# snayfach/MicrobeCensus

Hardware: AMD Instinct MI355X
Metric: reads/sec searched vs marker DB + AGS abs-error, 150 bp @ 1/2/4/8 GPU (higher is better)
Workload: dtype u8/int32

## Files before the change

### include/mcensus.h

```cpp
#ifndef MCENSUS_H
#define MCENSUS_H
#include <stdint.h>
#ifdef __cplusplus
extern "C" {
#endif

typedef struct mc_handle mc_handle;

typedef struct mc_row {
    int32_t query, subject;
    double ident;
    int32_t alnlen, mismatch, gapopen, qstart, qend, sstart, send;
    double loge, bits;
    int32_t score, nmatch;
} mc_row;

typedef struct mc_best_hit {
    int32_t read, family, aln, target_len;
    double bits;
} mc_best_hit;

typedef struct mc_stats {
    int64_t reads, seed_tasks, gap_tasks, hsps, rows, reads_with_rows, classified;
    int64_t bucket_lookups, key_probes;
    float ms_translate, ms_seed, ms_eval, ms_gapped, ms_sort, ms_finish, ms_total;
    int64_t seed_exact_asks, seed_wild_asks, seed_pair_asks, seed_probes;
    int64_t range_splits;
} mc_stats;

const char *mc_last_error(void);
int mc_device_count(void);

mc_handle *mc_open(const char *const *names, const char *const *seqs, int32_t nseq,
                   const int32_t *marker_family, int32_t nfam, int32_t device);
void mc_close(mc_handle *h);
int mc_set_index_cache(const char *dir);
int mc_index_cache_check(const char *const *names, const char *const *seqs, int32_t nseq, const char *dir);

mc_handle *mc_open_rapdb(const char *rapdb_path, int32_t device);
int32_t mc_marker_count(const mc_handle *h);
const char *mc_marker_name(const mc_handle *h, int32_t i);
int mc_set_families(mc_handle *h, const int32_t *marker_family, int32_t nfam);
int mc_rapdb_verify(const char *rapdb_path, const char *const *names, const char *const *seqs, int32_t nseq);
int mc_rapdb_write(const char *const *names, const char *const *seqs, int32_t nseq, const char *path);

int mc_index_view(const mc_handle *h, const uint8_t **res_codes, const uint32_t **offsets, const uint32_t **bucket_starts,
                  const uint32_t **postings, const uint16_t **keys, int64_t *nres, int64_t *npostings,
                  uint32_t *freq_thr, double letter_p[10]);

int mc_set_run(mc_handle *h, int32_t read_len, double loge_thr, const double *min_cov, const double *min_score,
               const int32_t *max_aaid, const int32_t *aln_stat);

int mc_search(mc_handle *h, const uint8_t *reads, int64_t nreads, int64_t first_read_id);

int mc_search_varlen(mc_handle *h, const uint8_t *bases, const int64_t *offsets, int64_t nreads, int64_t first_read_id);

int mc_set_run_classes(mc_handle *h, const int32_t *class_len, int32_t K, double loge_thr, const double *min_cov, const double *min_score,
                       const int32_t *max_aaid, const int32_t *aln_stat);
int mc_search_classes(mc_handle *h, const uint8_t *rows, int64_t nreads, int32_t stride, int64_t first_read_id);
int64_t mc_result_best_classes(mc_handle *h, const uint8_t **cls);
int mc_result_class_reads(mc_handle *h, int64_t *out );
int64_t mc_debug_classes_prologue(mc_handle *h, const uint8_t *rows, int64_t nreads, int32_t stride, uint32_t *perm, uint32_t *start, int64_t *word0,
                                  uint8_t *sorted, int64_t sorted_cap, float *ms);

int mc_upload(mc_handle *h, const uint8_t *reads, int64_t nreads);
int mc_attach(mc_handle *h, const void *device_reads, int64_t nreads);
int mc_run(mc_handle *h, int64_t first_read_id);
int mc_run_range(mc_handle *h, int64_t first, int64_t count, int64_t first_read_id);

int mc_range_begin(mc_handle *h, int64_t first, int64_t count, int64_t first_read_id);
int mc_range_end(mc_handle *h);
int mc_ranges_in_flight(const mc_handle *h);

int64_t mc_debug_stage(mc_handle *h, int what, void *dst, int64_t cap_bytes, int32_t *record_bytes);
void mc_debug_live(int64_t out[4]);

int mc_set_counting(mc_handle *h, int on);

int64_t mc_result_rows(mc_handle *h, const mc_row **rows);
int64_t mc_result_best_hits(mc_handle *h, const mc_best_hit **hits);
int mc_result_stats(mc_handle *h, mc_stats *out);

int mc_write_m8(mc_handle *h, const char *path, int append);
int mc_write_m8_named(mc_handle *h, const char *path, int append, const char *const *query_names, int64_t n_names, int64_t first_read_id);

int mc_grid_classify(mc_handle *h, const double *aln_covs, int32_t n_cov, const int32_t *max_pids, int32_t n_pid, const double *min_scores, int32_t n_score,
                     int64_t *count_hits, int64_t *count_aln, double *count_cov);

int mc_bootstrap(mc_handle *h, const mc_best_hit *best, int64_t n, const int32_t *family_stat, int32_t nfam, int32_t B, uint64_t seed,
                 int64_t *sums_i64, double *sums_f64);
float mc_bootstrap_ms(const mc_handle *h);

int mc_fit_weights(mc_handle *h, const double *pred, const double *truth, int32_t N, int32_t F, uint64_t seed, int32_t read_len, int32_t C, int32_t G,
                   double *weights, double *trace);
int mc_weights_mue(mc_handle *h, const double *pred, const double *truth, int32_t N, int32_t F, const double *w, int32_t K, double *out);
float mc_fit_weights_ms(const mc_handle *h);

typedef struct mc_genome mc_genome;
mc_genome *mc_genome_open(const uint8_t *bases, const int64_t *contig_off, int32_t ncontig, int32_t device);
void mc_genome_close(mc_genome *g);
int mc_simulate(mc_genome *g, int32_t read_len, int64_t first, int64_t n, uint64_t seed, uint64_t library_id, uint8_t *dst_host);
enum { MC_ERR_NONE = 0, MC_ERR_UNIFORM = 1, MC_ERR_ILLUMINA = 2 };
typedef struct mc_library { int32_t paired_end, insert, error_model; double error_rate; } mc_library;
int mc_genome_set_library(mc_genome *g, const mc_library *lib);
enum { MC_READLEN_FIXED = 0, MC_READLEN_REFERENCE = 1 };
int mc_genome_set_read_lengths(mc_genome *g, int32_t mode);
int64_t mc_simulate_varlen(mc_genome *g, int32_t read_len, int64_t first, int64_t n, uint64_t seed, uint64_t library_id, uint8_t *dst_host,
                           int64_t dst_cap, int64_t *offsets);
int mc_train_library(mc_handle *h, mc_genome *g, int64_t nreads, uint64_t seed, uint64_t library_id, const double *aln_covs, int32_t n_cov,
                     const int32_t *max_pids, int32_t n_pid, const double *min_scores, int32_t n_score, int64_t *count_hits, int64_t *count_aln, double *count_cov);
int64_t mc_train_library_bases(const mc_handle *h);
int mc_train_times(const mc_handle *h, float *ms);

typedef struct mc_community mc_community;
mc_community *mc_community_open(const uint8_t *bases, const int64_t *contig_off, int32_t ncontig, const int32_t *member_first_contig,
                                const int64_t *copies, int32_t M, int32_t device);
void mc_community_close(mc_community *c);
int mc_community_set_library(mc_community *c, const mc_library *lib);
int mc_community_simulate(mc_community *c, int32_t read_len, int64_t first, int64_t n, uint64_t seed, uint64_t library_id, uint8_t *dst_host);
int mc_community_library(mc_handle *h, mc_community *c, int64_t nreads, uint64_t seed, uint64_t library_id);
int mc_community_member_reads(mc_community *c, int64_t *out);
int mc_community_times(const mc_handle *h, float *ms);

typedef struct mc_reader mc_reader;
typedef struct mc_reader_stats {
    int64_t sampled, too_short, low_qual, dups;
    int64_t records;
    int64_t bases;
    int64_t exhausted;
    int64_t ragged_end;
} mc_reader_stats;

const char *mc_reader_last_error(void);
void mc_set_host_threads(int32_t n);
mc_reader *mc_reader_open(const char *const *paths, int32_t npaths, int32_t read_len, int64_t nreads, int32_t fastq, int32_t quality_offset,
                          double min_quality, double mean_quality, double max_unknown, int32_t filter_dups, const char *fasta_out);
mc_reader *mc_reader_open_classes(const char *const *paths, int32_t npaths, const int32_t *class_len, int32_t K, int64_t nreads, int32_t fastq,
                                  int32_t quality_offset, double min_quality, double mean_quality, double max_unknown, int32_t filter_dups, const char *fasta_out);
int32_t mc_reader_stride(const mc_reader *r);
mc_reader *mc_reader_open_range(const char *path, int64_t byte_lo, int64_t byte_hi, int32_t read_len, int64_t nreads, int32_t fastq,
                                int32_t quality_offset, double min_quality, double mean_quality, double max_unknown);
typedef struct mc_rec_desc { uint64_t h1, h2; uint64_t seq_off; uint32_t len; uint8_t flags, pad[3]; } mc_rec_desc;
typedef struct mc_dupset mc_dupset;
int64_t mc_reader_describe(mc_reader *r, const mc_rec_desc **out);
mc_dupset *mc_dupset_open(void);
void mc_dupset_close(mc_dupset *s);
int mc_dupset_walk(mc_dupset *s, const char *path, const mc_rec_desc *d, int64_t n, uint8_t *verdict);
int64_t mc_reader_take(mc_reader *r, const uint8_t *verdict, int64_t n, int64_t max_take, uint8_t *dst);
mc_reader *mc_reader_open_bz2_part(const char *path, int64_t block_lo, int64_t block_hi, int32_t kind, int32_t read_len, int64_t nreads, int32_t fastq,
                                   int32_t quality_offset, double min_quality, double mean_quality, double max_unknown);
int64_t mc_bz2_blocks(const char *path);
int64_t mc_gz_chunks(const char *path, int64_t chunk_bytes);
mc_reader *mc_reader_open_gz_part(const char *path, int64_t chunk_lo, int64_t chunk_hi, int64_t chunk_bytes, int32_t kind, int32_t read_len, int64_t nreads,
                                  int32_t fastq, int32_t quality_offset, double min_quality, double mean_quality, double max_unknown);
int mc_reader_gz_provide(mc_reader *r, const uint8_t *state, int64_t n);
int64_t mc_reader_gz_end_state(mc_reader *r, uint8_t *out, int64_t cap);
int mc_reader_gz_finish(mc_reader *r, const uint8_t *crc_in, uint8_t *crc_out);
int64_t mc_reader_run(mc_reader *r);
const uint8_t *mc_reader_reads(mc_reader *r);
int mc_reader_get_stats(mc_reader *r, mc_reader_stats *out);
int32_t mc_reader_times(const mc_reader *r, double *out, int32_t n);
void mc_reader_close(mc_reader *r);
void mc_reader_trim(int64_t keep_bytes);
int64_t mc_count_bases(const char *const *paths, int32_t npaths);
int32_t mc_quality_offset(const char *path);

int mc_reader_start(mc_reader *r);
int64_t mc_reader_fetch(mc_reader *r, int64_t first, int64_t max_reads, uint8_t *dst);
int64_t mc_reader_join(mc_reader *r);
int32_t mc_reader_read_len(const mc_reader *r);
int64_t mc_reader_nreads(const mc_reader *r);

int mc_search_files(mc_handle *h, mc_reader *r, int64_t first_read_id);
int mc_search_files_multi(mc_handle *const *handles, int32_t n_dev, mc_reader *r, int64_t first_read_id);
int mc_set_keep_rows(mc_handle *h, int keep);
int mc_set_best_hits_only(mc_handle *h, int on);

int mc_set_abundance(mc_handle *h, int on, int32_t min_ident, int32_t min_aln, double min_bits, double max_loge);
int mc_abundance_reset(mc_handle *h);
int mc_abundance_read(mc_handle *h, int64_t *reads , int64_t *aligned , int64_t *searched, int64_t *assigned);
float mc_abundance_ms(const mc_handle *h);

int mc_set_coverage(mc_handle *h, int on);
int mc_coverage_read(mc_handle *h, int64_t *covered , int64_t *spanned , int64_t *max_depth );
int mc_coverage_depth(mc_handle *h, uint32_t *depth , int64_t n);
float mc_coverage_ms(const mc_handle *h);

#ifdef __cplusplus
}
#endif
#endif
```

### microbecensus_amd/_native.py

```python
import ctypes as C
import gzip
import json
import math
import os
import sys

import numpy as np

_HERE = os.path.dirname(os.path.abspath(__file__))
LIB_PATH = os.path.join(_HERE, "libmcensus_hip.so")
DATA_DIR = os.path.join(_HERE, "data")


class McRow(C.Structure):
    _fields_ = [("query", C.c_int32), ("subject", C.c_int32), ("ident", C.c_double), ("alnlen", C.c_int32),
                ("mismatch", C.c_int32), ("gapopen", C.c_int32), ("qstart", C.c_int32), ("qend", C.c_int32),
                ("sstart", C.c_int32), ("send", C.c_int32), ("loge", C.c_double), ("bits", C.c_double),
                ("score", C.c_int32), ("nmatch", C.c_int32)]


class McBestHit(C.Structure):
    _fields_ = [("read", C.c_int32), ("family", C.c_int32), ("aln", C.c_int32), ("target_len", C.c_int32),
                ("bits", C.c_double)]


class McStats(C.Structure):
    _fields_ = [(n, C.c_int64) for n in ("reads", "seed_tasks", "gap_tasks", "hsps", "rows", "reads_with_rows", "classified", "bucket_lookups", "key_probes")] + \
               [(n, C.c_float) for n in ("ms_translate", "ms_seed", "ms_eval", "ms_gapped", "ms_sort", "ms_finish", "ms_total")] + \
               [("_pad", C.c_float)] + [(n, C.c_int64) for n in ("seed_exact_asks", "seed_wild_asks", "seed_pair_asks", "seed_probes", "range_splits")]


class McLibrary(C.Structure):
    _fields_ = [("paired_end", C.c_int32), ("insert", C.c_int32), ("error_model", C.c_int32), ("error_rate", C.c_double)]


ERROR_MODELS = {None: 0, "uniform": 1, "illumina": 2}


class McReaderStats(C.Structure):
    _fields_ = [(n, C.c_int64) for n in ("sampled", "too_short", "low_qual", "dups", "records", "bases", "exhausted", "ragged_end")]


ROW_DTYPE = np.dtype([("query", "<i4"), ("subject", "<i4"), ("ident", "<f8"), ("alnlen", "<i4"), ("mismatch", "<i4"),
                      ("gapopen", "<i4"), ("qstart", "<i4"), ("qend", "<i4"), ("sstart", "<i4"), ("send", "<i4"),
                      ("loge", "<f8"), ("bits", "<f8"), ("score", "<i4"), ("nmatch", "<i4")], align=True)
BEST_DTYPE = np.dtype([("read", "<i4"), ("family", "<i4"), ("aln", "<i4"), ("target_len", "<i4"), ("bits", "<f8")], align=True)
REC_DESC_DTYPE = np.dtype([("h1", "<u8"), ("h2", "<u8"), ("seq_off", "<u8"), ("len", "<u4"), ("flags", "u1"), ("pad", "u1", (3,))])

_lib = None


def _share_hip_runtime():
    if os.environ.get("MCENSUS_HIP_RUNTIME", "") == "system" or "torch" in sys.modules:
        return
    try:
        import importlib.util
        spec = importlib.util.find_spec("torch")
        cand = os.path.join(os.path.dirname(spec.origin), "lib", "libamdhip64.so") if spec is not None and spec.origin else None
        if cand and os.path.isfile(cand):
            C.CDLL(cand, mode=C.RTLD_GLOBAL)
    except Exception:
        pass


def load_library():
    global _lib
    if _lib is not None:
        return _lib
    path = os.environ.get("MCENSUS_LIB", LIB_PATH)
    if not os.path.isfile(path):
        raise RuntimeError("HIP extension %s is missing: run `python -c 'import __graft_entry__ as g; g.build()'`" % path)
    _share_hip_runtime()
    lib = C.CDLL(path)
    lib.mc_last_error.restype = C.c_char_p
    lib.mc_device_count.restype = C.c_int
    lib.mc_open.restype = C.c_void_p
    lib.mc_open.argtypes = [C.POINTER(C.c_char_p), C.POINTER(C.c_char_p), C.c_int32, C.POINTER(C.c_int32), C.c_int32, C.c_int32]
    lib.mc_close.argtypes = [C.c_void_p]
    lib.mc_set_index_cache.argtypes = [C.c_char_p]
    lib.mc_index_cache_check.argtypes = [C.POINTER(C.c_char_p), C.POINTER(C.c_char_p), C.c_int32, C.c_char_p]
    lib.mc_open_rapdb.restype = C.c_void_p
    lib.mc_open_rapdb.argtypes = [C.c_char_p, C.c_int32]
    lib.mc_marker_count.restype = C.c_int32
    lib.mc_marker_count.argtypes = [C.c_void_p]
    lib.mc_marker_name.restype = C.c_char_p
    lib.mc_marker_name.argtypes = [C.c_void_p, C.c_int32]
    lib.mc_set_families.argtypes = [C.c_void_p, C.POINTER(C.c_int32), C.c_int32]
    lib.mc_rapdb_verify.argtypes = [C.c_char_p, C.POINTER(C.c_char_p), C.POINTER(C.c_char_p), C.c_int32]
    lib.mc_rapdb_write.argtypes = [C.POINTER(C.c_char_p), C.POINTER(C.c_char_p), C.c_int32, C.c_char_p]
    lib.mc_index_view.argtypes = [C.c_void_p] + [C.POINTER(C.c_void_p)] * 5 + [C.POINTER(C.c_int64), C.POINTER(C.c_int64), C.POINTER(C.c_uint32), C.POINTER(C.c_double)]
    lib.mc_set_run.argtypes = [C.c_void_p, C.c_int32, C.c_double, C.POINTER(C.c_double), C.POINTER(C.c_double), C.POINTER(C.c_int32), C.POINTER(C.c_int32)]
    lib.mc_search.argtypes = [C.c_void_p, C.c_void_p, C.c_int64, C.c_int64]
    lib.mc_search_varlen.argtypes = [C.c_void_p, C.c_void_p, C.c_void_p, C.c_int64, C.c_int64]
    lib.mc_upload.argtypes = [C.c_void_p, C.c_void_p, C.c_int64]
    lib.mc_run.argtypes = [C.c_void_p, C.c_int64]
    lib.mc_attach.argtypes = [C.c_void_p, C.c_void_p, C.c_int64]
    lib.mc_run_range.argtypes = [C.c_void_p, C.c_int64, C.c_int64, C.c_int64]
    lib.mc_set_counting.argtypes = [C.c_void_p, C.c_int]
    lib.mc_debug_stage.restype = C.c_int64
    lib.mc_debug_stage.argtypes = [C.c_void_p, C.c_int, C.c_void_p, C.c_int64, C.POINTER(C.c_int32)]
    lib.mc_range_begin.argtypes = [C.c_void_p, C.c_int64, C.c_int64, C.c_int64]
    lib.mc_range_end.argtypes = [C.c_void_p]
    lib.mc_ranges_in_flight.argtypes = [C.c_void_p]
    lib.mc_result_rows.restype = C.c_int64
    lib.mc_result_rows.argtypes = [C.c_void_p, C.POINTER(C.POINTER(McRow))]
    lib.mc_result_best_hits.restype = C.c_int64
    lib.mc_result_best_hits.argtypes = [C.c_void_p, C.POINTER(C.POINTER(McBestHit))]
    lib.mc_result_stats.argtypes = [C.c_void_p, C.POINTER(McStats)]
    lib.mc_write_m8.argtypes = [C.c_void_p, C.c_char_p, C.c_int]
    lib.mc_write_m8_named.argtypes = [C.c_void_p, C.c_char_p, C.c_int, C.POINTER(C.c_char_p), C.c_int64, C.c_int64]
    lib.mc_reader_last_error.restype = C.c_char_p
    lib.mc_set_host_threads.restype = None
    lib.mc_set_host_threads.argtypes = [C.c_int32]
    lib.mc_reader_open.restype = C.c_void_p
    lib.mc_reader_open.argtypes = [C.POINTER(C.c_char_p), C.c_int32, C.c_int32, C.c_int64, C.c_int32, C.c_int32, C.c_double, C.c_double, C.c_double, C.c_int32, C.c_char_p]
    lib.mc_reader_open_range.restype = C.c_void_p
    lib.mc_reader_open_range.argtypes = [C.c_char_p, C.c_int64, C.c_int64, C.c_int32, C.c_int64, C.c_int32, C.c_int32, C.c_double, C.c_double, C.c_double]
    lib.mc_reader_run.restype = C.c_int64
    lib.mc_reader_run.argtypes = [C.c_void_p]
    lib.mc_reader_reads.restype = C.POINTER(C.c_uint8)
    lib.mc_reader_reads.argtypes = [C.c_void_p]
    lib.mc_reader_get_stats.argtypes = [C.c_void_p, C.POINTER(McReaderStats)]
    lib.mc_reader_open_bz2_part.restype = C.c_void_p
    lib.mc_reader_open_bz2_part.argtypes = [C.c_char_p, C.c_int64, C.c_int64, C.c_int32, C.c_int32, C.c_int64, C.c_int32, C.c_int32, C.c_double, C.c_double, C.c_double]
    lib.mc_bz2_blocks.restype = C.c_int64
    lib.mc_bz2_blocks.argtypes = [C.c_char_p]
    lib.mc_gz_chunks.restype = C.c_int64
    lib.mc_gz_chunks.argtypes = [C.c_char_p, C.c_int64]
    lib.mc_reader_open_gz_part.restype = C.c_void_p
    lib.mc_reader_open_gz_part.argtypes = [C.c_char_p, C.c_int64, C.c_int64, C.c_int64, C.c_int32, C.c_int32, C.c_int64, C.c_int32, C.c_int32, C.c_double, C.c_double, C.c_double]
    lib.mc_reader_gz_provide.argtypes = [C.c_void_p, C.c_char_p, C.c_int64]
    lib.mc_reader_gz_end_state.restype = C.c_int64
    lib.mc_reader_gz_end_state.argtypes = [C.c_void_p, C.c_void_p, C.c_int64]
    lib.mc_reader_gz_finish.argtypes = [C.c_void_p, C.c_char_p, C.c_void_p]
    lib.mc_reader_describe.restype = C.c_int64
    lib.mc_reader_describe.argtypes = [C.c_void_p, C.POINTER(C.c_void_p)]
    lib.mc_dupset_open.restype = C.c_void_p
    lib.mc_dupset_close.argtypes = [C.c_void_p]
    lib.mc_dupset_walk.argtypes = [C.c_void_p, C.c_char_p, C.c_void_p, C.c_int64, C.c_void_p]
    lib.mc_reader_take.restype = C.c_int64
    lib.mc_reader_take.argtypes = [C.c_void_p, C.c_void_p, C.c_int64, C.c_int64, C.c_void_p]
    lib.mc_reader_times.restype = C.c_int32
    lib.mc_reader_times.argtypes = [C.c_void_p, C.POINTER(C.c_double), C.c_int32]
    lib.mc_reader_close.argtypes = [C.c_void_p]
    lib.mc_reader_trim.restype = None
    lib.mc_reader_trim.argtypes = [C.c_int64]
    lib.mc_count_bases.restype = C.c_int64
    lib.mc_count_bases.argtypes = [C.POINTER(C.c_char_p), C.c_int32]
    lib.mc_quality_offset.restype = C.c_int32
    lib.mc_quality_offset.argtypes = [C.c_char_p]
    lib.mc_reader_start.argtypes = [C.c_void_p]
    lib.mc_reader_fetch.restype = C.c_int64
    lib.mc_reader_fetch.argtypes = [C.c_void_p, C.c_int64, C.c_int64, C.c_void_p]
    lib.mc_reader_join.restype = C.c_int64
    lib.mc_reader_join.argtypes = [C.c_void_p]
    lib.mc_reader_read_len.restype = C.c_int32
    lib.mc_reader_read_len.argtypes = [C.c_void_p]
    lib.mc_reader_nreads.restype = C.c_int64
    lib.mc_reader_nreads.argtypes = [C.c_void_p]
    lib.mc_search_files.argtypes = [C.c_void_p, C.c_void_p, C.c_int64]
    lib.mc_search_files_multi.argtypes = [C.POINTER(C.c_void_p), C.c_int32, C.c_void_p, C.c_int64]
    lib.mc_set_keep_rows.argtypes = [C.c_void_p, C.c_int]
    lib.mc_set_best_hits_only.argtypes = [C.c_void_p, C.c_int]
    lib.mc_grid_classify.argtypes = [C.c_void_p, C.POINTER(C.c_double), C.c_int32, C.POINTER(C.c_int32), C.c_int32, C.POINTER(C.c_double), C.c_int32,
                                     C.POINTER(C.c_int64), C.POINTER(C.c_int64), C.POINTER(C.c_double)]
    lib.mc_bootstrap.argtypes = [C.c_void_p, C.c_void_p, C.c_int64, C.POINTER(C.c_int32), C.c_int32, C.c_int32, C.c_uint64, C.POINTER(C.c_int64), C.POINTER(C.c_double)]
    lib.mc_bootstrap_ms.restype = C.c_float
    lib.mc_bootstrap_ms.argtypes = [C.c_void_p]
    lib.mc_fit_weights.argtypes = [C.c_void_p, C.c_void_p, C.c_void_p, C.c_int32, C.c_int32, C.c_uint64, C.c_int32, C.c_int32, C.c_int32, C.c_void_p, C.c_void_p]
    lib.mc_weights_mue.argtypes = [C.c_void_p, C.c_void_p, C.c_void_p, C.c_int32, C.c_int32, C.c_void_p, C.c_int32, C.c_void_p]
    lib.mc_fit_weights_ms.restype = C.c_float
    lib.mc_fit_weights_ms.argtypes = [C.c_void_p]
    lib.mc_genome_open.restype = C.c_void_p
    lib.mc_genome_open.argtypes = [C.c_void_p, C.c_void_p, C.c_int32, C.c_int32]
    lib.mc_genome_close.restype = None
    lib.mc_genome_close.argtypes = [C.c_void_p]
    lib.mc_genome_set_library.argtypes = [C.c_void_p, C.c_void_p]
    lib.mc_simulate.argtypes = [C.c_void_p, C.c_int32, C.c_int64, C.c_int64, C.c_uint64, C.c_uint64, C.c_void_p]
    lib.mc_train_library.argtypes = [C.c_void_p, C.c_void_p, C.c_int64, C.c_uint64, C.c_uint64, C.POINTER(C.c_double), C.c_int32, C.POINTER(C.c_int32), C.c_int32,
                                     C.POINTER(C.c_double), C.c_int32, C.POINTER(C.c_int64), C.POINTER(C.c_int64), C.POINTER(C.c_double)]
    lib.mc_train_times.argtypes = [C.c_void_p, C.POINTER(C.c_float)]
    lib.mc_genome_set_read_lengths.argtypes = [C.c_void_p, C.c_int32]
    lib.mc_simulate_varlen.restype = C.c_int64
    lib.mc_simulate_varlen.argtypes = [C.c_void_p, C.c_int32, C.c_int64, C.c_int64, C.c_uint64, C.c_uint64, C.c_void_p, C.c_int64, C.c_void_p]
    lib.mc_train_library_bases.restype = C.c_int64
    lib.mc_train_library_bases.argtypes = [C.c_void_p]
    lib.mc_community_open.restype = C.c_void_p
    lib.mc_community_open.argtypes = [C.c_void_p, C.c_void_p, C.c_int32, C.c_void_p, C.c_void_p, C.c_int32, C.c_int32]
    lib.mc_community_close.restype = None
    lib.mc_community_close.argtypes = [C.c_void_p]
    lib.mc_community_set_library.argtypes = [C.c_void_p, C.c_void_p]
    lib.mc_community_simulate.argtypes = [C.c_void_p, C.c_int32, C.c_int64, C.c_int64, C.c_uint64, C.c_uint64, C.c_void_p]
    lib.mc_community_library.argtypes = [C.c_void_p, C.c_void_p, C.c_int64, C.c_uint64, C.c_uint64]
    lib.mc_community_member_reads.argtypes = [C.c_void_p, C.c_void_p]
    lib.mc_community_times.argtypes = [C.c_void_p, C.POINTER(C.c_float)]
    lib.mc_set_run_classes.argtypes = [C.c_void_p, C.POINTER(C.c_int32), C.c_int32, C.c_double, C.POINTER(C.c_double), C.POINTER(C.c_double), C.POINTER(C.c_int32), C.POINTER(C.c_int32)]
    lib.mc_search_classes.argtypes = [C.c_void_p, C.c_void_p, C.c_int64, C.c_int32, C.c_int64]
    lib.mc_result_best_classes.restype = C.c_int64
    lib.mc_result_best_classes.argtypes = [C.c_void_p, C.POINTER(C.POINTER(C.c_uint8))]
    lib.mc_result_class_reads.argtypes = [C.c_void_p, C.POINTER(C.c_int64)]
    lib.mc_debug_classes_prologue.restype = C.c_int64
    lib.mc_debug_classes_prologue.argtypes = [C.c_void_p, C.c_void_p, C.c_int64, C.c_int32, C.c_void_p, C.c_void_p, C.c_void_p, C.c_void_p, C.c_int64, C.POINTER(C.c_float)]
    lib.mc_reader_open_classes.restype = C.c_void_p
    lib.mc_reader_open_classes.argtypes = [C.POINTER(C.c_char_p), C.c_int32, C.POINTER(C.c_int32), C.c_int32, C.c_int64, C.c_int32, C.c_int32, C.c_double, C.c_double, C.c_double, C.c_int32, C.c_char_p]
    lib.mc_reader_stride.restype = C.c_int32
    lib.mc_reader_stride.argtypes = [C.c_void_p]
    lib.mc_set_abundance.argtypes = [C.c_void_p, C.c_int, C.c_int32, C.c_int32, C.c_double, C.c_double]
    lib.mc_abundance_reset.argtypes = [C.c_void_p]
    lib.mc_abundance_read.argtypes = [C.c_void_p, C.c_void_p, C.c_void_p, C.POINTER(C.c_int64), C.POINTER(C.c_int64)]
    lib.mc_abundance_ms.restype = C.c_float
    lib.mc_abundance_ms.argtypes = [C.c_void_p]
    lib.mc_set_coverage.argtypes = [C.c_void_p, C.c_int]
    lib.mc_coverage_read.argtypes = [C.c_void_p, C.c_void_p, C.c_void_p, C.c_void_p]
    lib.mc_coverage_depth.argtypes = [C.c_void_p, C.c_void_p, C.c_int64]
    lib.mc_coverage_ms.restype = C.c_float
    lib.mc_coverage_ms.argtypes = [C.c_void_p]
    lib.mc_debug_live.restype = None
    lib.mc_debug_live.argtypes = [C.POINTER(C.c_int64)]
    _lib = lib
    return lib


EXPORTED_SYMBOLS = ["mc_last_error", "mc_device_count", "mc_open", "mc_close", "mc_set_index_cache", "mc_index_cache_check", "mc_open_rapdb", "mc_marker_count", "mc_marker_name", "mc_set_families", "mc_rapdb_verify", "mc_rapdb_write", "mc_index_view", "mc_set_run", "mc_search", "mc_search_varlen",
                    "mc_upload", "mc_attach", "mc_run", "mc_run_range", "mc_set_counting", "mc_debug_stage", "mc_range_begin", "mc_range_end", "mc_ranges_in_flight", "mc_result_rows", "mc_result_best_hits", "mc_result_stats", "mc_write_m8", "mc_write_m8_named",
                    "mc_reader_last_error", "mc_set_host_threads", "mc_reader_open", "mc_reader_open_range", "mc_reader_open_bz2_part", "mc_bz2_blocks", "mc_gz_chunks", "mc_reader_open_gz_part", "mc_reader_gz_provide", "mc_reader_gz_end_state", "mc_reader_gz_finish", "mc_reader_run", "mc_reader_reads", "mc_reader_get_stats", "mc_reader_times", "mc_reader_describe", "mc_dupset_open", "mc_dupset_close", "mc_dupset_walk", "mc_reader_take", "mc_reader_close", "mc_reader_trim", "mc_count_bases", "mc_quality_offset",
                    "mc_reader_start", "mc_reader_fetch", "mc_reader_join", "mc_reader_read_len", "mc_reader_nreads", "mc_search_files", "mc_search_files_multi", "mc_set_keep_rows", "mc_set_best_hits_only", "mc_grid_classify", "mc_bootstrap", "mc_bootstrap_ms",
                    "mc_fit_weights", "mc_weights_mue", "mc_fit_weights_ms",
                    "mc_genome_open", "mc_genome_close", "mc_genome_set_library", "mc_simulate", "mc_train_library", "mc_train_times",
                    "mc_genome_set_read_lengths", "mc_simulate_varlen", "mc_train_library_bases",
                    "mc_community_open", "mc_community_close", "mc_community_set_library", "mc_community_simulate", "mc_community_library", "mc_community_member_reads",
                    "mc_community_times",
                    "mc_set_run_classes", "mc_search_classes", "mc_result_best_classes", "mc_result_class_reads", "mc_debug_classes_prologue", "mc_reader_open_classes", "mc_reader_stride",
                    "mc_set_abundance", "mc_abundance_reset", "mc_abundance_read", "mc_abundance_ms",
                    "mc_set_coverage", "mc_coverage_read", "mc_coverage_depth", "mc_coverage_ms", "mc_debug_live"]


class DupSet:

    def __init__(self):
        self.lib = load_library()
        self.s = self.lib.mc_dupset_open()
        if not self.s:
            raise RuntimeError(self.lib.mc_reader_last_error().decode())

    def walk(self, path, descs):
        import numpy as np
        d = np.ascontiguousarray(descs)
        v = np.empty(len(d), np.uint8)
        if self.lib.mc_dupset_walk(self.s, path.encode(), d.ctypes.data, len(d), v.ctypes.data) != 0:
            raise RuntimeError(self.lib.mc_reader_last_error().decode())
        return v

    def close(self):
        if getattr(self, "s", None):
            self.lib.mc_dupset_close(self.s)
            self.s = None

    def __del__(self):
        try:
            self.close()
        except Exception:
            pass


class ReferenceError_(Exception):
    """The reference's Python would have raised inside run_pipeline (which prints the error and returns None)."""


class Reader:

    def __init__(self, paths, read_len, nreads, fastq, quality_offset, min_quality, mean_quality, max_unknown, filter_dups, fasta_out=None):
        lib = load_library()
        if nreads is None:
            nreads = (1 << 63) - 1
        arr = (C.c_char_p * len(paths))(*[p.encode() for p in paths])
        self.lib, self.read_len = lib, read_len
        self.r = lib.mc_reader_open(arr, len(paths), read_len, nreads, 1 if fastq else 0, int(quality_offset), float(min_quality), float(mean_quality),
                                    float(max_unknown), 1 if filter_dups else 0, fasta_out.encode() if fasta_out else None)
        if not self.r:
            raise RuntimeError(lib.mc_reader_last_error().decode())

    @classmethod
    def with_classes(cls, paths, class_len, nreads, fastq, quality_offset, min_quality, mean_quality, max_unknown, filter_dups, fasta_out=None):
        lib = load_library()
        self = cls.__new__(cls)
        if nreads is None:
            nreads = (1 << 63) - 1
        arr = (C.c_char_p * len(paths))(*[p.encode() for p in paths])
        cl = (C.c_int32 * len(class_len))(*[int(x) for x in class_len])
        self.lib, self.class_len = lib, [int(x) for x in class_len]
        self.r = lib.mc_reader_open_classes(arr, len(paths), cl, len(class_len), nreads, 1 if fastq else 0, int(quality_offset), float(min_quality), float(mean_quality),
                                            float(max_unknown), 1 if filter_dups else 0, fasta_out.encode() if fasta_out else None)
        if not self.r:
            raise RuntimeError(lib.mc_reader_last_error().decode())
        self.read_len = lib.mc_reader_stride(self.r)
        return self

    @classmethod
    def on_range(cls, path, byte_lo, byte_hi, read_len, nreads, fastq, quality_offset, min_quality, mean_quality, max_unknown):
        lib = load_library()
        self = cls.__new__(cls)
        self.lib, self.read_len = lib, read_len
        if nreads is None:
            nreads = (1 << 63) - 1
        self.r = lib.mc_reader_open_range(path.encode(), int(byte_lo), int(byte_hi), read_len, nreads, 1 if fastq else 0, int(quality_offset), float(min_quality),
                                          float(mean_quality), float(max_unknown))
        if not self.r:
            raise RuntimeError(lib.mc_reader_last_error().decode())
        return self

    @classmethod
    def on_bz2_part(cls, path, block_lo, block_hi, kind, read_len, nreads, fastq, quality_offset, min_quality, mean_quality, max_unknown):
        lib = load_library()
        self = cls.__new__(cls)
        self.lib, self.read_len = lib, read_len
        if nreads is None:
            nreads = (1 << 63) - 1
        self.r = lib.mc_reader_open_bz2_part(path.encode(), int(block_lo), int(block_hi), ord(kind), read_len, nreads, 1 if fastq else 0, int(quality_offset),
                                             float(min_quality), float(mean_quality), float(max_unknown))
        if not self.r:
            raise RuntimeError(lib.mc_reader_last_error().decode())
        return self

    @classmethod
    def on_gz_part(cls, path, chunk_lo, chunk_hi, chunk_bytes, kind, read_len, nreads, fastq, quality_offset, min_quality, mean_quality, max_unknown):
        lib = load_library()
        self = cls.__new__(cls)
        self.lib, self.read_len = lib, read_len
        if nreads is None:
            nreads = (1 << 63) - 1
        self.r = lib.mc_reader_open_gz_part(path.encode(), int(chunk_lo), int(chunk_hi), int(chunk_bytes), ord(kind), read_len, nreads, 1 if fastq else 0, int(quality_offset),
                                            float(min_quality), float(mean_quality), float(max_unknown))
        if not self.r:
            raise RuntimeError(lib.mc_reader_last_error().decode())
        return self

    def start(self):
        if self.lib.mc_reader_start(self.r) != 0:
            raise RuntimeError(self.lib.mc_reader_last_error().decode())

    def join(self):
        return self.check(self.lib.mc_reader_join(self.r))

    def gz_provide(self, state):
        self.lib.mc_reader_gz_provide(self.r, state if state else None, len(state) if state else 0)

    def gz_end_state(self):
        buf = C.create_string_buffer(32768 + 64)
        n = self.lib.mc_reader_gz_end_state(self.r, buf, len(buf))
        return None if n < 0 else buf.raw[:n]

    def gz_finish(self, crc_in):
        out = C.create_string_buffer(12)
        self.check(self.lib.mc_reader_gz_finish(self.r, crc_in, out))
        return out.raw

    def close(self):
        if getattr(self, "r", None):
            self.lib.mc_reader_close(self.r)
            self.r = None

    def __del__(self):
        try:
            self.close()
        except Exception:
            pass

    def check(self, n):
        if n == -3:
            raise ReferenceError_(self.lib.mc_reader_last_error().decode())
        if n < 0:
            raise RuntimeError(self.lib.mc_reader_last_error().decode())
        return n

    def run(self):
        return self.check(self.lib.mc_reader_run(self.r))

# ... 342 lines not shown
                cov[i], aaid[i], score[i], stat[i] = float(p[0]), int(round(float(p[1]))), float(p[2]), ALN_STAT[p[3]]
                assert float(p[1]) == aaid[i]
        self._check(self.lib.mc_set_run(self.h, read_len, loge_thr, cov, score, aaid, stat), "mc_set_run")
        self.read_len = read_len

    def set_run_classes(self, class_len, pars_by_len=None, families=None, loge_thr=1.0):
        nf, K = self.nfam, len(class_len)
        cov = (C.c_double * (nf * K))(*([0.0] * (nf * K))); score = (C.c_double * (nf * K))(*([0.0] * (nf * K)))
        aaid = (C.c_int32 * (nf * K))(*([100] * (nf * K))); stat = (C.c_int32 * (nf * K))(*([0] * (nf * K)))
        if pars_by_len is not None:
            for k, L in enumerate(class_len):
                for i, fam in enumerate(families):
                    p = pars_by_len[L][fam]
                    j = k * nf + i
                    cov[j], aaid[j], score[j], stat[j] = float(p[0]), int(round(float(p[1]))), float(p[2]), ALN_STAT[p[3]]
                    assert float(p[1]) == aaid[j]
        cl = (C.c_int32 * max(K, 1))(*[int(x) for x in class_len])
        self._check(self.lib.mc_set_run_classes(self.h, cl, K, loge_thr, cov, score, aaid, stat), "mc_set_run_classes")
        self.class_len = [int(x) for x in class_len]
        self.read_len = self.class_len[-1]

    def search_classes(self, rows, first_read_id=0):
        rows = np.ascontiguousarray(rows, dtype=np.uint8)
        assert rows.ndim == 2
        self._check(self.lib.mc_search_classes(self.h, rows.ctypes.data_as(C.c_void_p), rows.shape[0], rows.shape[1], first_read_id), "mc_search_classes")
        return self.class_results()

    def class_results(self):
        best = self.best_hits()
        pc = C.POINTER(C.c_uint8)()
        m = self.lib.mc_result_best_classes(self.h, C.byref(pc))
        if m < 0:
            raise RuntimeError("mc_result_best_classes failed: %s" % self.lib.mc_last_error().decode())
        cls = np.ctypeslib.as_array(pc, shape=(m,)).copy() if m else np.zeros(0, np.uint8)
        out = (C.c_int64 * (len(self.class_len) + 1))()
        self._check(self.lib.mc_result_class_reads(self.h, out), "mc_result_class_reads")
        return best, cls, np.array(list(out), np.int64)

    def classes_prologue(self, rows, want_sorted=True):
        rows = np.ascontiguousarray(rows, dtype=np.uint8)
        n, K = rows.shape[0], len(self.class_len)
        perm = np.zeros(n, np.uint32); start = np.zeros(K + 2, np.uint32); word0 = np.zeros(K + 1, np.int64)
        cap = n * rows.shape[1] + 16 * K + 16
        srt = np.zeros(cap if want_sorted else 0, np.uint8)
        ms = (C.c_float * 2)()
        nb = self.lib.mc_debug_classes_prologue(self.h, rows.ctypes.data_as(C.c_void_p), n, rows.shape[1], perm.ctypes.data_as(C.c_void_p), start.ctypes.data_as(C.c_void_p),
                                                word0.ctypes.data_as(C.c_void_p), srt.ctypes.data_as(C.c_void_p) if want_sorted else None, len(srt), ms)
        if nb < 0:
            raise RuntimeError("mc_debug_classes_prologue failed: %s" % self.lib.mc_last_error().decode())
        return perm, start, word0, (srt[:nb] if want_sorted else None), (ms[0], ms[1])

    def search(self, reads, first_read_id=0):
        reads = np.ascontiguousarray(reads, dtype=np.uint8)
        assert reads.ndim == 2 and reads.shape[1] == self.read_len
        self._check(self.lib.mc_search(self.h, reads.ctypes.data_as(C.c_void_p), reads.shape[0], first_read_id), "mc_search")
        return self.results()

    def search_varlen(self, reads, first_read_id=0):
        if isinstance(reads, tuple):
            bases, offsets = reads
            bases = np.ascontiguousarray(bases, dtype=np.uint8)
            offsets = np.ascontiguousarray(offsets, dtype=np.int64)
            if bases.ndim != 1 or offsets.ndim != 1 or len(offsets) < 1:
                raise ValueError("search_varlen: bases and offsets must be 1-D, offsets of n + 1 values")
            if len(offsets) > 1 and (offsets[0] < 0 or offsets[-1] > len(bases) or (np.diff(offsets) < 0).any()):
                raise ValueError("search_varlen: offsets must ascend from >= 0 to at most len(bases)")
        else:
            seqs = [s.encode("latin-1") if isinstance(s, str) else bytes(s) for s in reads]
            bases = np.frombuffer(b"".join(seqs), dtype=np.uint8)
            offsets = np.zeros(len(seqs) + 1, np.int64)
            np.cumsum([len(s) for s in seqs], out=offsets[1:])
        self._check(self.lib.mc_search_varlen(self.h, bases.ctypes.data_as(C.c_void_p), offsets.ctypes.data_as(C.c_void_p), len(offsets) - 1, first_read_id),
                    "mc_search_varlen")
        return self.results()

    def set_best_hits_only(self, on):
        self._check(self.lib.mc_set_best_hits_only(self.h, 1 if on else 0), "mc_set_best_hits_only")

    def search_files(self, reader, first_read_id=0, keep_rows=True, best_only=False):
        self._check(self.lib.mc_set_keep_rows(self.h, 1 if keep_rows else 0), "mc_set_keep_rows")
        self.set_best_hits_only(best_only)
        try:
            rc = self.lib.mc_search_files(self.h, reader.r, first_read_id)
            if rc == -3:
                raise ReferenceError_(self.lib.mc_last_error().decode())
            self._check(rc, "mc_search_files")
        finally:
            self.lib.mc_set_keep_rows(self.h, 1)
            self.lib.mc_set_best_hits_only(self.h, 0)
        return self.results()

    def set_abundance(self, on=True, min_ident=0, min_aln=0, min_bits=0.0, max_loge=1.0):
        if on and (isinstance(min_ident, float) and min_ident != int(min_ident)):
            raise ValueError("min_ident must be an integer percent (%r given)" % (min_ident,))
        self._check(self.lib.mc_set_abundance(self.h, 1 if on else 0, int(min_ident), int(min_aln), float(min_bits), float(max_loge)), "mc_set_abundance")

    def abundance_reset(self):
        self._check(self.lib.mc_abundance_reset(self.h), "mc_abundance_reset")

    def abundance(self):
        n = len(self.names)
        reads = np.zeros(n, np.int64); aligned = np.zeros(n, np.int64)
        searched, assigned = C.c_int64(0), C.c_int64(0)
        self._check(self.lib.mc_abundance_read(self.h, reads.ctypes.data_as(C.c_void_p), aligned.ctypes.data_as(C.c_void_p), C.byref(searched), C.byref(assigned)),
                    "mc_abundance_read")
        return {"reads": reads, "aligned": aligned, "searched": int(searched.value), "assigned": int(assigned.value)}

    def abundance_ms(self):
        return float(self.lib.mc_abundance_ms(self.h))

    def set_coverage(self, on=True):
        self._check(self.lib.mc_set_coverage(self.h, 1 if on else 0), "mc_set_coverage")

    def coverage(self):
        n = len(self.names)
        out = {k: np.zeros(n, np.int64) for k in ("covered", "spanned", "max_depth")}
        self._check(self.lib.mc_coverage_read(self.h, *(out[k].ctypes.data_as(C.c_void_p) for k in ("covered", "spanned", "max_depth"))), "mc_coverage_read")
        return out

    def coverage_depth(self):
        p = [C.c_void_p() for _ in range(5)]
        nres, npost, thr, lp = C.c_int64(), C.c_int64(), C.c_uint32(), (C.c_double * 10)()
        self._check(self.lib.mc_index_view(self.h, *[C.byref(x) for x in p], C.byref(nres), C.byref(npost), C.byref(thr), lp), "mc_index_view")
        depth = np.zeros(int(nres.value), np.uint32)
        self._check(self.lib.mc_coverage_depth(self.h, depth.ctypes.data_as(C.c_void_p), depth.size), "mc_coverage_depth")
        return depth

    def coverage_ms(self):
        return float(self.lib.mc_coverage_ms(self.h))

    def upload(self, reads):
        reads = np.ascontiguousarray(reads, dtype=np.uint8)
        assert reads.ndim == 2 and reads.shape[1] == self.read_len
        self._check(self.lib.mc_upload(self.h, reads.ctypes.data_as(C.c_void_p), reads.shape[0]), "mc_upload")

    def run(self, first_read_id=0):
        self._check(self.lib.mc_run(self.h, first_read_id), "mc_run")

    def attach(self, device_ptr, nreads):
        self._check(self.lib.mc_attach(self.h, C.c_void_p(device_ptr), nreads), "mc_attach")

    def set_counting(self, on):
        self._check(self.lib.mc_set_counting(self.h, 1 if on else 0), "mc_set_counting")

    def range_begin(self, first, count, first_read_id=0):
        self._check(self.lib.mc_range_begin(self.h, first, count, first_read_id), "mc_range_begin")

    def range_end(self):
        self._check(self.lib.mc_range_end(self.h), "mc_range_end")

    def ranges_in_flight(self):
        return self.lib.mc_ranges_in_flight(self.h)

    def run_range(self, first, count, first_read_id=0):
        self._check(self.lib.mc_run_range(self.h, first, count, first_read_id), "mc_run_range")

    def debug_stage(self, what):
        rec = C.c_int32(0)
        n = self.lib.mc_debug_stage(self.h, what, None, 0, C.byref(rec))
        if n < 0:
            raise RuntimeError("mc_debug_stage failed: %s" % self.lib.mc_last_error().decode())
        buf = np.zeros(n, np.uint8)
        if n and self.lib.mc_debug_stage(self.h, what, buf.ctypes.data_as(C.c_void_p), n, C.byref(rec)) != n:
            raise RuntimeError("mc_debug_stage failed: %s" % self.lib.mc_last_error().decode())
        return buf.reshape(-1, rec.value) if rec.value else buf

    def gap_counts(self):
        v = self.debug_stage(4).reshape(-1).view("<u4")
        return {"flanks": int(v[0]), "second_window": int(v[1]), "full_size": int(v[2])}

    def rows(self, copy=True):
        pr = C.POINTER(McRow)()
        n = self.lib.mc_result_rows(self.h, C.byref(pr))
        if not n:
            return np.zeros(0, ROW_DTYPE)
        a = np.ctypeslib.as_array(C.cast(pr, C.POINTER(C.c_uint8)), shape=(n * C.sizeof(McRow),)).view(ROW_DTYPE)
        return a.copy() if copy else a

    def best_hits(self, copy=True):
        pb = C.POINTER(McBestHit)()
        m = self.lib.mc_result_best_hits(self.h, C.byref(pb))
        if not m:
            return np.zeros(0, BEST_DTYPE)
        a = np.ctypeslib.as_array(C.cast(pb, C.POINTER(C.c_uint8)), shape=(m * C.sizeof(McBestHit),)).view(BEST_DTYPE)
        return a.copy() if copy else a

    def results(self):
        return self.rows(), self.best_hits()

    def stats(self):
        s = McStats()
        self._check(self.lib.mc_result_stats(self.h, C.byref(s)), "mc_result_stats")
        return {k: getattr(s, k) for k, _ in McStats._fields_ if not k.startswith("_")}

    def write_m8(self, path, append=False):
        self._check(self.lib.mc_write_m8(self.h, path.encode(), 1 if append else 0), "mc_write_m8")

    def write_m8_named(self, path, names, append=False, first_read_id=0):
        arr = (C.c_char_p * len(names))(*[n.encode() for n in names])
        self._check(self.lib.mc_write_m8_named(self.h, path.encode(), 1 if append else 0, arr, len(names), first_read_id), "mc_write_m8_named")

    def grid_classify(self, aln_covs, max_pids, min_scores):
        nc, npid, ns = len(aln_covs), len(max_pids), len(min_scores)
        shape = (nc, npid, ns, self.nfam)
        hits = np.zeros(shape, np.int64); aln = np.zeros(shape, np.int64); cov = np.zeros(shape, np.float64)
        self._check(self.lib.mc_grid_classify(self.h, (C.c_double * nc)(*aln_covs), nc, (C.c_int32 * npid)(*_grid_pids(max_pids)), npid, (C.c_double * ns)(*min_scores), ns,
                                              hits.ctypes.data_as(C.POINTER(C.c_int64)), aln.ctypes.data_as(C.POINTER(C.c_int64)), cov.ctypes.data_as(C.POINTER(C.c_double))),
                    "mc_grid_classify")
        return hits, aln, cov

    def bootstrap(self, best, stats, B, seed):
        best = np.ascontiguousarray(best, dtype=BEST_DTYPE)
        nfam, B = len(stats), int(B)
        stat = (C.c_int32 * nfam)(*[ALN_STAT.get(s, s) for s in stats])
        si = np.zeros((max(B, 0), nfam + 1), np.int64); sf = np.zeros((max(B, 0), nfam), np.float64)
        self._check(self.lib.mc_bootstrap(self.h, best.ctypes.data_as(C.c_void_p), len(best), stat, nfam, B, int(seed) & 0xFFFFFFFFFFFFFFFF,
                                          si.ctypes.data_as(C.POINTER(C.c_int64)), sf.ctypes.data_as(C.POINTER(C.c_double))), "mc_bootstrap")
        return si, sf

    def bootstrap_ms(self):
        return float(self.lib.mc_bootstrap_ms(self.h))

    def fit_weights(self, pred, truth, seed, read_len, candidates=None, generations=None):
        pred = np.ascontiguousarray(pred, dtype=np.float64)
        truth = np.ascontiguousarray(truth, dtype=np.float64)
        if pred.ndim != 2 or truth.shape != (pred.shape[0],):
            raise ValueError("fit_weights: pred (N, F) and truth (N,)")
        Cn = 0 if candidates is None else int(candidates)
        Gn = -1 if generations is None else int(generations)
        rows = (WFIT_DEFAULT_G if Gn == -1 else max(Gn, 0)) + 1
        w = np.zeros(pred.shape[1], np.float64); trace = np.zeros((rows, 3), np.float64)
        self._check(self.lib.mc_fit_weights(self.h, pred.ctypes.data, truth.ctypes.data, pred.shape[0], pred.shape[1], int(seed) & 0xFFFFFFFFFFFFFFFF, int(read_len), Cn, Gn,
                                            w.ctypes.data, trace.ctypes.data), "mc_fit_weights")
        return w, trace

    def weights_mue(self, pred, truth, w):
        pred = np.ascontiguousarray(pred, dtype=np.float64)
        truth = np.ascontiguousarray(truth, dtype=np.float64)
        w = np.ascontiguousarray(np.atleast_2d(w), dtype=np.float64)
        if pred.ndim != 2 or truth.shape != (pred.shape[0],) or w.shape[1] != pred.shape[1]:
            raise ValueError("weights_mue: pred (N, F), truth (N,) and w (K, F)")
        out = np.zeros(w.shape[0], np.float64)
        self._check(self.lib.mc_weights_mue(self.h, pred.ctypes.data, truth.ctypes.data, pred.shape[0], pred.shape[1], w.ctypes.data, w.shape[0], out.ctypes.data), "mc_weights_mue")
        return out

    def fit_weights_ms(self):
        return float(self.lib.mc_fit_weights_ms(self.h))

    def simulate(self, genome, n, seed, library_id, first=0):
        return genome.simulate(self.read_len, n, seed, library_id, first)

    def train_library(self, genome, nreads, seed, library_id, aln_covs, max_pids, min_scores):
        nc, npid, ns = len(aln_covs), len(max_pids), len(min_scores)
        shape = (nc, npid, ns, self.nfam)
        hits = np.zeros(shape, np.int64); aln = np.zeros(shape, np.int64); cov = np.zeros(shape, np.float64)
        self._check(self.lib.mc_train_library(self.h, genome.g, int(nreads), int(seed), int(library_id), (C.c_double * nc)(*aln_covs), nc,
                                              (C.c_int32 * npid)(*_grid_pids(max_pids)), npid, (C.c_double * ns)(*min_scores), ns,
                                              hits.ctypes.data_as(C.POINTER(C.c_int64)), aln.ctypes.data_as(C.POINTER(C.c_int64)), cov.ctypes.data_as(C.POINTER(C.c_double))),
                    "mc_train_library")
        return hits, aln, cov

    def train_library_bases(self):
        return int(self.lib.mc_train_library_bases(self.h))

    def train_times(self):
        ms = (C.c_float * 3)()
        self._check(self.lib.mc_train_times(self.h, ms), "mc_train_times")
        return {"simulate": ms[0], "search": ms[1], "grid": ms[2]}

    def community_library(self, community, nreads, seed, library_id):
        self._check(self.lib.mc_community_library(self.h, community.c, int(nreads), int(seed), int(library_id)), "mc_community_library")
        return self.best_hits()

    def community_times(self):
        ms = (C.c_float * 2)()
        self._check(self.lib.mc_community_times(self.h, ms), "mc_community_times")
        return {"simulate": ms[0], "search": ms[1]}

    def index_view(self):
        p = [C.c_void_p() for _ in range(5)]
        nres, npost, thr = C.c_int64(), C.c_int64(), C.c_uint32()
        lp = (C.c_double * 10)()
        self._check(self.lib.mc_index_view(self.h, *[C.byref(x) for x in p], C.byref(nres), C.byref(npost), C.byref(thr), lp), "mc_index_view")
        nseq = len(self.names)

        def arr(ptr, dtype, n):
            return np.ctypeslib.as_array(C.cast(ptr, C.POINTER(C.c_uint8)), shape=(n * np.dtype(dtype).itemsize,)).view(dtype).copy()
        return {"res": arr(p[0], "u1", nres.value), "off": arr(p[1], "<u4", nseq + 1), "bstart": arr(p[2], "<u4", 1000001),
                "post": arr(p[3], "<u4", npost.value), "keys": arr(p[4], "<u2", npost.value), "thr": thr.value, "letter_p": list(lp)}


def search_files_multi(engines, reader, first_read_id=0, keep_rows=False, best_only=False):
    lib = load_library()
    arr = (C.c_void_p * len(engines))(*[e.h for e in engines])
    for e in engines:
        lib.mc_set_keep_rows(e.h, 1 if keep_rows else 0)
        lib.mc_set_best_hits_only(e.h, 1 if best_only else 0)
    try:
        rc = lib.mc_search_files_multi(arr, len(engines), reader.r, first_read_id)
        if rc == -3:
            raise ReferenceError_(lib.mc_last_error().decode())
        if rc != 0:
            raise RuntimeError("mc_search_files_multi failed (%d): %s" % (rc, lib.mc_last_error().decode()))
    finally:
        for e in engines:
            lib.mc_set_keep_rows(e.h, 1)
# ... 4 lines not shown
```

### microbecensus_amd/csrc/mc_hip.hip

```cpp
#include "mc_hip_common.h"
#include "k_translate_seg.h"
#include "k_enumerate.h"
#include "k_eval_seeds.h"
#include "k_gapped.h"
#include "k_order.h"
#include "k_finish.h"
#include "k_grid.h"
#include "k_simulate.h"
#include "k_community.h"
#include "k_varlen.h"
#include "k_classes.h"
#include "k_bootstrap.h"
#include "k_wfit.h"
#include "k_abundance.h"
#include "k_coverage.h"
#include "mc_pieces.h"
#include "mc_owned.h"

#include <map>

struct McCtx {
    McStream stream; hipStream_t side = nullptr, side2 = nullptr;
    McEvent ev[8], ev_fork, ev_join, ev_join2;
    int64_t cap_reads = 0; int pool_len = 0;
    int ts_staged = -1;
    uint32_t cap_tasks = 0, cap_gaps = 0, cap_hsps = 0, cap_rows = 0;
    McDev<uint8_t> d_frames_base; uint8_t *d_frames = nullptr;
    McDev<unsigned long long> d_stats;
    McDev<McSeedTask> d_tasks; McDev<McGapTask> d_gaps; McDev<McHsp> d_hsps, d_v, d_tmp;
    McDev<uint64_t> d_k64, d_hkeys, d_hplace, d_places; McDev<uint32_t> d_idx, d_idxo, d_heads, d_scan, d_gsz, d_nv, d_ghist;
    McDev<uint32_t> d_counters;
    McDev<McRow> d_rows; McDev<uint32_t> d_nrow, d_rowoff; McDev<McBestHit> d_best, d_bestof; McDev<uint8_t> d_low, d_cand;
    McDev<McGapCell> d_gws_full; McDev<uint32_t> d_retry, d_retry2; int gap_threads_full = 0;
    McDev<unsigned long long> d_gtab; uint32_t gtab_slots = 0; McDev<uint32_t> d_gleader; McDev<McFlankOut> d_fout;
    McPin<uint32_t> h_c; McPin<unsigned long long> h_stats; McPin<McBestHit> h_best; size_t h_best_cap = 0;
    const uint8_t *reads = nullptr; int64_t n = 0, first_read_id = 0;
    uint32_t ntasks = 0, ngaps = 0, gpad = 0, nh = 0, nh_all = 0, nheads = 0, nrows = 0, nbest = 0, nsegs = 0;
    bool busy = false;
};

struct mc_handle {
    McHostIndex H;
    std::vector<int32_t> fam;
    int nfam = 0, device = 0;
    McDev<uint8_t> d_res_base; uint8_t *d_res = nullptr; McDev<uint32_t> d_off, d_bstart, d_post; McDev<unsigned long long> d_post8; McDev<uint16_t> d_keys; McDev<int32_t> d_fam;
    McDev<McTables> d_T; McDev<McClassPars> d_P;
    McTables hT; McClassPars hP;
    int read_len = 0, FP = 0; bool run_set = false;
    McDev<uint32_t> d_bitmap;
    McDev<McBucketRec> d_rec;
    McDev<uint32_t> d_filt, d_wild, d_pair; McDev<uint64_t> d_segtab; McDev<unsigned long long> d_rt;
    bool fast_enum = false;
    bool count_traffic = false;
    int pipe_nout = 0;
    bool keep_rows = true;
    bool best_only = false;
    bool rows_stay = false;
    float train_ms[3] = {0, 0, 0};
    float comm_ms[2] = {0, 0};
    int64_t train_bases = 0;
    float boot_ms = 0;
    float wfit_ms = 0;
    bool abund = false; McAbundPars abund_pars = {}; McDev<unsigned long long> d_abund; int64_t abund_searched = 0; float abund_ms = 0;
    McEvent ev_abund[2];
    bool cov = false; McDev<uint32_t> d_cov; McDev<unsigned long long> d_covout; float cov_ms = 0;
    McEvent ev_cov[2];
    McPin<uint8_t> stage_pin[2]; McDev<uint8_t> stage_dev[2]; size_t stage_bytes = 0; McStream copy_stream;
    int64_t nreads = 0, cap_own = 0;
    McDev<uint8_t> d_reads;
    const uint8_t *reads_dev = nullptr;
    McCtx ctx;
    McPin<mc_row> pin_slot[2]; size_t pin_slot_cap[2] = {0, 0}; int pin_cur = 0;
    McStream side, side2;
    McStream rows_stream; McEvent ev_rows; bool rows_pending = false, rows_ever = false;
    std::vector<mc_row> all_rows, split_rows;
    const mc_row *res_rows = nullptr; int64_t n_res_rows = 0;
    std::vector<mc_best_hit> best; mc_stats stats;
    McCtx *best_from = nullptr; uint32_t best_count = 0;
    std::map<int, McTables> vl_tables; double vl_thr = 0;
    McClasses cls = {}; bool cls_set = false, cls_results = false; std::vector<McClassPars> cls_pars;
    std::vector<uint8_t> best_cls; int64_t cls_reads[MC_CL_BINS] = {};
};

static McIndex dev_index(const mc_handle *h)
{
    McIndex X; X.res = h->d_res; X.off = h->d_off; X.bstart = h->d_bstart; X.post = h->d_post; X.post8 = h->d_post8; X.keys = h->d_keys; X.rec = h->d_rec; X.filt = h->d_filt; X.wild = h->d_wild; X.pair = h->d_pair; X.rt = h->d_rt; X.rt_mask = h->H.rt_mask; X.nseq = h->H.nseq;
    return X;
}

extern "C" void mc_debug_live(int64_t out[4]) { for (int k = 0; k < MC_LIVE_N; k++) out[k] = mc_live[k].load(); }

extern "C" int mc_device_count(void)
{
    int n = 0;
    if (hipGetDeviceCount(&n) != hipSuccess) return 0;
    return n;
}

extern "C" void mc_close(mc_handle *h)
{
    if (!h) return;
    (void)hipSetDevice(h->device);
    if (h->rows_stream) (void)hipStreamSynchronize(h->rows_stream);
    delete h;
}

struct McUploader {
    static constexpr size_t CH = (size_t)8 << 20;
    McPin<uint8_t> pin[2]; McEvent ev[2]; McStream st; int k = 0; bool used[2] = {false, false};
    int init()
    {
        if (st.create()) return -1;
        for (int i = 0; i < 2; i++) if (pin[i].alloc(CH) || ev[i].create(false)) return -1;
        return 0;
    }
    int put(void *dst, const void *src, size_t bytes)
    {
        for (size_t at = 0; at < bytes; at += CH) {
            const size_t n = std::min(CH, bytes - at);
            if (used[k]) HIPCK(hipEventSynchronize(ev[k]));
            memcpy(pin[k], (const uint8_t *)src + at, n);
            HIPCK(hipMemcpyAsync((uint8_t *)dst + at, pin[k], n, hipMemcpyHostToDevice, st));
            HIPCK(hipEventRecord(ev[k], st)); used[k] = true;
            k ^= 1;
        }
        return 0;
    }
    int finish() { if (st) HIPCK(hipStreamSynchronize(st)); return 0; }
    ~McUploader() { if (st) (void)hipStreamSynchronize(st); }
};

static int open_impl(mc_handle *h, const int32_t *marker_family, int32_t nfam, int32_t device)
{
    int ndev = 0;
    double t0 = mc_now();
    if (hipGetDeviceCount(&ndev) != hipSuccess || ndev <= 0) { g_err = "no HIP device available: libmcensus_hip has no CPU fallback"; return -1; }
    if (device < 0 || device >= ndev) { g_err = "device index out of range"; return -1; }
    if (nfam > 32) { g_err = "at most 32 gene families are supported"; return -1; }
    const int nseq = h->H.nseq;
    if (nseq > 32767) { g_err = "more than 32767 markers: the HSP sort key (read<<43 | subject<<28 | hit order) holds 15 bits of subject index"; return -1; }
    for (int s = 0; s < nseq; s++) if ((int)(h->H.off[s + 1] - h->H.off[s]) > MC_GAP_W - 8) { g_err = "marker longer than the gapped-extension workspace"; return -1; }
    if (marker_family) h->fam.assign(marker_family, marker_family + nseq); else h->fam.assign((size_t)nseq, 0);
    h->nfam = nfam; h->device = device;
    HIPCK(hipSetDevice(device));
    HIPCK(hipFree(nullptr));
    MC_OT("  HIP runtime, device", t0);
    if (h->side.create() || h->side2.create()) return -1;
    {
        McCtx &c = h->ctx;
        if (c.stream.create()) return -1;
        c.side = h->side; c.side2 = h->side2;
        for (auto &e : c.ev) if (e.create()) return -1;
        if (c.ev_fork.create(false) || c.ev_join.create(false) || c.ev_join2.create(false)) return -1;
        if (c.d_counters.alloc(C_N) || c.d_stats.alloc(S_N) || c.d_ghist.alloc((size_t)MC_GS_BINS)) return -1;
        if (c.h_c.alloc(C_N) || c.h_stats.alloc(S_N)) return -1;
    }
    if (h->rows_stream.create() || h->ev_rows.create(false)) return -1;
    const McHostIndex &H = h->H;
    if (H.res.size() >= MC_TASK_ABS_LIMIT) { g_err = "marker database too large: more than 16 M residues (MC_TASK_W3)"; return -1; }
    if (h->d_res_base.alloc(H.res.size() + 128) || h->d_off.alloc(H.off.size()) || h->d_bstart.alloc(H.bstart.size()) || h->d_post.alloc(H.post.size() + 1) || h->d_post8.alloc((H.post.size() + 1) * MC_POST_WORDS) ||
        h->d_keys.alloc(H.keys.size()) || h->d_fam.alloc((size_t)nseq) || h->d_T.alloc(1) || h->d_P.alloc(1)) return -1;
    HIPCK(hipMemset(h->d_res_base, MC_INV, H.res.size() + 128));
    h->d_res = h->d_res_base + 64;
    if (h->d_bitmap.alloc(H.bitmap.size()) || h->d_filt.alloc(H.filt.size()) || h->d_wild.alloc(H.wild.size()) || h->d_pair.alloc(H.pair.size()) || h->d_rt.alloc(H.rt.size())) return -1;
    if (!H.rec.empty() && h->d_rec.alloc(H.rec.size())) return -1;
    {
        McUploader up;
        if (up.init() || up.put(h->d_res, H.res.data(), H.res.size()) || up.put(h->d_off, H.off.data(), H.off.size() * 4) || up.put(h->d_bstart, H.bstart.data(), H.bstart.size() * 4) ||
            up.put(h->d_post, H.post.data(), H.post.size() * 4) || up.put(h->d_keys, H.keys.data(), H.keys.size() * 2) || up.put(h->d_fam, h->fam.data(), (size_t)nseq * 4) ||
            up.put(h->d_bitmap, H.bitmap.data(), H.bitmap.size() * 4) || up.put(h->d_pair, H.pair.data(), H.pair.size() * 4) || up.put(h->d_wild, H.wild.data(), H.wild.size() * 4) ||
            up.put(h->d_rt, H.rt.data(), H.rt.size() * 8) || up.put(h->d_filt, H.filt.data(), H.filt.size() * 4) ||
            (!H.rec.empty() && up.put(h->d_rec, H.rec.data(), H.rec.size() * sizeof(McBucketRec))) || up.finish()) return -1;
    }
    if (H.nseq > 32767) { g_err = "marker database too large: more than 32,767 sequences (MC_POST8)"; return -1; }
    k_post8<<<dim3((unsigned)((H.post.size() + 255) / 256)), dim3(256)>>>(h->d_post, h->d_off, h->d_res, (uint32_t)H.post.size(), h->d_post8);
    HIPCK(hipDeviceSynchronize());
    MC_OT("  index upload", t0);
    if (H.max_bucket > 2047) { g_err = "a seed bucket holds more than 2047 postings: the hit-order key cannot index it"; return -1; }
    h->fast_enum = (H.freq_thr == 0) && !H.rec.empty() && !getenv("MC_FORCE_SEQUENTIAL_ENUM");
    for (int g = 0; g < 10; g++) if (!(H.letter_p[g] > 0.0)) h->fast_enum = false;
    return 0;
}

static std::mutex g_ixc_mu;
static std::string g_ixc_dir;
extern "C" int mc_set_index_cache(const char *dir)
{
    std::unique_lock<std::mutex> lk(g_ixc_mu);
    g_ixc_dir = dir ? dir : "";
    return 0;
}

extern "C" int mc_index_cache_check(const char *const *names, const char *const *seqs, int32_t nseq, const char *dir)
{
    McHostIndex A, B, C2;
    std::string err;
    if (!dir || !mc_build_index(A, names, seqs, nseq, err)) { g_err = err.empty() ? "bad argument" : err; return -1; }
    const uint64_t ih = mc_ixc_input_hash(names, seqs, nseq);
    char nm[64]; snprintf(nm, sizeof nm, "/index_%016llx.mcix", (unsigned long long)ih);
    const std::string path = std::string(dir) + nm;
    if (!mc_index_save(A, ih, path.c_str())) { g_err = "cannot write " + path; return -1; }
    if (!mc_index_load(B, ih, nseq, path.c_str())) { g_err = "the file just written was not accepted"; return 1; }
    if (!(A.names == B.names && A.res_code == B.res_code && A.res == B.res && A.off == B.off && A.bstart == B.bstart && A.post == B.post && A.keys == B.keys && A.bitmap == B.bitmap &&
          A.filt == B.filt && A.wild == B.wild && A.pair == B.pair && A.rt == B.rt && A.rec.size() == B.rec.size() &&
          (A.rec.empty() || memcmp(A.rec.data(), B.rec.data(), A.rec.size() * sizeof(McBucketRec)) == 0) && A.rt_mask == B.rt_mask && A.max_bucket == B.max_bucket &&
          A.freq_thr == B.freq_thr && A.nres == B.nres && A.nseq == B.nseq && memcmp(A.letter_p, B.letter_p, sizeof A.letter_p) == 0)) { g_err = "the index read back differs from the one built"; return 2; }
    if (mc_index_load(C2, ih ^ 1, nseq, path.c_str())) { g_err = "a file of other sequences was accepted"; return 3; }
    if (!mc_index_matches_input(B, names, seqs, nseq)) { g_err = "the index read back does not pass the input comparison"; return 6; }
    {
        McHostIndex D = B;
        if (D.nres > 0) { D.res[(size_t)D.nres / 2] ^= 1; if (mc_index_matches_input(D, names, seqs, nseq)) { g_err = "an index with another residue was accepted"; return 7; } D.res[(size_t)D.nres / 2] ^= 1; }
        if (!D.post.empty()) { const uint32_t keep = D.post[D.post.size() / 2]; D.post[D.post.size() / 2] = ((uint32_t)nseq << 11); if (mc_index_matches_input(D, names, seqs, nseq)) { g_err = "a posting outside the database was accepted"; return 8; } D.post[D.post.size() / 2] = keep; }
        if (!D.rec.empty()) { D.rec[D.rec.size() / 3].start += 1; if (mc_index_matches_input(D, names, seqs, nseq)) { g_err = "a bucket record outside its bucket was accepted"; return 9; } D.rec[D.rec.size() / 3].start -= 1; }
        if (nseq > 1) { std::vector<const char *> nm2(names, names + nseq); std::swap(nm2[0], nm2[1]); if (mc_index_matches_input(D, nm2.data(), seqs, nseq)) { g_err = "other marker names were accepted"; return 10; } }
    }
    {
        FILE *f = fopen(path.c_str(), "r+b");
        if (!f) { g_err = "cannot reopen " + path; return -1; }
        fseek(f, 0, SEEK_END); const long sz = ftell(f);
        fseek(f, sz / 2, SEEK_SET); int c = fgetc(f); fseek(f, sz / 2, SEEK_SET); fputc(c ^ 0x40, f); fclose(f);
        if (mc_index_load(C2, ih, nseq, path.c_str())) { g_err = "a damaged file was accepted"; return 4; }
        f = fopen(path.c_str(), "r+b"); fseek(f, sz / 2, SEEK_SET); fputc(c, f); fclose(f);
        if (truncate(path.c_str(), sz - 9) != 0 || mc_index_load(C2, ih, nseq, path.c_str())) { g_err = "a truncated file was accepted"; return 5; }
    }
    remove(path.c_str());
    return 0;
}

extern "C" mc_handle *mc_open(const char *const *names, const char *const *seqs, int32_t nseq, const int32_t *marker_family, int32_t nfam, int32_t device)
{
    mc_handle *h = new mc_handle();
    std::string err;
    double t0 = mc_now();
    std::string cache;
    uint64_t ih = 0;
    { std::unique_lock<std::mutex> lk(g_ixc_mu); cache = g_ixc_dir; }
    bool loaded = false;
    if (!cache.empty() && nseq > 0) {
        ih = mc_ixc_input_hash(names, seqs, nseq);
        char nm[64]; snprintf(nm, sizeof nm, "/index_%016llx.mcix", (unsigned long long)ih);
        cache += nm;
        loaded = mc_index_load(h->H, ih, nseq, cache.c_str());
        if (loaded && !mc_index_matches_input(h->H, names, seqs, nseq)) { loaded = false; h->H = McHostIndex(); }
        MC_OT(loaded ? "index cache: loaded" : "index cache: none / not usable", t0);
    }
    if (!loaded) {
        if (!mc_build_index(h->H, names, seqs, nseq, err)) { delete h; g_err = err; return nullptr; }
        MC_OT("mc_build_index", t0);
        if (!cache.empty()) { (void)mc_index_save(h->H, ih, cache.c_str()); MC_OT("index cache: written", t0); }
    }
    if (open_impl(h, marker_family, nfam, device) != 0) { std::string e = g_err; mc_close(h); g_err = e; return nullptr; }
    MC_OT("open_impl (device side)", t0);
    return h;
}

extern "C" mc_handle *mc_open_rapdb(const char *rapdb_path, int32_t device)
{
    mc_handle *h = new mc_handle();
    std::string err;
    if (!mc_load_rapdb(h->H, rapdb_path, err)) { delete h; g_err = err; return nullptr; }
    if (open_impl(h, nullptr, 1, device) != 0) { std::string e = g_err; mc_close(h); g_err = e; return nullptr; }
    return h;
}

extern "C" int32_t mc_marker_count(const mc_handle *h) { return h ? h->H.nseq : -1; }
extern "C" const char *mc_marker_name(const mc_handle *h, int32_t i) { return (h && i >= 0 && i < h->H.nseq) ? h->H.names[(size_t)i].c_str() : nullptr; }

extern "C" int mc_set_families(mc_handle *h, const int32_t *marker_family, int32_t nfam)
{
    if (!h || !marker_family) { g_err = "null argument"; return -1; }
    if (nfam < 1 || nfam > 32) { g_err = "1..32 gene families are supported"; return -1; }
    for (int i = 0; i < h->H.nseq; i++) if (marker_family[i] < 0 || marker_family[i] >= nfam) { g_err = "family index out of range"; return -1; }
    HIPCK(hipSetDevice(h->device));
    h->fam.assign(marker_family, marker_family + h->H.nseq);
    h->nfam = nfam;
    HIPCK(hipMemcpy(h->d_fam, h->fam.data(), (size_t)h->H.nseq * 4, hipMemcpyHostToDevice));
    h->run_set = false;
    return 0;
}

extern "C" int mc_rapdb_write(const char *const *names, const char *const *seqs, int32_t nseq, const char *path)
{
    McHostIndex A;
    std::string err;
    if (!mc_build_index(A, names, seqs, nseq, err) || !mc_write_rapdb(A, path, err)) { g_err = err; return -1; }
    return 0;
}

extern "C" int mc_rapdb_verify(const char *rapdb_path, const char *const *names, const char *const *seqs, int32_t nseq)
{
    McHostIndex A, B;
    std::string err;
    if (!mc_load_rapdb(A, rapdb_path, err) || !mc_build_index(B, names, seqs, nseq, err)) { g_err = err; return -1; }
    if (A.nseq != B.nseq || A.off != B.off) { g_err = "sequence count / offsets differ"; return 1; }
    if (A.res != B.res) { g_err = "residues differ"; return 2; }
    if (A.bstart != B.bstart) { g_err = "bucket sizes differ"; return 3; }
    if (A.post != B.post) { g_err = "posting order differs"; return 4; }
    if (A.keys != B.keys) { g_err = "suffix keys differ"; return 5; }
    if (A.names != B.names) { g_err = "names differ"; return 6; }
    return 0;
}

extern "C" int mc_index_view(const mc_handle *h, const uint8_t **res_codes, const uint32_t **offsets, const uint32_t **bucket_starts, const uint32_t **postings,
                             const uint16_t **keys, int64_t *nres, int64_t *npostings, uint32_t *freq_thr, double letter_p[10])
{
    if (!h) { g_err = "null handle"; return -1; }
    *res_codes = h->H.res_code.data(); *offsets = h->H.off.data(); *bucket_starts = h->H.bstart.data(); *postings = h->H.post.data(); *keys = h->H.keys.data();
    *nres = h->H.nres; *npostings = (int64_t)h->H.post.size(); *freq_thr = h->H.freq_thr;
    for (int i = 0; i < 10; i++) letter_p[i] = h->H.letter_p[i];
    return 0;
}

static hipError_t run_tables_up(mc_handle *h) { return hipMemcpy(h->d_T, &h->hT, sizeof(McTables), hipMemcpyHostToDevice); }

extern "C" int mc_set_run(mc_handle *h, int32_t read_len, double loge_thr, const double *min_cov, const double *min_score, const int32_t *max_aaid, const int32_t *aln_stat)
{
    if (!h) { g_err = "null handle"; return -1; }
    if (read_len < 18 || read_len > 3 * MC_MAXAA) { g_err = "read_len out of range (18..510)"; return -1; }
    HIPCK(hipSetDevice(h->device));
    double t0 = mc_now();
    mc_fill_tables(h->hT, h->H, read_len, loge_thr);
    MC_OT("set_run: tables", t0);
    if (mc_seg_fx_verify(h->hT, nullptr) != 0) { g_err = "internal: the fixed-point SEG tests disagree with the reference arithmetic"; return -1; }
    MC_OT("set_run: seg_fx_verify", t0);
    memset(&h->hP, 0, sizeof h->hP);
    h->hP.nfam = h->nfam; h->hP.read_len = read_len;
    for (int f = 0; f < h->nfam; f++) { h->hP.min_cov[f] = min_cov[f]; h->hP.min_score[f] = min_score[f]; h->hP.max_aaid[f] = max_aaid[f]; h->hP.aln_stat[f] = aln_stat[f]; }
    HIPCK(run_tables_up(h));
    if (!h->d_segtab) {
        std::vector<uint64_t> tab;
        mc_build_segtab(h->hT.lnfac, tab);
        if (h->d_segtab.alloc(tab.size())) return -1;
        HIPCK(hipMemcpy(h->d_segtab, tab.data(), tab.size() * 8, hipMemcpyHostToDevice));
    }
    HIPCK(hipMemcpy(h->d_P, &h->hP, sizeof(McClassPars), hipMemcpyHostToDevice));
    const int newFP = ((read_len / 3 + 2) + 3) & ~3;
    if (newFP != h->FP || read_len != h->read_len) h->ctx.cap_reads = 0;
    h->read_len = read_len; h->FP = newFP; h->run_set = true;
    h->cls_set = false;
    MC_OT("set_run: segtab, uploads", t0);
    return 0;
}

static void best_materialize(mc_handle *h);
static int ensure_capacity(mc_handle *h, McCtx &c, int64_t nreads)
{
    if (nreads <= c.cap_reads && h->read_len <= c.pool_len) return 0;
    if (h->best_from == &c) best_materialize(h);
    double t0 = mc_now();
    int64_t cap = nreads;
    if (cap > (1 << 21) - 1) { g_err = "batch larger than 2097151 reads"; return -1; }
    const int64_t L = h->read_len;
    c.cap_reads = 0;
    c.cap_tasks = (uint32_t)std::min<int64_t>(cap * (L + 32) + (1 << 20) + (int64_t)256 * 32 * MC_EN_BLK, 0x7fffffff);
    const int64_t ev_pad = (int64_t)256 * 8 * (MC_EV_BS / 64) * MC_EV_BLK;
    c.cap_gaps = (uint32_t)std::min<int64_t>(cap * (L / 8 + 8) + (1 << 18) + ev_pad, (1 << 27) - 2);
    c.cap_hsps = (uint32_t)std::min<int64_t>(cap * (L / 3 + 8) + (1 << 20) + ev_pad, 0x7fffffff);
    c.cap_rows = (uint32_t)std::min<int64_t>(cap * 16 + (1 << 20), 0x7fffffff);
    c.gap_threads_full = 16 * 1024;
    if (c.d_frames_base.alloc((size_t)cap * 6 * h->FP + 128) || c.d_tasks.alloc(c.cap_tasks) ||
        c.d_gaps.alloc(c.cap_gaps) || c.d_hsps.alloc(c.cap_hsps) || c.d_v.alloc(c.cap_hsps) ||
        c.d_tmp.alloc((size_t)c.cap_hsps * 2) || c.d_k64.alloc(c.cap_hsps) || c.d_hkeys.alloc(c.cap_hsps) || c.d_hplace.alloc(c.cap_hsps) || c.d_places.alloc(c.cap_hsps) || c.d_idx.alloc(c.cap_hsps) ||
        c.d_idxo.alloc(c.cap_hsps) || c.d_heads.alloc((size_t)cap + 2) || c.d_scan.alloc((size_t)4100) || c.d_gsz.alloc(c.cap_hsps) || c.d_nv.alloc((size_t)cap + 1) || c.d_rows.alloc(c.cap_rows) ||
        c.d_low.alloc((size_t)cap + 64) || c.d_cand.alloc((size_t)cap + 64) || c.d_nrow.alloc((size_t)cap + 1) || c.d_rowoff.alloc((size_t)cap + 1) || c.d_best.alloc((size_t)cap + 1) || c.d_bestof.alloc((size_t)cap + 1) ||
        c.d_gws_full.alloc((size_t)c.gap_threads_full * MC_GAP_W) || c.d_retry.alloc((size_t)c.cap_gaps * 2 + (size_t)cap + 1) || c.d_retry2.alloc((size_t)c.cap_gaps * 2) || c.d_gleader.alloc((size_t)c.cap_gaps) ||
        c.d_fout.alloc((size_t)c.cap_gaps * 2))
        return -1;
    c.d_frames = c.d_frames_base + 64;
    HIPCK(hipMemsetAsync(c.d_frames_base, MC_INV, 64, c.stream));
    if (c.h_best.alloc((size_t)cap + 1)) return -1;
    c.h_best_cap = (size_t)cap + 1;
    c.cap_reads = cap; c.pool_len = (int)L;
    HIPCK(hipStreamSynchronize(c.stream));
    MC_OT("ensure_capacity (pools)", t0);
    return 0;
}

static int reads_reserve(mc_handle *h, int64_t nreads)
{
    const int64_t need = nreads * (int64_t)h->read_len + 16;
    if (need > h->cap_own) { if (h->d_reads.alloc((size_t)need)) return -1; h->cap_own = need; }
    return 0;
}

extern "C" int mc_upload(mc_handle *h, const uint8_t *reads, int64_t nreads)
{
    if (!h || !h->run_set) { g_err = "mc_set_run() must be called first"; return -1; }
    HIPCK(hipSetDevice(h->device));
    if (reads_reserve(h, nreads)) return -1;
    if (nreads) HIPCK(hipMemcpyAsync(h->d_reads, reads, (size_t)nreads * h->read_len, hipMemcpyHostToDevice, h->ctx.stream));
    HIPCK(hipStreamSynchronize(h->ctx.stream));
    h->reads_dev = h->d_reads; h->nreads = nreads;
    return 0;
}

extern "C" int mc_attach(mc_handle *h, const void *device_reads, int64_t nreads)
{
    if (!h || !h->run_set) { g_err = "mc_set_run() must be called first"; return -1; }
    h->reads_dev = (const uint8_t *)device_reads; h->nreads = nreads;
    return 0;
}

static float ev_ms(hipEvent_t a, hipEvent_t b) { float ms = 0; (void)hipEventElapsedTime(&ms, a, b); return ms; }

static int stage_wait(McCtx &c) { HIPCK(hipStreamSynchronize(c.stream)); return 0; }
static int counters_to_host(McCtx &c) { HIPCK(hipMemcpyAsync(c.h_c, c.d_counters, sizeof(uint32_t) * C_N, hipMemcpyDeviceToHost, c.stream)); return 0; }

#ifdef MC_EXP_TIMING
static int exp_timing_dump(McCtx &c, char stage)
{
    if (stage == 'a') {
        HIPCK(hipStreamSynchronize(c.stream));
        unsigned long long acc[12], cnt[12];
        HIPCK(hipMemcpyFromSymbol(acc, HIP_SYMBOL(g_ts_acc), sizeof acc)); HIPCK(hipMemcpyFromSymbol(cnt, HIP_SYMBOL(g_ts_cnt), sizeof cnt));
        const char *nm[12] = {"flags", "advance", "numbering", "class-0 rounds", "class-1 rounds", "reduction", "owners", "mask", "staging", "translation", "write-out", ""};
        const double waves = (double)((c.n + MC_TS_READS - 1) / MC_TS_READS) * MC_TS_WAVES;
        for (int k = 0; k < 11; k++) fprintf(stderr, "ts-timing %-15s %9.1f cycles/wave  %8.2f entries/wave  total %8.1f Mcycles\n", nm[k], (double)acc[k] / waves, (double)cnt[k] / waves, acc[k] / 1e6);
        unsigned long long z[12] = {0, 0, 0, 0, 0, 0, 0, 0, 0, 0, 0, 0};
        HIPCK(hipMemcpyToSymbol(HIP_SYMBOL(g_ts_acc), z, sizeof z)); HIPCK(hipMemcpyToSymbol(HIP_SYMBOL(g_ts_cnt), z, sizeof z));
    } else {
        HIPCK(hipStreamSynchronize(c.stream)); HIPCK(hipStreamSynchronize(c.side));
        unsigned long long acc[8], cnt[8];
        HIPCK(hipMemcpyFromSymbol(acc, HIP_SYMBOL(g_fh_acc), sizeof acc)); HIPCK(hipMemcpyFromSymbol(cnt, HIP_SYMBOL(g_fh_cnt), sizeof cnt));
        {
            unsigned long long fr[8];
            HIPCK(hipMemcpyFromSymbol(fr, HIP_SYMBOL(g_fr_acc), sizeof fr));
            const char *fn[7] = {"groups", "items", "std::sort", "threshold, keys", "heap sort", "rows", "classification"};
            for (int k = 0; k < 7; k++) fprintf(stderr, "fr-timing %-17s total %9.1f Mcycles (thread wall time, summed)\n", fn[k], fr[k] / 1e6);
            unsigned long long z8[8] = {0, 0, 0, 0, 0, 0, 0, 0};
            HIPCK(hipMemcpyToSymbol(HIP_SYMBOL(g_fr_acc), z8, sizeof z8));
            HIPCK(hipMemcpyFromSymbol(fr, HIP_SYMBOL(g_fr_acc2), sizeof fr));
            const char *gn[8] = {"-", "sort by frame", "sort by start, stable", "choice", "sum statistics", "copies", "groups (count)", "groups linked (count)"};
            for (int k = 1; k < 8; k++) fprintf(stderr, "fg-timing %-22s %12.1f M\n", gn[k], fr[k] / 1e6);
            HIPCK(hipMemcpyToSymbol(HIP_SYMBOL(g_fr_acc2), z8, sizeof z8));
        }
        {
            unsigned long long ev[8];
            HIPCK(hipMemcpyFromSymbol(ev, HIP_SYMBOL(g_ev_acc), sizeof ev));
            const char *en[7] = {"loop, records asked", "survivors queued", "X-drop extension", "HSP, marks", "records written", "residue wait + seed", "growth, gate"};
            for (int k = 0; k < 7; k++) fprintf(stderr, "ev-timing %-21s total %9.1f Mcycles (lane 0 of every wave)\n", en[k], ev[k] / 1e6);
            unsigned long long z8[8] = {0, 0, 0, 0, 0, 0, 0, 0};
            HIPCK(hipMemcpyToSymbol(HIP_SYMBOL(g_ev_acc), z8, sizeof z8));
            unsigned long long tr[4];
            HIPCK(hipMemcpyFromSymbol(tr, HIP_SYMBOL(g_ev_turns), sizeof tr));
            fprintf(stderr, "ev-turns forward: %.1f M lane-turns in %.2f M wave-turns = %.1f lanes of 64; backward: %.1f M in %.2f M = %.1f lanes\n", tr[0] / 1e6, tr[1] / 1e6, tr[1] ? (double)tr[0] / (double)tr[1] : 0.0,
                    tr[2] / 1e6, tr[3] / 1e6, tr[3] ? (double)tr[2] / (double)tr[3] : 0.0);
            HIPCK(hipMemcpyToSymbol(HIP_SYMBOL(g_ev_turns), z8, sizeof tr));
        }
        const char *nm[8] = {"group starts", "groups", "scan, items", "sort", "threshold, ranks", "heap sort", "rows", "other"};
        for (int k = 0; k < 8; k++) fprintf(stderr, "fh-timing %-17s total %9.1f Mcycles %9llu entries\n", nm[k], acc[k] / 1e6, cnt[k]);
        {
            unsigned long long w[12];
            HIPCK(hipMemcpyFromSymbol(w, HIP_SYMBOL(g_fh_worst), sizeof w));
            fprintf(stderr, "fh-worst read: %llu stacked HSPs, %.3f Mcycles:", w[0] & 0xFFFFF, (double)(w[0] >> 20) / 1e6);
            for (int k = 0; k < 8; k++) fprintf(stderr, " %s %.3f", nm[k], (double)w[1 + k] / 1e6);
            fprintf(stderr, "\n");
            unsigned long long z12[12] = {0, 0, 0, 0, 0, 0, 0, 0, 0, 0, 0, 0};
            HIPCK(hipMemcpyToSymbol(HIP_SYMBOL(g_fh_worst), z12, sizeof z12));
        }
        unsigned long long z[8] = {0, 0, 0, 0, 0, 0, 0, 0};
        HIPCK(hipMemcpyToSymbol(HIP_SYMBOL(g_fh_acc), z, sizeof z)); HIPCK(hipMemcpyToSymbol(HIP_SYMBOL(g_fh_cnt), z, sizeof z));
    }
    return 0;
}
#else
static int exp_timing_dump(McCtx &, char) { return 0; }
#endif

static int stage_a(mc_handle *h, McCtx &c)
{
    const int64_t n = c.n;
    const int L = h->read_len, FP = h->FP;
    hipStream_t st = c.stream;
    McIndex X = dev_index(h);
    c.ntasks = c.ngaps = c.gpad = c.nh = c.nheads = c.nrows = c.nbest = c.nsegs = 0;
    HIPCK(hipMemsetAsync(c.d_counters, 0, sizeof(uint32_t) * C_N, st));
    HIPCK(hipMemsetAsync(c.d_stats, 0, sizeof(unsigned long long) * S_N, st));
    if (h->best_only) HIPCK(hipMemsetAsync(c.d_cand, 0, (size_t)n, st));
    HIPCK(hipMemsetAsync(c.d_low, 0, (size_t)n, st));
    HIPCK(hipEventRecord(c.ev[0], st));
    const int64_t threads = n * 6;
    const size_t lds_rest = (size_t)MC_TS_NLNF(FP) * 8 + (size_t)MC_TS_THREADS * MC_TS_STRIDE(FP);
    const size_t lds_staged = (size_t)MC_TS_STAGE(L) + lds_rest, lds_direct = (size_t)MC_TS_STAGE(0) + lds_rest;
    static const int ts_force = getenv("MC_TS_STAGED") ? atoi(getenv("MC_TS_STAGED")) : -1;
    const size_t cu_lds = 160 * 1024 - 1024;
    const bool staged = ts_force >= 0 ? ts_force != 0 : cu_lds / lds_staged >= cu_lds / lds_direct;
    const size_t lds = staged ? lds_staged : lds_direct;
    c.ts_staged = staged ? 1 : 0;
    const unsigned ts_blocks = (unsigned)((n + MC_TS_READS - 1) / MC_TS_READS);
    if (staged) {
        if (lds > 48 * 1024) HIPCK(hipFuncSetAttribute((const void *)k_translate_seg<true>, hipFuncAttributeMaxDynamicSharedMemorySize, (int)lds));
        k_translate_seg<true><<<dim3(ts_blocks), dim3(MC_TS_THREADS), lds, st>>>(h->d_T, c.reads, L, n, c.d_frames, FP, h->d_segtab);
    } else {
        if (lds > 48 * 1024) HIPCK(hipFuncSetAttribute((const void *)k_translate_seg<false>, hipFuncAttributeMaxDynamicSharedMemorySize, (int)lds));
        k_translate_seg<false><<<dim3(ts_blocks), dim3(MC_TS_THREADS), lds, st>>>(h->d_T, c.reads, L, n, c.d_frames, FP, h->d_segtab);
    }
    HIPCK(hipEventRecord(c.ev[1], st));
    if (exp_timing_dump(c, 'a')) return -1;
    if (h->fast_enum) {
        const bool enq = !h->count_traffic;
        const size_t per_wave = enq ? MC_ENQ_WAVE_LDS(FP, L) : sizeof(McEnWave) + MC_EN_WAVE_LDS(FP, L);
        int waves = 0, bpc = 1;
        {
            static const int shapes_q[][2] = {{8, 2}, {4, 4}, {16, 1}, {12, 1}, {4, 3}, {8, 1}, {4, 2}, {4, 1}};
            static const int shapes_c[][2] = {{12, 2}, {8, 3}, {4, 6}, {4, 5}, {16, 1}, {8, 2}, {4, 4}, {12, 1}, {4, 3}, {8, 1}, {4, 2}, {4, 1}};
            if (enq) { for (const auto &sh : shapes_q) if (!waves && (size_t)sh[1] * (64 + sh[0] * per_wave) <= 160 * 1024) { waves = sh[0]; bpc = sh[1]; } }
            else for (const auto &sh : shapes_c) if (!waves && (size_t)sh[1] * (64 + sh[0] * per_wave) <= 160 * 1024) { waves = sh[0]; bpc = sh[1]; }
        }
        if (!waves) { g_err = "reads too long for the seed kernel's LDS layout"; return -1; }
        const size_t lds2 = 64 + waves * per_wave;
#define MC_LAUNCH_EN(KERNEL, WV)                                                                                                                   \
    do {                                                                                                                                           \
        HIPCK(hipFuncSetAttribute((const void *)KERNEL<WV>, hipFuncAttributeMaxDynamicSharedMemorySize, (int)lds2));                               \
        const int blocks_ = (int)std::min<int64_t>((int64_t)256 * bpc, (n + WV - 1) / WV);                                                         \
        KERNEL<WV><<<dim3(blocks_), dim3(64 * WV), lds2, st>>>(h->d_T, X, h->d_bitmap, c.d_frames, FP, L, n, c.d_tasks, c.cap_tasks, c.d_counters, c.d_stats); \
    } while (0)
        if (enq) { if (waves == 16) MC_LAUNCH_EN(k_enumerate_q, 16); else if (waves == 12) MC_LAUNCH_EN(k_enumerate_q, 12); else if (waves == 8) MC_LAUNCH_EN(k_enumerate_q, 8); else MC_LAUNCH_EN(k_enumerate_q, 4); }
        else { if (waves == 16) MC_LAUNCH_EN(k_enumerate_count, 16); else if (waves == 12) MC_LAUNCH_EN(k_enumerate_count, 12); else if (waves == 8) MC_LAUNCH_EN(k_enumerate_count, 8); else MC_LAUNCH_EN(k_enumerate_count, 4); }
#undef MC_LAUNCH_EN
    } else
        k_enumerate<<<dim3((unsigned)((threads + 255) / 256)), dim3(256), 0, st>>>(h->d_T, X, c.d_frames, FP, L, n, c.d_tasks, c.cap_tasks, c.d_counters, c.d_stats);
    HIPCK(hipEventRecord(c.ev[2], st));
    const size_t lds_ev = (size_t)(MC_EV_BS / 64) * MC_EV_QCAP * 32;
    const bool ranges = h->fast_enum && !h->count_traffic;
    HIPCK(hipFuncSetAttribute(ranges ? (const void *)k_eval_seeds<true> : (const void *)k_eval_seeds<false>, hipFuncAttributeMaxDynamicSharedMemorySize, (int)lds_ev));
    if (ranges) k_eval_seeds<true><<<dim3(256u * MC_EV_BPC), dim3(MC_EV_BS), lds_ev, st>>>(h->d_T, X, c.d_frames, FP, L, c.d_tasks, c.d_counters + C_TASKS, c.cap_tasks, c.d_hsps, c.cap_hsps, c.d_gaps, c.cap_gaps, c.d_counters, h->d_P, h->d_fam, h->best_only ? c.d_cand : nullptr, c.d_hkeys, c.d_low, c.d_hplace);
    else k_eval_seeds<false><<<dim3(256u * MC_EV_BPC), dim3(MC_EV_BS), lds_ev, st>>>(h->d_T, X, c.d_frames, FP, L, c.d_tasks, c.d_counters + C_TASKS, c.cap_tasks, c.d_hsps, c.cap_hsps, c.d_gaps, c.cap_gaps, c.d_counters, h->d_P, h->d_fam, h->best_only ? c.d_cand : nullptr, c.d_hkeys, c.d_low, c.d_hplace);
    HIPCK(hipEventRecord(c.ev[3], st));
    return counters_to_host(c);
}

static int stage_b(mc_handle *h, McCtx &c)
{
    const int L = h->read_len, FP = h->FP;
    hipStream_t st = c.stream;
    McIndex X = dev_index(h);
    if (c.h_c[C_OVERFLOW]) { g_err = "seed task / HSP / gap task buffer overflow"; return -2; }
    c.ntasks = c.h_c[C_TASKS];
    const uint32_t ngaps = c.ngaps = c.h_c[C_GAPS];
    c.gpad = c.h_c[C_GPAD];
    if (ngaps) {
        uint32_t slots = 1u << 16;
        while (slots < 2 * ngaps) slots <<= 1;
        if (slots > c.gtab_slots) { if (c.d_gtab.alloc((size_t)slots)) return -1; c.gtab_slots = slots; }
        if (2 * (uint64_t)ngaps > c.cap_hsps) { g_err = "gap task pool larger than the sort buffers"; return -2; }
        uint32_t *gk = (uint32_t *)c.d_k64.get(), *gi = c.d_idx, *gio = c.d_idxo;
        HIPCK(hipMemsetAsync(c.d_gtab, 0, (size_t)slots * 8, st));
        HIPCK(hipMemsetAsync(c.d_ghist, 0, MC_GS_BINS * sizeof(uint32_t), st));
        k_gap_dedupe<<<dim3((ngaps + 255) / 256), dim3(256), 0, st>>>(X, L, c.d_gaps, ngaps, c.d_gtab, slots - 1, c.d_gleader, gk, gi, c.d_counters);
        k_gap_sort_hist<<<dim3(512), dim3(256), 0, st>>>(gk, c.d_counters + C_ITEMS, 2 * ngaps, c.d_ghist);
        k_gap_sort_scan<<<dim3(1), dim3(1024), 0, st>>>(c.d_ghist);
        k_gap_sort_scatter<<<dim3(512), dim3(256), 0, st>>>(gk, gi, c.d_counters + C_ITEMS, 2 * ngaps, c.d_ghist, gio);
        k_gapped_lds<MC_GAP_WIN, 64, MC_GAP_REFILL><<<dim3(std::min<uint32_t>((2 * ngaps + 63) / 64, 256u * 8u)), dim3(64), 0, st>>>(h->d_T, X, c.d_frames, FP, L, c.d_gaps, gio, c.d_counters + C_ITEMS, c.d_fout,
                                                                                                                          c.d_counters + C_RETRY, c.d_retry, c.d_counters + C_GTAKE);
        k_gapped_lds<MC_GAP_WIN2, MC_GAP_LANES2, 1><<<dim3(256u * 4u), dim3(64), 0, st>>>(h->d_T, X, c.d_frames, FP, L, c.d_gaps, c.d_retry, c.d_counters + C_RETRY, c.d_fout, c.d_counters + C_RETRY2, c.d_retry2, c.d_counters + C_GTAKE2);
        k_gapped<<<dim3(c.gap_threads_full / 128), dim3(128), 0, st>>>(h->d_T, X, c.d_frames, FP, L, c.d_gaps, c.d_retry2, c.d_counters + C_RETRY2, c.d_fout, c.d_counters, c.d_gws_full, MC_GAP_W);
        k_gap_emit<<<dim3((ngaps + 255) / 256), dim3(256), 0, st>>>(h->d_T, X, L, c.d_gaps, ngaps, c.d_gleader, c.d_fout, c.d_hsps, c.cap_hsps, c.d_counters, h->d_P, h->d_fam, h->best_only ? c.d_cand : nullptr, c.d_hkeys, c.d_low, c.d_hplace);
    }
    HIPCK(hipEventRecord(c.ev[4], st));
    return counters_to_host(c);
}

static int stage_c(mc_handle *h, McCtx &c)
{
    hipStream_t st = c.stream;
    if (c.h_c[C_OVERFLOW]) { g_err = "HSP buffer overflow"; return -2; }
    const uint32_t nslots = c.h_c[C_HSPS];
    c.nh_all = nslots - c.h_c[C_HPAD];
    c.nh = c.nh_all;
    if (c.nh) {
        const uint32_t n = (uint32_t)c.n;
        const uint8_t *cand = h->best_only ? c.d_cand : nullptr;
        uint32_t *cur = c.d_heads + 1;
        uint64_t *keys = c.d_k64;
        uint32_t *slots = c.d_idxo, *order = c.d_idx, *heavy = c.d_retry2, *heavy2 = c.d_retry2 + c.cap_gaps;
        HIPCK(hipMemsetAsync(c.d_heads, 0, ((size_t)n + 2) * sizeof(uint32_t), st));
        HIPCK(hipMemsetAsync(c.d_nrow, 0, ((size_t)n + 1) * sizeof(uint32_t), st));
        HIPCK(hipMemsetAsync(order, 0xFF, (size_t)nslots * sizeof(uint32_t), st));
        k_bin_count<<<dim3(256u * 8u), dim3(256), 0, st>>>(c.d_hkeys, c.d_counters, c.cap_hsps, cand, cur);
        if (mc_scan_u32(cur, n, cur, c.d_scan, st)) return -1;
        k_bin_scatter<<<dim3(256u * 8u), dim3(256), 0, st>>>(c.d_hkeys, c.d_counters, c.cap_hsps, cand, cur, c.d_hplace, keys, c.d_places, slots);
        uint32_t *heavy3 = heavy2 + c.cap_gaps / 2;
        k_order_lists<<<dim3((n + 255) / 256), dim3(256), 0, st>>>(c.d_heads, n, c.d_counters, heavy, heavy2, heavy3);
        hipStream_t side = c.side, side2 = h->best_only ? c.side : c.side2;
        HIPCK(hipEventRecord(c.ev_fork, st)); HIPCK(hipStreamWaitEvent(c.side, c.ev_fork, 0)); HIPCK(hipStreamWaitEvent(c.side2, c.ev_fork, 0));
        HIPCK(hipFuncSetAttribute((const void *)k_order_heavy<1024, MC_ORDER_LDS>, hipFuncAttributeMaxDynamicSharedMemorySize, (int)(MC_ORDER_LDS * 18)));
        k_order_heavy<1024, MC_ORDER_LDS><<<dim3(256u), dim3(1024), MC_ORDER_LDS * 18, side>>>(keys, c.d_places, slots, c.d_heads, heavy3, c.d_counters + C_ORDER3, c.d_counters + C_OTAKE3, c.d_low, order, c.d_gsz, c.d_nv, c.d_nrow, (uint64_t *)c.d_tmp.get());
        k_order_heavy<256, MC_ORDER_MID><<<dim3(256u * 4u), dim3(256), MC_ORDER_MID * 18, side2>>>(keys, c.d_places, slots, c.d_heads, heavy2, c.d_counters + C_ORDER2, c.d_counters + C_OTAKE2, c.d_low, order, c.d_gsz, c.d_nv, c.d_nrow, (uint64_t *)c.d_tmp.get());
        HIPCK(hipEventRecord(c.ev_join, c.side)); HIPCK(hipEventRecord(c.ev_join2, c.side2));
        k_order_light<<<dim3((n + MC_OL_READS - 1) / MC_OL_READS), dim3(256), 0, st>>>(keys, c.d_places, slots, c.d_heads, n, c.d_low, order, c.d_gsz, c.d_nv, c.d_nrow);
        k_order_heavy<64, MC_ORDER_SMALL><<<dim3(256u * 16u), dim3(64), MC_ORDER_SMALL * 18, st>>>(keys, c.d_places, slots, c.d_heads, heavy, c.d_counters + C_ORDER, c.d_counters + C_OTAKE, c.d_low, order, c.d_gsz, c.d_nv, c.d_nrow, (uint64_t *)c.d_tmp.get());
        HIPCK(hipStreamWaitEvent(st, c.ev_join, 0)); HIPCK(hipStreamWaitEvent(st, c.ev_join2, 0));
        k_order_copy<<<dim3(256u * 8u), dim3(256), 0, st>>>(order, c.d_gsz, c.d_hsps, c.d_heads, n, c.d_v);
    }
    HIPCK(hipEventRecord(c.ev[5], st));
    return 0;
}

static int stage_d(mc_handle *h, McCtx &c)
{
    hipStream_t st = c.stream;
    McIndex X = dev_index(h);
    const uint32_t nh = c.nh, nheads = c.nheads = nh ? (uint32_t)c.n : 0u;
    if (nh) {
        uint32_t *d_heavy = c.d_retry, *d_heavy2 = c.d_retry + c.cap_gaps / 2, *d_heavy3 = c.d_retry + c.cap_gaps;
        uint32_t *d_light = c.d_retry + c.cap_gaps + c.cap_gaps / 2;
        uint32_t *d_heavy1 = c.d_retry2, *d_heap_order = c.d_retry2 + c.cap_gaps;
        const uint32_t light_pitch = (uint32_t)c.cap_reads + 1;
        k_heavy_lists<<<dim3((nheads + 255) / 256), dim3(256), 0, st>>>(c.d_nv, nheads, c.d_nrow, c.d_bestof, c.d_counters, d_heavy, d_light, light_pitch, h->best_only ? MC_FH_MIN_BEST : MC_FH_MIN,
                                                                         d_heavy1, d_heavy2, d_heavy3);
        HIPCK(hipEventRecord(c.ev_fork, st));
        {
            const size_t l1 = (size_t)MC_FH_N1 * 16 + 3 * (size_t)(MC_FH_N1 + 2) * 2, l2 = (size_t)MC_FH_N2 * 16 + 3 * (size_t)(MC_FH_N2 + 2) * 2, l3 = (size_t)MC_FH_N3 * 16 + 3 * (size_t)(MC_FH_N3 + 2) * 2;
            HIPCK(hipFuncSetAttribute((const void *)k_finish_heavy<MC_FH_N3, C_HEAVY3, -1>, hipFuncAttributeMaxDynamicSharedMemorySize, (int)l3));
            HIPCK(hipStreamWaitEvent(c.side, c.ev_fork, 0));
            HIPCK(hipStreamWaitEvent(c.side2, c.ev_fork, 0));
            const unsigned wpc2 = (unsigned)std::min<size_t>(8, std::max<size_t>(1, (size_t)(158 * 1024) / (l2 + 1024)));
            uint32_t *d_sorted1 = c.d_retry2 + c.cap_gaps / 2, *d_sorted2 = c.d_retry2 + c.cap_gaps + c.cap_gaps / 2;
            k_heavy_order<<<dim3(1), dim3(1024), 0, c.side2>>>(d_heavy2, c.d_counters + C_HEAVY2, d_heavy, c.d_nv, 2, d_sorted2);
            k_finish_heavy<MC_FH_N2, C_HEAVY2, -1><<<dim3(256 * wpc2), dim3(64), l2, c.side2>>>(h->d_T, X, h->d_P, h->d_fam, c.d_nv, c.d_heads, nheads, c.d_v, c.d_tmp, c.first_read_id,
                                                                                            c.d_nrow, c.d_bestof, c.d_counters, d_heavy, d_sorted2, nullptr);
            k_finish_heavy<MC_FH_N3, C_HEAVY3, -1><<<dim3(256), dim3(64), l3, c.side2>>>(h->d_T, X, h->d_P, h->d_fam, c.d_nv, c.d_heads, nheads, c.d_v, c.d_tmp, c.first_read_id,
                                                                                         c.d_nrow, c.d_bestof, c.d_counters, d_heavy, d_heavy3, nullptr);
            HIPCK(hipEventRecord(c.ev_join2, c.side2));
            k_heavy_order<<<dim3(1), dim3(1024), 0, c.side>>>(d_heavy1, c.d_counters + C_HEAVY1, d_heavy, c.d_nv, 0, d_sorted1);
            k_finish_heavy<MC_FH_N1, C_HEAVY1, -1><<<dim3(256 * 12), dim3(64), l1, c.side>>>(h->d_T, X, h->d_P, h->d_fam, c.d_nv, c.d_heads, nheads, c.d_v, c.d_tmp, c.first_read_id,
                                                                                            c.d_nrow, c.d_bestof, c.d_counters, d_heavy, d_sorted1, nullptr);
            HIPCK(hipStreamWaitEvent(c.side, c.ev_join2, 0));
            const size_t lh = (size_t)(MC_MAX_M8 + 2) * 64 * 4;
            HIPCK(hipFuncSetAttribute((const void *)k_heap_lanes, hipFuncAttributeMaxDynamicSharedMemorySize, (int)lh));
            k_heap_order<<<dim3(1), dim3(1024), 0, c.side>>>(d_heavy, c.d_nrow, c.d_counters, d_heap_order);
            k_heap_lanes<<<dim3(256), dim3(64), lh, c.side>>>(c.d_heads, nheads, nh, c.d_tmp, c.d_nrow, c.d_counters, d_heavy, d_heap_order);
            k_heavy_rows<<<dim3(256 * 12), dim3(64), 0, c.side>>>(h->d_T, X, h->d_P, h->d_fam, c.d_heads, nheads, c.d_v, c.d_tmp, c.first_read_id, c.d_nrow, c.d_bestof, c.d_counters, d_heavy);
            HIPCK(hipEventRecord(c.ev_join, c.side));
        }
        {
            const size_t lb = 32 * (MC_FH_MIN * 16 + 16), ls = 128 * (16 * 16 + 16);
            HIPCK(hipFuncSetAttribute((const void *)k_finish<32, MC_FH_MIN, 2>, hipFuncAttributeMaxDynamicSharedMemorySize, (int)lb));
            k_finish<32, MC_FH_MIN, 2><<<dim3((nheads + 31) / 32, 2), dim3(32), lb, st>>>(h->d_T, X, h->d_P, h->d_fam, c.d_nv, c.d_heads, nheads, c.d_v, c.d_tmp,
                                                                                 c.first_read_id, c.d_nrow, c.d_bestof, d_light, light_pitch, c.d_counters + C_LIGHT0);
            k_finish<128, 16, 0><<<dim3((nheads + 127) / 128, 2), dim3(128), ls, st>>>(h->d_T, X, h->d_P, h->d_fam, c.d_nv, c.d_heads, nheads, c.d_v, c.d_tmp,
                                                                                     c.first_read_id, c.d_nrow, c.d_bestof, d_light, light_pitch, c.d_counters + C_LIGHT0);
        }
        HIPCK(hipStreamWaitEvent(st, c.ev_join, 0));
        if (mc_scan_u32(c.d_nrow, nheads, c.d_rowoff, c.d_scan, st)) return -1;
        if (h->rows_ever) HIPCK(hipStreamWaitEvent(st, h->ev_rows, 0));
        k_emit_rows<<<dim3((nheads + 255) / 256), dim3(256), 0, st>>>(c.d_heads, nheads, c.d_nrow, c.d_rowoff, c.d_tmp, c.d_rows, c.cap_rows, c.d_bestof, c.d_best, c.d_counters, h->best_only ? 0 : 1);
    }
    HIPCK(hipEventRecord(c.ev[6], st));
    if (exp_timing_dump(c, 'd')) return -1;
    HIPCK(hipMemcpyAsync(c.h_stats, c.d_stats, sizeof(unsigned long long) * S_N, hipMemcpyDeviceToHost, st));
    return counters_to_host(c);
}

static bool rows_stay(const mc_handle *h) { return h->rows_stay || (h->abund && !h->keep_rows); }

static int stage_e(mc_handle *h, McCtx &c)
{
    hipStream_t st = c.stream;
    if (c.nrows && !rows_stay(h)) HIPCK(hipMemcpyAsync(h->pin_slot[h->pin_cur], c.d_rows, sizeof(McRow) * c.nrows, hipMemcpyDeviceToHost, h->rows_stream));
    if (c.nbest) HIPCK(hipMemcpyAsync(c.h_best, c.d_best, sizeof(McBestHit) * c.nbest, hipMemcpyDeviceToHost, st));
    return 0;
}

static void rows_wait(mc_handle *h)
{
    if (h->rows_pending) { (void)hipEventSynchronize(h->ev_rows); h->rows_pending = false; }
}

static void stats_add(mc_stats &tot, const mc_stats &s)
{
    tot.reads += s.reads; tot.seed_tasks += s.seed_tasks; tot.gap_tasks += s.gap_tasks; tot.hsps += s.hsps; tot.rows += s.rows;
    tot.reads_with_rows += s.reads_with_rows; tot.classified += s.classified; tot.bucket_lookups += s.bucket_lookups; tot.key_probes += s.key_probes;
    tot.seed_exact_asks += s.seed_exact_asks; tot.seed_wild_asks += s.seed_wild_asks; tot.seed_pair_asks += s.seed_pair_asks; tot.seed_probes += s.seed_probes;
    tot.ms_translate += s.ms_translate; tot.ms_seed += s.ms_seed; tot.ms_eval += s.ms_eval; tot.ms_gapped += s.ms_gapped;
    tot.ms_sort += s.ms_sort; tot.ms_finish += s.ms_finish; tot.ms_total += s.ms_total;
    tot.range_splits += s.range_splits;
}

static int run_range_once(mc_handle *h, int64_t first, int64_t count, int64_t first_read_id);
static void best_materialize(mc_handle *h);

struct McResults {
    std::vector<mc_row> own_rows, &rows;
    std::vector<mc_best_hit> best; std::vector<uint8_t> tag; mc_stats tot;
    bool want_rows, tagged;
    McResults(bool want_rows_, std::vector<mc_row> *rows_ = nullptr, bool tagged_ = false) : rows(rows_ ? *rows_ : own_rows), want_rows(want_rows_), tagged(tagged_) { memset(&tot, 0, sizeof tot); }
    McResults(const McResults &) = delete;
    void take(mc_handle *h, int tag_ = 0)
    {
        if (want_rows) { rows_wait(h); rows.insert(rows.end(), h->res_rows, h->res_rows + h->n_res_rows); }
        best_materialize(h);
        best.insert(best.end(), h->best.begin(), h->best.end());
        if (tagged) tag.insert(tag.end(), h->best.size(), (uint8_t)tag_);
        stats_add(tot, h->stats);
    }
};

extern "C" int mc_run_range(mc_handle *h, int64_t first, int64_t count, int64_t first_read_id)
{
    if (h && h->pipe_nout) { g_err = "mc_run_range: ranges begun with mc_range_begin() are still in flight"; return -1; }
    int rc = run_range_once(h, first, count, first_read_id);
    if (rc != -2 || count <= 1) return rc;
    h->split_rows.clear();
    McResults R(true, &h->split_rows);
    R.tot.range_splits = 1;
    int64_t off = 0, step = std::max<int64_t>(1, count / 2);
    while (off < count) {
        const int64_t nb = std::min<int64_t>(step, count - off);
        rc = run_range_once(h, first + off, nb, first_read_id + off);
        if (rc == -2 && nb > 1) { step = std::max<int64_t>(1, nb / 2); R.tot.range_splits++; continue; }
        if (rc) return rc;
        R.take(h);
        off += nb;
    }
    h->res_rows = R.rows.data(); h->n_res_rows = (int64_t)R.rows.size(); h->best.swap(R.best); h->best_from = nullptr; h->stats = R.tot;
    return 0;
}

static int range_begin(mc_handle *h, McCtx &c, int64_t first, int64_t count, int64_t first_read_id)
{
    if (ensure_capacity(h, c, count)) return -1;
    c.reads = h->reads_dev + first * h->read_len; c.n = count; c.first_read_id = first_read_id;
    const int rc = stage_a(h, c);
    if (rc) { (void)hipStreamSynchronize(c.stream); return rc; }
    c.busy = true;
    return 0;
}

static void best_materialize(mc_handle *h)
{
    McCtx *c = h->best_from;
    if (!c) return;
    h->best_from = nullptr;
    const uint32_t nb = h->best_count;
    std::sort(c->h_best.get(), c->h_best + nb, [](const McBestHit &x, const McBestHit &y) { return x.read < y.read; });
    h->best.resize(nb);
    for (uint32_t i = 0; i < nb; i++) { const McBestHit &x = c->h_best[i]; mc_best_hit &o = h->best[i]; o.read = x.read; o.family = x.family; o.aln = x.aln; o.target_len = x.target_len; o.bits = x.bits; }
}

static int range_end(mc_handle *h, McCtx &c)
{
    c.busy = false;
    h->cls_results = false;
    memset(&h->stats, 0, sizeof h->stats);
    h->res_rows = nullptr; h->n_res_rows = 0; h->best.clear(); h->best_from = nullptr;
    h->stats.reads = c.n;
    int rc = stage_wait(c);
    if (rc == 0) rc = stage_b(h, c);
    if (rc == 0 && (rc = stage_wait(c)) == 0 && (rc = stage_c(h, c)) == 0) rc = stage_d(h, c);
    if (rc == 0) rc = stage_wait(c);
    if (rc == 0 && c.h_c[C_OVERFLOW]) { g_err = "row buffer overflow"; rc = -2; }
    if (rc) { (void)hipStreamSynchronize(c.stream); return rc; }
    h->pin_cur ^= 1;
    c.nrows = (c.nh && !h->best_only) ? c.h_c[C_ROWS] : 0u; c.nsegs = c.h_c[C_SEGS]; c.nbest = c.h_c[C_BEST];
    const bool abund = h->abund && !h->best_only;
    if (abund) {
        HIPCK(hipEventRecord(h->ev_abund[0], c.stream));
        const uint32_t nr = std::min(c.nrows, c.cap_rows);
        if (nr && h->cov) k_abundance_cov<<<dim3((nr + 255) / 256), dim3(256), 0, c.stream>>>(h->abund_pars, c.d_rows, nr, (int32_t)h->H.nseq, h->d_abund, h->d_off, h->d_cov);
        else if (nr) k_abundance<<<dim3((nr + 255) / 256), dim3(256), 0, c.stream>>>(h->abund_pars, c.d_rows, nr, (int32_t)h->H.nseq, h->d_abund);
        HIPCK(hipEventRecord(h->ev_abund[1], c.stream));
    }
    if ((size_t)c.nrows > h->pin_slot_cap[h->pin_cur] && !rows_stay(h)) {
        (void)hipStreamSynchronize(h->rows_stream);
        const size_t want = (size_t)c.nrows + c.nrows / 4 + 1024;
        McPin<mc_row> nb, ob;
        if (nb.alloc(want)) { g_err = "out of pinned host memory for the rows"; return -1; }
        h->pin_slot[h->pin_cur] = std::move(nb); h->pin_slot_cap[h->pin_cur] = want;
        const int other = h->pin_cur ^ 1;
        if (h->pin_slot_cap[other] < want && ob.alloc(want) == 0) { h->pin_slot[other] = std::move(ob); h->pin_slot_cap[other] = want; }
    }
    rc = stage_e(h, c);
    if (rc) { (void)hipStreamSynchronize(c.stream); (void)hipStreamSynchronize(h->rows_stream); return rc; }
    if (c.nrows && !rows_stay(h)) { HIPCK(hipEventRecord(h->ev_rows, h->rows_stream)); h->rows_pending = true; h->rows_ever = true; }
    if ((rc = stage_wait(c)) != 0) return rc;
    if (abund) { h->abund_searched += c.n; h->abund_ms += ev_ms(h->ev_abund[0], h->ev_abund[1]); }
    h->res_rows = rows_stay(h) ? nullptr : (const mc_row *)h->pin_slot[h->pin_cur]; h->n_res_rows = rows_stay(h) ? 0 : (int64_t)c.nrows;
    h->best_from = &c; h->best_count = c.nbest;
#ifdef MC_EXP_TIMING
    { const char *nm[6] = {"staging/other", "append", "lookup", "push", "setup", "expand"}; for (int k = 0; k < 6; k++) fprintf(stderr, "timing %-14s %8.3f Mcycles/wave-avg  %10llu entries\n", nm[k], (double)c.h_stats[4 + k] / 4096.0 / 1e6, c.h_stats[10 + k]); }
#endif
    h->stats.bucket_lookups += (int64_t)c.h_stats[S_LOOKUPS]; h->stats.key_probes += (int64_t)c.h_stats[S_KEYPROBES]; h->stats.seed_tasks += (int64_t)c.h_stats[S_TASKS];
    h->stats.seed_exact_asks += (int64_t)c.h_stats[S_EXACT]; h->stats.seed_wild_asks += (int64_t)c.h_stats[S_WILD]; h->stats.seed_pair_asks += (int64_t)c.h_stats[S_PAIRS]; h->stats.seed_probes += (int64_t)c.h_stats[S_PROBES];
    h->stats.gap_tasks += c.ngaps - c.gpad; h->stats.hsps += c.nh_all; h->stats.rows += c.nrows; h->stats.reads_with_rows += c.nsegs;
    h->stats.ms_translate += ev_ms(c.ev[0], c.ev[1]); h->stats.ms_seed += ev_ms(c.ev[1], c.ev[2]); h->stats.ms_eval += ev_ms(c.ev[2], c.ev[3]);
    h->stats.ms_gapped += ev_ms(c.ev[3], c.ev[4]); h->stats.ms_sort += ev_ms(c.ev[4], c.ev[5]); h->stats.ms_finish += ev_ms(c.ev[5], c.ev[6]); h->stats.ms_total += ev_ms(c.ev[0], c.ev[6]);
    h->stats.classified = (int64_t)c.nbest;
    return 0;
}

static int range_check(mc_handle *h, int64_t first, int64_t count)
{
    if (!h || !h->run_set) { g_err = "mc_set_run() must be called first"; return -1; }
    if (first < 0 || count < 0 || first + count > h->nreads) { g_err = "range outside the resident read set"; return -1; }
    if (count > (1 << 21) - 1) { g_err = "batch larger than 2097151 reads"; return -1; }
    HIPCK(hipSetDevice(h->device));
    return 0;
}

static int run_range_once(mc_handle *h, int64_t first, int64_t count, int64_t first_read_id)
{
    if (range_check(h, first, count)) return -1;
    if (count == 0) { memset(&h->stats, 0, sizeof h->stats); h->res_rows = nullptr; h->n_res_rows = 0; h->best.clear(); h->best_from = nullptr; return 0; }
    McCtx &c = h->ctx;
    const int rc = range_begin(h, c, first, count, first_read_id);
    if (rc) return rc;
    return range_end(h, c);
}

extern "C" int mc_range_begin(mc_handle *h, int64_t first, int64_t count, int64_t first_read_id)
{
    if (range_check(h, first, count)) return -1;
    if (count <= 0) { g_err = "mc_range_begin: an empty range"; return -1; }
    if (h->pipe_nout) { g_err = "mc_range_begin: a range is in flight already (mc_range_end first)"; return -1; }
    const int rc = range_begin(h, h->ctx, first, count, first_read_id);
    if (rc) return rc;
    h->pipe_nout = 1;
    return 0;
}

extern "C" int mc_range_end(mc_handle *h)
{
    if (!h) { g_err = "null handle"; return -1; }
    if (h->pipe_nout == 0) { g_err = "mc_range_end: no range in flight"; return -1; }
    HIPCK(hipSetDevice(h->device));
    h->pipe_nout = 0;
    return range_end(h, h->ctx);
}

extern "C" int mc_ranges_in_flight(const mc_handle *h) { return h ? h->pipe_nout : 0; }

extern "C" int64_t mc_debug_stage(mc_handle *h, int what, void *dst, int64_t cap_bytes, int32_t *record_bytes)
{
    if (!h || !h->run_set || what < 0 || what > 5) { g_err = "mc_debug_stage: bad argument"; return -1; }
    if (h->pipe_nout) { g_err = "mc_debug_stage: ranges are in flight"; return -1; }
    HIPCK(hipSetDevice(h->device));
    const McCtx &c = h->ctx;
    if (what == 4) {
        if (!c.h_c) { g_err = "mc_debug_stage: no range has run"; return -1; }
        const uint32_t v[3] = {c.h_c[C_ITEMS], c.h_c[C_RETRY], c.h_c[C_RETRY2]};
        if (record_bytes) *record_bytes = (int32_t)sizeof(uint32_t);
        if (dst && (int64_t)sizeof v <= cap_bytes) memcpy(dst, v, sizeof v);
        return (int64_t)sizeof v;
    }
    if (what == 5) {
        if (c.ts_staged < 0) { g_err = "mc_debug_stage: no range has run"; return -1; }
        const uint32_t v = (uint32_t)c.ts_staged;
        if (record_bytes) *record_bytes = (int32_t)sizeof v;
        if (dst && (int64_t)sizeof v <= cap_bytes) memcpy(dst, &v, sizeof v);
        return (int64_t)sizeof v;
    }
    const void *src = nullptr; int64_t bytes = 0; int32_t rec = 0;
    if (what == 0) { src = c.d_frames; rec = h->FP; bytes = c.n * 6 * (int64_t)h->FP; }
    else if (what == 1) { src = c.d_tasks; rec = (int32_t)sizeof(McSeedTask); bytes = (int64_t)c.ntasks * rec; }
    else if (what == 2) { src = c.d_gaps; rec = (int32_t)sizeof(McGapTask); bytes = (int64_t)c.ngaps * rec; }
    else { src = c.d_hsps; rec = (int32_t)sizeof(McHsp); bytes = (int64_t)(c.nh_all + (c.h_c ? c.h_c[C_HPAD] : 0u)) * rec; }
    if (record_bytes) *record_bytes = rec;
    if (dst && bytes && bytes <= cap_bytes) { HIPCK(hipStreamSynchronize(c.stream)); HIPCK(hipMemcpy(dst, src, (size_t)bytes, hipMemcpyDeviceToHost)); }
    return bytes;
}

extern "C" int mc_set_counting(mc_handle *h, int on)
{
    if (!h) { g_err = "null handle"; return -1; }
    h->count_traffic = on != 0;
    return 0;
}

extern "C" int mc_run(mc_handle *h, int64_t first_read_id) { return h ? mc_run_range(h, 0, h->nreads, first_read_id) : -1; }

#define MC_STREAM_BATCH 2000000
static int64_t stream_batch()
{
    if (const char *e = getenv("MC_STREAM_BATCH")) { const long long v = atoll(e); if (v >= 1000 && v <= MC_STREAM_BATCH) return (int64_t)v; }
    return MC_STREAM_BATCH;
}
struct McBatchSlot { uint8_t *pin = nullptr, *dev = nullptr; int64_t n = 0, first = 0; int state = 0;  int64_t rc = 0; };

static int run_stream(mc_handle *h, const std::function<int64_t(uint8_t *, int64_t, int64_t *)> &fetch, int64_t first_read_id, int64_t expect_reads = 0)
{
    HIPCK(hipSetDevice(h->device));
    if (h->pipe_nout) { g_err = "ranges begun with mc_range_begin() are still in flight"; return -1; }
    const int64_t BMAX = MC_STREAM_BATCH, B = stream_batch(), L = h->read_len;
    double t0 = mc_now();
    int64_t bmax_run = B;
    if (B == BMAX && expect_reads > 0) { bmax_run = 262144; while (bmax_run < BMAX && bmax_run * 4 < expect_reads) bmax_run <<= 1; bmax_run = std::min(bmax_run, BMAX); }
    const size_t stage_bytes = (size_t)(bmax_run * L + 64);
    if (h->stage_bytes < stage_bytes) {
        h->stage_bytes = 0;
        for (int k = 0; k < 2; k++) if (h->stage_pin[k].alloc(stage_bytes) || h->stage_dev[k].alloc(stage_bytes)) return -1;
        h->stage_bytes = stage_bytes;
        MC_OT("run_stream: staging buffers", t0);
    }
    if (!h->copy_stream && h->copy_stream.create()) return -1;
    if (expect_reads > 0 && ensure_capacity(h, h->ctx, std::min<int64_t>(bmax_run, expect_reads))) return -1;
    MC_OT("run_stream: pools", t0);
    McBatchSlot slot[2];
    for (int k = 0; k < 2; k++) { slot[k].pin = h->stage_pin[k]; slot[k].dev = h->stage_dev[k]; }
    std::mutex mu; std::condition_variable cv;
    bool abort_up = false;
    std::string up_err;
    std::thread uploader([&] {
        (void)hipSetDevice(h->device);
        int nb = 0;
        for (int k = 0;; k ^= 1) {
            { std::unique_lock<std::mutex> lk(mu); cv.wait(lk, [&] { return slot[k].state == 0 || abort_up; }); if (abort_up) return; }
            int64_t at = 0;
            const int64_t want = B == BMAX ? std::min<int64_t>(bmax_run, (int64_t)262144 << std::min(nb, 3)) : B;
            nb++;
            const int64_t n = fetch(slot[k].pin, want, &at);
            int64_t rc = n;
            if (n > 0) {
                hipError_t e = hipMemcpyAsync(slot[k].dev, slot[k].pin, (size_t)(n * L), hipMemcpyHostToDevice, h->copy_stream);
                if (e == hipSuccess) e = hipStreamSynchronize(h->copy_stream);
                if (e != hipSuccess) { up_err = std::string("upload: ") + hipGetErrorString(e); rc = -1; }
            }
            std::unique_lock<std::mutex> lk(mu);
            slot[k].n = n > 0 ? n : 0; slot[k].first = at; slot[k].rc = rc; slot[k].state = rc > 0 ? 1 : 2;
            cv.notify_all();
            if (rc <= 0) return;
        }
    });
    h->all_rows.clear();
    if (h->keep_rows && expect_reads > 0) h->all_rows.reserve((size_t)expect_reads * 2 + 1024);
    McResults R(h->keep_rows, &h->all_rows);
    const uint8_t *saved_reads = h->reads_dev; const int64_t saved_n = h->nreads;
    bool pending = false;
    auto collect = [&]() { if (pending) { pending = false; R.take(h); } };
    auto release = [&](int k) { std::unique_lock<std::mutex> lk(mu); slot[k].state = 0; cv.notify_all(); };
    auto end_batch = [&](int k) -> int {
        int r = mc_range_end(h);
        if (r == -2) { h->reads_dev = slot[k].dev; h->nreads = slot[k].n; r = mc_run_range(h, 0, slot[k].n, first_read_id + slot[k].first); }
        if (r) return r;
        pending = true;
        release(k);
        return 0;
    };
    int rc = 0, flying = -1;
    for (int k = 0;; k ^= 1) {
        {
            bool ready;
            { std::unique_lock<std::mutex> lk(mu); ready = slot[k].state != 0; }
            if (!ready && flying >= 0) { if ((rc = end_batch(flying)) != 0) break; flying = -1; collect(); }
        }
        { std::unique_lock<std::mutex> lk(mu); cv.wait(lk, [&] { return slot[k].state != 0; }); }
        if (slot[k].state == 2) { if (slot[k].rc < 0) { rc = (int)slot[k].rc; if (!up_err.empty()) g_err = up_err; } break; }
        if (flying >= 0) { if ((rc = end_batch(flying)) != 0) break; flying = -1; }
        h->reads_dev = slot[k].dev; h->nreads = slot[k].n;
        if ((rc = mc_range_begin(h, 0, slot[k].n, first_read_id + slot[k].first)) != 0) break;
        flying = k;
        collect();
    }
    if (rc == 0 && flying >= 0) { rc = end_batch(flying); flying = -1; }
    if (rc == 0) collect();
    if (h->pipe_nout) (void)mc_range_end(h);
    { std::unique_lock<std::mutex> lk(mu); abort_up = true; cv.notify_all(); }
    uploader.join();
    h->reads_dev = saved_reads; h->nreads = saved_n;
    if (rc) return rc;
    h->res_rows = R.rows.data(); h->n_res_rows = (int64_t)R.rows.size(); h->best.swap(R.best); h->best_from = nullptr; h->stats = R.tot;
    return 0;
}

void mc_host_copy(uint8_t *dst, const uint8_t *src, size_t bytes);
int32_t mc_reader_class_list(const mc_reader *r, int32_t *out);
extern "C" int mc_search(mc_handle *h, const uint8_t *reads, int64_t nreads, int64_t first_read_id)
{
    if (!h || !h->run_set) { g_err = "mc_set_run() must be called first"; return -1; }
    if (nreads < 0 || (nreads > 0 && !reads)) { g_err = "bad argument"; return -1; }
    const int64_t L = h->read_len;
    int64_t at = 0;
    return run_stream(h, [&](uint8_t *dst, int64_t max_reads, int64_t *first) -> int64_t {
        const int64_t n = std::max<int64_t>(0, std::min(max_reads, nreads - at));
        if (n > 0) mc_host_copy(dst, reads + at * L, (size_t)(n * L));
        *first = at; at += n;
        return n;
    }, first_read_id, nreads);
}

extern "C" int mc_search_files_multi(mc_handle *const *handles, int32_t n_dev, mc_reader *r, int64_t first_read_id)
{
    if (!handles || n_dev < 1 || !r) { g_err = "bad argument"; return -1; }
    { int32_t cl[MC_CLS_MAX]; if (mc_reader_class_list(r, cl) > 0) { g_err = "mc_search_files_multi: a reader of length classes (one device: mc_search_files)"; return -1; } }
    for (int d = 0; d < n_dev; d++) {
        if (!handles[d] || !handles[d]->run_set) { g_err = "mc_set_run() must be called first on every handle"; return -1; }
        if (mc_reader_read_len(r) != handles[d]->read_len) { g_err = "the reader trims to another length than mc_set_run() was given"; return -1; }
    }
    if (mc_reader_start(r) != 0) { g_err = mc_reader_last_error(); return -1; }
    const int64_t cap_reads = mc_reader_nreads(r);
    const int64_t expect = cap_reads > 0 && cap_reads < ((int64_t)1 << 40) ? (cap_reads + n_dev - 1) / n_dev : 0;
    std::mutex deal_mu;
    int64_t next = 0;
    bool ended = false;
    std::vector<int> rcs((size_t)n_dev, 0);
    std::vector<std::string> errs((size_t)n_dev);
    auto work = [&](int d) {
        std::string ferr;
        rcs[(size_t)d] = run_stream(handles[d], [&](uint8_t *dst, int64_t max_reads, int64_t *first) -> int64_t {
            int64_t at;
            { std::unique_lock<std::mutex> lk(deal_mu); if (ended) return 0; at = next; next += max_reads; }
            const int64_t n = mc_reader_fetch(r, at, max_reads, dst);
            if (n < 0) ferr = mc_reader_last_error();
            if (n < max_reads) { std::unique_lock<std::mutex> lk(deal_mu); ended = true; }
            *first = at;
            return n;
        }, first_read_id, expect);
        errs[(size_t)d] = !ferr.empty() ? ferr : std::string(rcs[(size_t)d] ? mc_last_error() : "");
    };
    std::vector<std::thread> th;
    for (int d = 1; d < n_dev; d++) th.emplace_back(work, d);
    work(0);
    for (auto &t : th) t.join();
    const int64_t sampled = mc_reader_join(r);
    for (int d = 0; d < n_dev; d++) if (rcs[(size_t)d] == -3) { g_err = errs[(size_t)d]; return -3; }
    if (sampled == -3) { g_err = mc_reader_last_error(); return -3; }
    for (int d = 0; d < n_dev; d++) if (rcs[(size_t)d]) { g_err = errs[(size_t)d]; return rcs[(size_t)d]; }
    if (sampled < 0) { g_err = mc_reader_last_error(); return (int)sampled; }
    return 0;
}

static int search_files_classes(mc_handle *h, mc_reader *r, int64_t first_read_id);
extern "C" int mc_search_files(mc_handle *h, mc_reader *r, int64_t first_read_id)
{
    int32_t cl[MC_CLS_MAX];
    if (h && r && (h->cls_set || mc_reader_class_list(r, cl) > 0)) return search_files_classes(h, r, first_read_id);
    return mc_search_files_multi(&h, 1, r, first_read_id);
}

struct McModeGuard {
    mc_handle *h; bool best_only, rows_stay;
    McModeGuard(mc_handle *h_, bool best, bool stay) : h(h_), best_only(h_->best_only), rows_stay(h_->rows_stay) { h->best_only = best; h->rows_stay = stay; }
    McModeGuard(const McModeGuard &) = delete;
    ~McModeGuard() { h->best_only = best_only; h->rows_stay = rows_stay; }
};

struct McLenBorrow {
    mc_handle *h; int read_len, FP; const uint8_t *reads_dev; int64_t nreads; bool tables = false, pars = false, open = true;
    explicit McLenBorrow(mc_handle *h_) : h(h_), read_len(h_->read_len), FP(h_->FP), reads_dev(h_->reads_dev), nreads(h_->nreads) {}
    McLenBorrow(const McLenBorrow &) = delete;
    ~McLenBorrow() { (void)close(-1); }
    void set_len(int L) { h->read_len = L; h->FP = ((L / 3 + 2) + 3) & ~3; }
    int pools(int Lmax, int64_t nmax)
    {
        set_len(Lmax);
        return ensure_capacity(h, h->ctx, std::min<int64_t>(std::max(h->ctx.cap_reads, nmax), (1 << 21) - 1));
    }
    int use(int L, const McClassPars *P = nullptr)
    {
        if (h->vl_thr != h->hT.loge_thr) { h->vl_tables.clear(); h->vl_thr = h->hT.loge_thr; }
        auto it = h->vl_tables.find(L);
        if (it == h->vl_tables.end()) { it = h->vl_tables.emplace(L, McTables()).first; mc_fill_tables(it->second, h->H, L, h->vl_thr); }
        tables = true;
        HIPCK(hipMemcpy(h->d_T, &it->second, sizeof(McTables), hipMemcpyHostToDevice));
        if (P) { pars = true; HIPCK(hipMemcpy(h->d_P, P, sizeof(McClassPars), hipMemcpyHostToDevice)); }
        set_len(L);
        return 0;
    }
    int close(int rc = 0)
    {
        if (!open) return rc;
        open = false;
        h->read_len = read_len; h->FP = FP; h->reads_dev = reads_dev; h->nreads = nreads;
        hipError_t e = tables ? run_tables_up(h) : hipSuccess;
        if (e == hipSuccess && pars) e = hipMemcpy(h->d_P, &h->hP, sizeof(McClassPars), hipMemcpyHostToDevice);
        if (rc == 0 && e != hipSuccess) { g_err = std::string("restoring the run's tables: ") + hipGetErrorString(e); rc = -1; }
        return rc;
    }
};

template <class BlockOf> static int run_pieces(mc_handle *h, McLenBorrow &len, const std::vector<McPiece> &pieces, BlockOf block_of, const McClassPars *pars, McResults &R)
{
    auto begin = [&](const McPiece &q) -> int {
        if (len.use(q.L, pars ? pars + q.tag : nullptr)) return -1;
        h->reads_dev = block_of(q); h->nreads = q.bin_n;
        return mc_range_begin(h, q.first, q.n, q.bin_first + q.first);
    };
    int rc = pieces.empty() ? 0 : begin(pieces[0]);
    for (size_t j = 0; rc == 0 && j < pieces.size(); j++) {
        const McPiece &q = pieces[j];
        rc = mc_range_end(h);
        if (rc == -2) rc = mc_run_range(h, q.first, q.n, q.bin_first + q.first);
        if (rc) break;
        if (j + 1 < pieces.size() && (rc = begin(pieces[j + 1])) != 0) break;
        R.take(h, q.tag);
    }
    if (h->pipe_nout) (void)mc_range_end(h);
    return rc;
}


static int vl_bucket(McDevBuf &B, hipStream_t st, const uint8_t *d_bases, const int64_t *d_off, int64_t nreads, int64_t total, uint8_t **d_sorted,
                     uint32_t **d_perm, std::vector<uint32_t> &start, std::vector<int64_t> &boff)
{
    const uint32_t ntiles = (uint32_t)((nreads + MC_VL_TILE - 1) / MC_VL_TILE);
    int64_t *d_boff = nullptr; uint32_t *d_cnt = nullptr, *d_start = nullptr;
    if (B.get(d_sorted, (size_t)total + 64) || B.get(&d_boff, MC_VL_BINS) || B.get(&d_cnt, (size_t)MC_VL_BINS * ntiles) || B.get(&d_start, MC_VL_BINS + 1) ||
        B.get(d_perm, (size_t)nreads)) return -1;
    HIPCK(hipMemsetAsync(*d_sorted + total, 0, 64, st));
    k_vl_hist<<<dim3(ntiles), dim3(MC_VL_BS), 0, st>>>(d_off, nreads, ntiles, d_cnt);
    HIPCK(hipGetLastError());
    k_bin_scan<<<dim3(1), dim3(1024), 0, st>>>(d_cnt, (uint32_t)MC_VL_BINS * ntiles, ntiles, MC_VL_BINS, d_start);
    HIPCK(hipGetLastError());
    k_vl_scatter<<<dim3(ntiles), dim3(MC_VL_BS), 0, st>>>(d_off, nreads, ntiles, d_cnt, *d_perm);
    HIPCK(hipGetLastError());
    start.assign(MC_VL_BINS + 1, 0);
    HIPCK(hipMemcpyAsync(start.data(), d_start, start.size() * 4, hipMemcpyDeviceToHost, st));
    HIPCK(hipStreamSynchronize(st));
    if (start[MC_VL_BINS] != (uint32_t)nreads) { g_err = "internal: the length buckets do not hold every read"; return -1; }
    boff.assign(MC_VL_BINS, 0);
    for (int L = 1; L < MC_VL_BINS; L++) boff[(size_t)L] = boff[(size_t)L - 1] + (int64_t)(start[(size_t)L] - start[(size_t)L - 1]) * (L - 1);
    HIPCK(hipMemcpyAsync(d_boff, boff.data(), boff.size() * 8, hipMemcpyHostToDevice, st));
    const int64_t waves = MC_VL_BS / 64;
    k_vl_gather<<<dim3((unsigned)std::min<int64_t>((nreads + waves - 1) / waves, MC_VL_GATHER_BLOCKS)), dim3(MC_VL_BS), 0, st>>>(d_bases, d_off, *d_perm, nreads, d_start, d_boff, *d_sorted);
    HIPCK(hipGetLastError());
    return 0;
}

static std::vector<McBin> vl_bins(const std::vector<uint32_t> &start)
{
    std::vector<McBin> bins;
    for (int L = 1; L < MC_VL_BINS; L++) bins.push_back({L, (int64_t)(start[(size_t)L + 1] - start[(size_t)L]), (int64_t)start[(size_t)L]});
    return bins;
}

static int search_varlen(mc_handle *h, const uint8_t *bases, const int64_t *offsets, int64_t nreads, int64_t first_read_id)
{
    McCtx &c = h->ctx;
    const int64_t total = offsets[nreads] - offsets[0];
    std::vector<int64_t> off((size_t)nreads + 1);
    for (int64_t i = 0; i <= nreads; i++) off[(size_t)i] = offsets[i] - offsets[0];
    McDevBuf B;
    uint8_t *d_bases = nullptr, *d_sorted = nullptr; int64_t *d_off = nullptr; uint32_t *d_perm = nullptr;
    if (B.get(&d_bases, (size_t)total + 64) || B.get(&d_off, (size_t)nreads + 1)) return -1;
    hipStream_t st = c.stream;
    HIPCK(hipMemcpyAsync(d_bases, bases + offsets[0], (size_t)total, hipMemcpyHostToDevice, st));
    HIPCK(hipMemcpyAsync(d_off, off.data(), off.size() * 8, hipMemcpyHostToDevice, st));
    std::vector<uint32_t> start; std::vector<int64_t> boff;
    if (vl_bucket(B, st, d_bases, d_off, nreads, total, &d_sorted, &d_perm, start, boff)) { (void)hipStreamSynchronize(st); return -1; }
    std::vector<uint32_t> perm((size_t)nreads);
    HIPCK(hipMemcpyAsync(perm.data(), d_perm, perm.size() * 4, hipMemcpyDeviceToHost, st));
    HIPCK(hipStreamSynchronize(st));
    const McPieces P = mc_cut_pieces(vl_bins(start), stream_batch());
    McResults R(h->keep_rows);
    int rc = 0;
    if (!P.v.empty()) {
        McLenBorrow len(h);
        if ((rc = len.pools(P.Lmax, P.nmax)) == 0) rc = run_pieces(h, len, P.v, [&](const McPiece &q) { return d_sorted + boff[(size_t)q.L]; }, nullptr, R);
        rows_wait(h);
        rc = len.close(rc);
    }
    h->res_rows = nullptr; h->n_res_rows = 0; h->best.clear(); h->best_from = nullptr;
    if (rc) return rc;
    std::vector<int64_t> at((size_t)nreads + 1, 0);
    for (const mc_row &r : R.rows) at[(size_t)perm[(size_t)r.query] + 1]++;
    for (int64_t i = 0; i < nreads; i++) at[(size_t)i + 1] += at[(size_t)i];
    std::vector<mc_row> &out = h->all_rows; out.resize(R.rows.size());
    for (const mc_row &r : R.rows) { const uint32_t o = perm[(size_t)r.query]; mc_row &d = out[(size_t)at[o]++]; d = r; d.query = (int32_t)(first_read_id + o); }
    for (mc_best_hit &b : R.best) b.read = (int32_t)(first_read_id + perm[(size_t)b.read]);
    std::sort(R.best.begin(), R.best.end(), [](const mc_best_hit &x, const mc_best_hit &y) { return x.read < y.read; });
    R.tot.reads += P.nshort;
    if (h->abund) h->abund_searched += P.nshort;
    h->res_rows = out.data(); h->n_res_rows = (int64_t)out.size(); h->best.swap(R.best); h->stats = R.tot;
    return 0;
}

extern "C" int mc_search_varlen(mc_handle *h, const uint8_t *bases, const int64_t *offsets, int64_t nreads, int64_t first_read_id)
{
    if (!h || !h->run_set) { g_err = "mc_set_run() must be called first"; return -1; }
    if (nreads < 0 || !offsets || (nreads > 0 && !bases)) { g_err = "bad argument"; return -1; }
    if (nreads > 0x7fffffff) { g_err = "more than 2^31 - 1 reads in one call"; return -1; }
    if (h->pipe_nout) { g_err = "ranges begun with mc_range_begin() are still in flight"; return -1; }
    bool one = true;
    for (int64_t i = 0; i < nreads; i++) {
        const int64_t len = offsets[i + 1] - offsets[i];
        if (len <= 0) { g_err = "read " + std::to_string(i) + " is empty (offsets " + std::to_string(offsets[i]) + ", " + std::to_string(offsets[i + 1]) + ")"; return -1; }
        if (len > 3 * MC_MAXAA) { g_err = "read " + std::to_string(i) + " is " + std::to_string(len) + " bases long: longer than 510"; return -1; }
        one = one && len == h->read_len;
    }
    if (one) return mc_search(h, nreads ? bases + offsets[0] : nullptr, nreads, first_read_id);
    HIPCK(hipSetDevice(h->device));
    return search_varlen(h, bases, offsets, nreads, first_read_id);
}

extern "C" int mc_set_run_classes(mc_handle *h, const int32_t *class_len, int32_t K, double loge_thr, const double *min_cov, const double *min_score,
                                  const int32_t *max_aaid, const int32_t *aln_stat)
{
    if (!h || !class_len || !min_cov || !min_score || !max_aaid || !aln_stat) { g_err = "null argument"; return -1; }
    int32_t bad = 0;
    const int what = mc_classes_check(class_len, K, &bad);
    if (what == 1) { g_err = "mc_set_run_classes: " + std::to_string(bad) + " length classes (1 .. 32 are supported)"; return -1; }
    if (what == 2) { g_err = "mc_set_run_classes: class length " + std::to_string(bad) + " out of range (18 .. 510)"; return -1; }
    if (what == 3) { g_err = "mc_set_run_classes: class length " + std::to_string(bad) + " does not ascend"; return -1; }
    if (h->pipe_nout) { g_err = "mc_set_run_classes: ranges begun with mc_range_begin() are still in flight"; return -1; }
    const size_t F = (size_t)h->nfam, top = (size_t)(K - 1) * F;
    if (mc_set_run(h, class_len[K - 1], loge_thr, min_cov + top, min_score + top, max_aaid + top, aln_stat + top)) return -1;
    h->cls.K = K;
    h->cls_pars.assign((size_t)K, h->hP);
    for (int k = 0; k < K; k++) {
        h->cls.len[k] = class_len[k];
        McClassPars &P = h->cls_pars[(size_t)k];
        P.read_len = class_len[k];
        for (size_t f = 0; f < F; f++) { P.min_cov[f] = min_cov[k * F + f]; P.min_score[f] = min_score[k * F + f]; P.max_aaid[f] = max_aaid[k * F + f]; P.aln_stat[f] = aln_stat[k * F + f]; }
    }
    h->cls_set = true;
    return 0;
}

struct McClSorted { uint8_t *d_sorted = nullptr; uint32_t *d_perm = nullptr; std::vector<uint32_t> start; McClGather G; float ms[2] = {0, 0}; };

static int cl_prologue(McDevBuf &B, hipStream_t st, const uint8_t *d_rows, int64_t n, int stride, const McClasses &C, McClSorted &S, hipEvent_t *ev = nullptr)
{
    const uint32_t ntiles = (uint32_t)((n + MC_CL_TILE - 1) / MC_CL_TILE), nbins = (uint32_t)C.K + 1;
    uint8_t *d_cls = nullptr; uint32_t *d_cnt = nullptr, *d_start = nullptr;
    if (B.get(&d_cls, (size_t)n) || B.get(&d_cnt, (size_t)nbins * ntiles) || B.get(&d_start, nbins + 1) || B.get(&S.d_perm, (size_t)n)) return -1;
    if (ev) HIPCK(hipEventRecord(ev[0], st));
    k_cl_hist<<<dim3(ntiles), dim3(MC_CL_BS), 0, st>>>(d_rows, n, stride, C, mc_cl_lanes(stride), ntiles, d_cls, d_cnt);
    HIPCK(hipGetLastError());
    k_bin_scan<<<dim3(1), dim3(1024), 0, st>>>(d_cnt, nbins * ntiles, ntiles, nbins, d_start);
    HIPCK(hipGetLastError());
    k_cl_scatter<<<dim3(ntiles), dim3(MC_CL_BS), 0, st>>>(d_cls, n, ntiles, nbins, d_cnt, S.d_perm);
    HIPCK(hipGetLastError());
    if (ev) HIPCK(hipEventRecord(ev[1], st));
    S.start.assign(nbins + 1, 0);
    HIPCK(hipMemcpyAsync(S.start.data(), d_start, S.start.size() * 4, hipMemcpyDeviceToHost, st));
    HIPCK(hipStreamSynchronize(st));
    if (S.start[nbins] != (uint32_t)n) { g_err = "internal: the length classes do not hold every row"; return -1; }
    memset(&S.G, 0, sizeof S.G);
    S.G.K = C.K;
    for (int k = 0; k < C.K; k++) {
        S.G.first[k] = S.start[(size_t)k]; S.G.cnt[k] = S.start[(size_t)k + 1] - S.start[(size_t)k];
        S.G.word0[k + 1] = S.G.word0[k] + ((int64_t)S.G.cnt[k] * C.len[k] + 15) / 16;
    }
    const int64_t W = S.G.word0[C.K];
    if (B.get(&S.d_sorted, (size_t)W * 16 + MC_CL_SLACK)) return -1;
    HIPCK(hipMemsetAsync(S.d_sorted + W * 16, 0, MC_CL_SLACK, st));
    if (ev) HIPCK(hipEventRecord(ev[2], st));
    if (W) {
        k_cl_gather<<<dim3((unsigned)std::min<int64_t>((W + MC_CL_BS - 1) / MC_CL_BS, MC_CL_GATHER_BLOCKS)), dim3(MC_CL_BS), 0, st>>>(d_rows, stride, S.d_perm, C, S.G, S.d_sorted);
        HIPCK(hipGetLastError());
// ... 689 lines not shown
    const int span = span_to_make(*c, L);
    if (span <= 0) return span;
    std::vector<int64_t> vs((size_t)c->ncontig), total((size_t)c->M);
    std::vector<uint64_t> cum((size_t)c->M + 1);
    const int bad = mc_sim_member_table(c->off.data(), c->mfirst.data(), c->copies.data(), c->M, span, vs.data(), total.data(), cum.data());
    if (bad == 1) return no_contig(*c, span);
    if (bad) { g_err = "the community's universe (the sum of copies x valid starts) does not stay below 2^62"; return -1; }
    HIPCK(hipMemcpy(c->d_vstart, vs.data(), sizeof(int64_t) * vs.size(), hipMemcpyHostToDevice));
    HIPCK(hipMemcpy(c->d_total, total.data(), sizeof(int64_t) * total.size(), hipMemcpyHostToDevice));
    HIPCK(hipMemcpy(c->d_cum, cum.data(), sizeof(uint64_t) * cum.size(), hipMemcpyHostToDevice));
    c->span = span;
    return 0;
}

template <class S> static int simulate_begin(S *s, int read_len)
{
    if (read_len < 18 || read_len > 3 * MC_MAXAA) { g_err = "read_len out of range (18..510)"; return -1; }
    HIPCK(hipSetDevice(s->device));
    return source_for_len(s, read_len);
}

static uint64_t sim_key(uint64_t seed, uint64_t library_id) { return mc_mix64(seed ^ mc_mix64(library_id)); }
static McSimKind sim_kind(const McSimSource &s, int L) { return McSimKind{L, s.lib.paired_end ? 1 : 0, s.lib.paired_end ? s.lib.insert : L, s.lib.error_model != MC_ERR_NONE ? 1 : 0}; }

template <class S> static int launch_simulate(const S *s, int L, uint64_t key, int64_t first, int64_t n, uint8_t *dst, hipStream_t st)
{
    if (n <= 0) return 0;
    const auto place = s->placer();
    if (default_library(s->lib)) {
        k_sim_copy<<<dim3((unsigned)((n + 255) / 256)), dim3(256), place.lds_bytes(), st>>>(s->d_bases, place, L, key, first, n, dst);
    } else {
        const size_t lds = (size_t)64 * L + sizeof(uint64_t) * MC_SIM_NTHR + place.lds_bytes();
        k_sim_walk<<<dim3((unsigned)((n + 63) / 64)), dim3(64), lds, st>>>(s->d_bases, place, sim_kind(*s, L), s->d_thr, key, mc_mix64(key ^ MC_SIM_EKEY), first, n, dst);
    }
    HIPCK(hipGetLastError());
    return 0;
}

template <class S> static int simulate_to_host(const S *s, int L, int64_t first, int64_t n, uint64_t key, uint8_t *dst_host, const char *fn)
{
    const int64_t B = std::min<int64_t>(n, stream_batch());
    McDevBuf buf;
    uint8_t *d = nullptr;
    if (buf.get(&d, (size_t)(B * L))) return -1;
    for (int64_t at = 0; at < n; at += B) {
        const int64_t cnt = std::min(B, n - at);
        if (launch_simulate(s, L, key, first + at, cnt, d, nullptr)) return -1;
        if (hipMemcpy(dst_host + at * L, d, (size_t)(cnt * L), hipMemcpyDeviceToHost) != hipSuccess) { g_err = std::string(fn) + ": copy failed"; return -1; }
    }
    return 0;
}

static_assert(MC_READLEN_FIXED == MC_SIM_LEN_FIXED && MC_READLEN_REFERENCE == MC_SIM_LEN_REFERENCE, "one numbering of the read-length modes");
extern "C" int mc_genome_set_read_lengths(mc_genome *g, int32_t mode)
{
    if (!g) { g_err = "mc_genome_set_read_lengths: bad argument"; return -1; }
    if (mode != MC_READLEN_FIXED && mode != MC_READLEN_REFERENCE) { g_err = "unknown read-length mode " + std::to_string(mode); return -1; }
    g->read_lengths = mode;
    return 0;
}

static int simulate_var(const mc_genome *g, int L, uint64_t key, int64_t first, int64_t n, uint32_t *d_lens, int64_t *d_roff, uint8_t *d_dst, hipStream_t st,
                        int64_t *total)
{
    *total = 0;
    if (n <= 0) return 0;
    const McSimKind kind = sim_kind(*g, L);
    const McGenomePlacer place = g->placer();
    const uint64_t ekey = mc_mix64(key ^ MC_SIM_EKEY);
    const dim3 grid((unsigned)((n + 63) / 64));
    k_simulate_var<<<grid, dim3(64), 0, st>>>(g->d_bases, place, kind, g->d_thr, key, ekey, first, n, d_lens, nullptr, nullptr);
    HIPCK(hipGetLastError());
    std::vector<uint32_t> lens((size_t)n);
    HIPCK(hipMemcpyAsync(lens.data(), d_lens, (size_t)n * 4, hipMemcpyDeviceToHost, st));
    HIPCK(hipStreamSynchronize(st));
    int64_t sum = 0;
    for (int64_t k = 0; k < n; k++) {
        if (lens[(size_t)k] > 3 * MC_MAXAA) {
            g_err = "read " + std::to_string(first + k) + " of the library is " + std::to_string(lens[(size_t)k]) + " bases long (read length " + std::to_string(L) +
                    " plus its insertions): longer than 510";
            return -1;
        }
        sum += lens[(size_t)k];
    }
    k_sim_scan<<<dim3(1), dim3(1024), 0, st>>>(d_lens, n, d_roff);
    HIPCK(hipGetLastError());
    k_simulate_var<<<grid, dim3(64), 0, st>>>(g->d_bases, place, kind, g->d_thr, key, ekey, first, n, nullptr, d_roff, d_dst);
    HIPCK(hipGetLastError());
    *total = sum;
    return 0;
}

extern "C" int64_t mc_simulate_varlen(mc_genome *g, int32_t read_len, int64_t first, int64_t n, uint64_t seed, uint64_t library_id, uint8_t *dst_host,
                                      int64_t dst_cap, int64_t *offsets)
{
    if (!g || first < 0 || n < 0 || !offsets) { g_err = "mc_simulate_varlen: bad argument"; return -1; }
    if (simulate_begin(g, read_len)) return -1;
    offsets[0] = 0;
    if (n == 0) return 0;
    const int64_t B = std::min<int64_t>(n, stream_batch()), W = std::min(2 * read_len, 3 * MC_MAXAA);
    McDevBuf buf;
    uint8_t *d = nullptr; uint32_t *d_lens = nullptr; int64_t *d_roff = nullptr;
    if (buf.get(&d, (size_t)(B * W + 64)) || buf.get(&d_lens, (size_t)B) || buf.get(&d_roff, (size_t)B + 1)) return -1;
    const uint64_t key = sim_key(seed, library_id);
    int64_t at_byte = 0;
    for (int64_t at = 0; at < n; at += B) {
        const int64_t cnt = std::min(B, n - at);
        int64_t total = 0;
        if (simulate_var(g, read_len, key, first + at, cnt, d_lens, d_roff, d, nullptr, &total)) return -1;
        std::vector<int64_t> ro((size_t)cnt + 1);
        HIPCK(hipMemcpy(ro.data(), d_roff, ro.size() * 8, hipMemcpyDeviceToHost));
        for (int64_t k = 1; k <= cnt; k++) offsets[at + k] = at_byte + ro[(size_t)k];
        if (dst_host && at_byte + total <= dst_cap) HIPCK(hipMemcpy(dst_host + at_byte, d, (size_t)total, hipMemcpyDeviceToHost));
        at_byte += total;
    }
    return at_byte;
}

extern "C" int mc_simulate(mc_genome *g, int32_t read_len, int64_t first, int64_t n, uint64_t seed, uint64_t library_id, uint8_t *dst_host)
{
    if (!g || first < 0 || n < 0 || (n > 0 && !dst_host)) { g_err = "mc_simulate: bad argument"; return -1; }
    if (simulate_begin(g, read_len)) return -1;
    if (n == 0) return 0;
    return simulate_to_host(g, read_len, first, n, sim_key(seed, library_id), dst_host, "mc_simulate");
}

static int train_range(mc_handle *h, int64_t first, int64_t count, int64_t first_read_id, const McGridPars &G, unsigned long long *d_bins, size_t nbins,
                       hipEvent_t e0, hipEvent_t e1, mc_stats &tot)
{
    if (count <= 0) return 0;
    McCtx &c = h->ctx;
    int rc = range_begin(h, c, first, count, first_read_id);
    if (rc == 0) rc = range_end(h, c);
    if (rc == -2 && count > 1) {
        tot.range_splits++;
        const int64_t a = count / 2;
        if ((rc = train_range(h, first, a, first_read_id, G, d_bins, nbins, e0, e1, tot)) != 0) return rc;
        return train_range(h, first + a, count - a, first_read_id + a, G, d_bins, nbins, e0, e1, tot);
    }
    if (rc) return rc;
    stats_add(tot, h->stats);
    const int64_t nrows = (int64_t)c.nrows;
    HIPCK(hipEventRecord(e0, c.stream));
    if (nrows) k_grid_classify<<<dim3((unsigned)((nrows + 127) / 128)), dim3(128), 0, c.stream>>>(G, dev_index(h), h->d_fam, c.d_rows, nrows, d_bins, d_bins + nbins, (double *)(d_bins + 2 * nbins));
    HIPCK(hipEventRecord(e1, c.stream));
    HIPCK(hipEventSynchronize(e1));
    h->train_ms[2] += ev_ms(e0, e1);
    return 0;
}

template <class S> static int simulate_resident(mc_handle *h, const S *s, uint64_t key, int64_t at, int64_t cnt, const McEvents &ev)
{
    hipStream_t st = h->ctx.stream;
    if (hipEventRecord(ev[0], st) != hipSuccess || launch_simulate(s, h->read_len, key, at, cnt, h->d_reads, st) || hipEventRecord(ev[1], st) != hipSuccess) return -1;
    h->reads_dev = h->d_reads; h->nreads = cnt;
    return 0;
}

extern "C" int mc_train_library(mc_handle *h, mc_genome *g, int64_t nreads, uint64_t seed, uint64_t library_id, const double *aln_covs, int32_t n_cov,
                                const int32_t *max_pids, int32_t n_pid, const double *min_scores, int32_t n_score, int64_t *count_hits, int64_t *count_aln, double *count_cov)
{
    if (!h || !h->run_set) { g_err = "mc_set_run() must be called first"; return -1; }
    if (!g || nreads < 0 || !count_hits || !count_aln || !count_cov) { g_err = "mc_train_library: bad argument"; return -1; }
    if (g->lib.paired_end && (nreads & 1)) { g_err = "a paired-end library has an even number of reads (" + std::to_string(nreads) + " given)"; return -1; }
    if (g->device != h->device) { g_err = "mc_train_library: the genome lies on another device than the handle"; return -1; }
    if (h->pipe_nout) { g_err = "mc_train_library: ranges begun with mc_range_begin() are still in flight"; return -1; }
    if (h->abund) { g_err = "mc_train_library: refused while abundance counting is on (mc_set_abundance)"; return -1; }
    McGridPars G; std::vector<int> order;
    if (grid_pars(h, aln_covs, n_cov, max_pids, n_pid, min_scores, n_score, G, order)) return -1;
    HIPCK(hipSetDevice(h->device));
    const int L = h->read_len;
    if (source_for_len(g, L)) return -1;
    const int nfam = h->nfam;
    const size_t nbins = (size_t)n_cov * n_pid * (MC_GRID_MAXS + 1) * nfam;
    const size_t nout = (size_t)n_cov * n_pid * n_score * nfam;
    memset(count_hits, 0, nout * 8); memset(count_aln, 0, nout * 8); memset(count_cov, 0, nout * 8);
    h->train_ms[0] = h->train_ms[1] = h->train_ms[2] = 0.f;
    mc_stats tot; memset(&tot, 0, sizeof tot);
    if (nreads == 0) { h->stats = tot; return 0; }
    const int64_t B = std::min<int64_t>(nreads, stream_batch());
    const bool ref = g->read_lengths == MC_SIM_LEN_REFERENCE;
    h->train_bases = 0;
    if (!ref && (reads_reserve(h, B) || ensure_capacity(h, h->ctx, B))) return -1;
    McDevBuf vb;
    uint8_t *d_sim = nullptr; uint32_t *d_lens = nullptr; int64_t *d_roff = nullptr;
    if (ref && (vb.get(&d_sim, (size_t)(B * std::min(2 * L, 3 * MC_MAXAA) + 64)) || vb.get(&d_lens, (size_t)B) || vb.get(&d_roff, (size_t)B + 1))) return -1;
    unsigned long long *d_bins = nullptr;
    if (vb.get(&d_bins, nbins * 3)) { g_err = "out of device memory"; return -1; }
    McEvents ev;
    if (ev.make(4)) return -1;
    hipStream_t st = h->ctx.stream;
    McModeGuard mode(h, false, true);
    int rc = hipMemsetAsync(d_bins, 0, nbins * 24, st) == hipSuccess ? 0 : -1;
    if (rc) g_err = "hipMemsetAsync failed";
    const uint64_t key = sim_key(seed, library_id);
    for (int64_t at = 0; at < nreads && rc == 0 && !ref; at += B) {
        const int64_t cnt = std::min(B, nreads - at);
        if (simulate_resident(h, g, key, at, cnt, ev)) { rc = -1; break; }
        rc = train_range(h, 0, cnt, at, G, d_bins, nbins, ev[2], ev[3], tot);
        if (rc) break;
        h->train_ms[0] += ev_ms(ev[0], ev[1]);
        h->train_bases += cnt * L;
    }
    if (ref) {
        McLenBorrow len(h);
        for (int64_t at = 0; at < nreads && rc == 0; at += B) {
            const int64_t cnt = std::min(B, nreads - at);
            int64_t bases = 0;
            if (hipEventRecord(ev[0], st) != hipSuccess || simulate_var(g, L, key, at, cnt, d_lens, d_roff, d_sim, st, &bases)) { rc = -1; break; }
            McDevBuf bb;
            uint8_t *d_sorted = nullptr; uint32_t *d_perm = nullptr;
            std::vector<uint32_t> start; std::vector<int64_t> boff;
            if (vl_bucket(bb, st, d_sim, d_roff, cnt, bases, &d_sorted, &d_perm, start, boff) || hipEventRecord(ev[1], st) != hipSuccess || hipEventSynchronize(ev[1]) != hipSuccess) { rc = -1; break; }
            h->train_ms[0] += ev_ms(ev[0], ev[1]);
            h->train_bases += bases;
            const McPieces P = mc_cut_pieces(vl_bins(start), B);
            tot.reads += P.nshort;
            if (!P.v.empty() && (rc = len.pools(P.Lmax, P.nmax)) != 0) break;
            for (const McPiece &q : P.v) {
                if ((rc = len.use(q.L)) != 0) break;
                h->reads_dev = d_sorted + boff[(size_t)q.L]; h->nreads = q.bin_n;
                if ((rc = train_range(h, q.first, q.n, at + q.bin_first + q.first, G, d_bins, nbins, ev[2], ev[3], tot)) != 0) break;
            }
            (void)hipStreamSynchronize(st);
        }
        rc = len.close(rc);
        h->reads_dev = nullptr; h->nreads = 0;
    }
    h->res_rows = nullptr; h->n_res_rows = 0; h->best.clear(); h->best_from = nullptr;
    std::vector<unsigned long long> bins(nbins * 3);
    if (rc == 0 && (hipMemcpyAsync(bins.data(), d_bins, nbins * 24, hipMemcpyDeviceToHost, st) != hipSuccess || hipStreamSynchronize(st) != hipSuccess)) { g_err = "mc_train_library: copy of the bins failed"; rc = -1; }
    if (rc) { (void)hipStreamSynchronize(st); return rc; }
    grid_counts(bins, nbins, n_cov * n_pid, n_score, nfam, order, count_hits, count_aln, count_cov);
    h->stats = tot; h->train_ms[1] = tot.ms_total;
    return 0;
}

extern "C" int64_t mc_train_library_bases(const mc_handle *h) { if (!h) { g_err = "null handle"; return -1; } return h->train_bases; }

extern "C" int mc_train_times(const mc_handle *h, float *ms)
{
    if (!h || !ms) { g_err = "null argument"; return -1; }
    for (int k = 0; k < 3; k++) ms[k] = h->train_ms[k];
    return 0;
}

static int community_open(mc_community *c, const uint8_t *bases, const int64_t *contig_off, int32_t ncontig, const int32_t *member_first_contig, const int64_t *copies,
                          int32_t M, int32_t device)
{
    if (!bases || !contig_off || ncontig < 1 || !member_first_contig || !copies) { g_err = "mc_community_open: bad argument"; return -1; }
    if (M < 1 || M > MC_SIM_MAX_MEMBERS) { g_err = "mc_community_open: " + std::to_string(M) + " members (1 .. " + std::to_string(MC_SIM_MAX_MEMBERS) + ")"; return -1; }
    if (source_args(*c, bases, contig_off, ncontig)) return -1;
    if (member_first_contig[0] != 0 || member_first_contig[M] != ncontig) { g_err = "mc_community_open: member_first_contig must run from 0 to ncontig"; return -1; }
    for (int m = 0; m < M; m++) {
        if (member_first_contig[m + 1] <= member_first_contig[m]) { g_err = "mc_community_open: member " + std::to_string(m) + " has no contig"; return -1; }
        if (copies[m] < 1 || copies[m] > MC_SIM_MAX_COPIES) { g_err = "mc_community_open: member " + std::to_string(m) + " has " + std::to_string(copies[m]) + " copies (1 .. " + std::to_string(MC_SIM_MAX_COPIES) + ")"; return -1; }
    }
    if (source_open(*c, bases, contig_off, ncontig, device)) return -1;
    c->M = M; c->copies.assign(copies, copies + M); c->mfirst.assign(member_first_contig, member_first_contig + M + 1);
    c->member_reads.assign((size_t)M, 0);
    if (c->mem.get(&c->d_total, (size_t)M) || c->mem.get(&c->d_cum, (size_t)M + 1) || c->mem.get(&c->d_mfirst, (size_t)M + 1) || c->mem.get(&c->d_counts, (size_t)M) ||
        hipMemcpy(c->d_mfirst, member_first_contig, sizeof(int32_t) * (M + 1), hipMemcpyHostToDevice) != hipSuccess) {
        g_err = "mc_community_open: out of device memory";
        return -1;
    }
    return 0;
}
extern "C" mc_community *mc_community_open(const uint8_t *bases, const int64_t *contig_off, int32_t ncontig, const int32_t *member_first_contig, const int64_t *copies,
                                           int32_t M, int32_t device)
{
    mc_community *c = new mc_community();
    if (community_open(c, bases, contig_off, ncontig, member_first_contig, copies, M, device)) { mc_community_close(c); return nullptr; }
    return c;
}
extern "C" void mc_community_close(mc_community *c) { source_close(c); }

static int community_counts_reset(mc_community *c, hipStream_t st) { HIPCK(hipMemsetAsync(c->d_counts, 0, sizeof(unsigned long long) * c->M, st)); return 0; }
static int community_counts(mc_community *c, hipStream_t st)
{
    std::vector<unsigned long long> v((size_t)c->M);
    HIPCK(hipMemcpyAsync(v.data(), c->d_counts, sizeof(unsigned long long) * v.size(), hipMemcpyDeviceToHost, st));
    HIPCK(hipStreamSynchronize(st));
    for (int m = 0; m < c->M; m++) c->member_reads[(size_t)m] = (int64_t)v[(size_t)m];
    return 0;
}

extern "C" int mc_community_simulate(mc_community *c, int32_t read_len, int64_t first, int64_t n, uint64_t seed, uint64_t library_id, uint8_t *dst_host)
{
    if (!c || first < 0 || n < 0 || (n > 0 && !dst_host)) { g_err = "mc_community_simulate: bad argument"; return -1; }
    if (simulate_begin(c, read_len)) return -1;
    std::fill(c->member_reads.begin(), c->member_reads.end(), 0);
    if (n == 0) return 0;
    if (community_counts_reset(c, nullptr) || simulate_to_host(c, read_len, first, n, sim_key(seed, library_id), dst_host, "mc_community_simulate")) return -1;
    return community_counts(c, nullptr);
}

extern "C" int mc_community_member_reads(mc_community *c, int64_t *out)
{
    if (!c || !out) { g_err = "mc_community_member_reads: bad argument"; return -1; }
    memcpy(out, c->member_reads.data(), sizeof(int64_t) * (size_t)c->M);
    return 0;
}

extern "C" int mc_community_library(mc_handle *h, mc_community *c, int64_t nreads, uint64_t seed, uint64_t library_id)
{
    if (!h || !h->run_set) { g_err = "mc_set_run() must be called first"; return -1; }
    if (!c || nreads < 0) { g_err = "mc_community_library: bad argument"; return -1; }
    if (nreads > 0x7fffffff) { g_err = "mc_community_library: more than 2^31 - 1 reads"; return -1; }
    if (c->lib.paired_end && (nreads & 1)) { g_err = "a paired-end library has an even number of reads (" + std::to_string(nreads) + " given)"; return -1; }
    if (c->device != h->device) { g_err = "mc_community_library: the community lies on another device than the handle"; return -1; }
    if (h->pipe_nout) { g_err = "mc_community_library: ranges begun with mc_range_begin() are still in flight"; return -1; }
    if (h->abund) { g_err = "mc_community_library: refused while abundance counting is on (it runs best hits only; mc_set_abundance)"; return -1; }
    HIPCK(hipSetDevice(h->device));
    if (source_for_len(c, h->read_len)) return -1;
    std::fill(c->member_reads.begin(), c->member_reads.end(), 0);
    h->comm_ms[0] = h->comm_ms[1] = 0.f;
    mc_stats tot; memset(&tot, 0, sizeof tot);
    std::vector<mc_best_hit> all_best;
    h->res_rows = nullptr; h->n_res_rows = 0; h->best.clear(); h->best_from = nullptr;
    if (nreads == 0) { h->stats = tot; return 0; }
    const int64_t B = std::min<int64_t>(nreads, stream_batch());
    if (reads_reserve(h, B) || ensure_capacity(h, h->ctx, B)) return -1;
    McEvents ev;
    if (ev.make(2)) return -1;
    hipStream_t st = h->ctx.stream;
    McModeGuard mode(h, true, h->rows_stay);
    int rc = community_counts_reset(c, st);
    const uint64_t key = sim_key(seed, library_id);
    for (int64_t at = 0; at < nreads && rc == 0; at += B) {
        const int64_t cnt = std::min(B, nreads - at);
        if (simulate_resident(h, c, key, at, cnt, ev)) { rc = -1; break; }
        if ((rc = mc_run_range(h, 0, cnt, at)) != 0) break;
        h->comm_ms[0] += ev_ms(ev[0], ev[1]);
        best_materialize(h);
        all_best.insert(all_best.end(), h->best.begin(), h->best.end());
        stats_add(tot, h->stats);
    }
    if (rc == 0) rc = community_counts(c, st); else (void)hipStreamSynchronize(st);
    if (rc) return rc;
    h->res_rows = nullptr; h->n_res_rows = 0; h->best.swap(all_best); h->best_from = nullptr; h->stats = tot;
    h->comm_ms[1] = tot.ms_total;
    return 0;
}

extern "C" int mc_community_times(const mc_handle *h, float *ms)
{
    if (!h || !ms) { g_err = "null argument"; return -1; }
    ms[0] = h->comm_ms[0]; ms[1] = h->comm_ms[1];
    return 0;
}
```

Baseline: 64.30 million.

## Translate next batch's reads ahead on a side stream during current batch

Splits the six-frame translation/SEG stage out of stage A and issues it for the next range on a dedicated stream while the current range runs stages C and D. The next range_begin takes the precomputed frames when a key of reads generation, range, read length and tables generation matches, and otherwise falls back to translating them itself. Generation counters are bumped wherever reads or tables change, so that stale prefetched frames are dropped. This adds a second stream, events and invalidation bookkeeping, with a risk of races on the shared frames buffer or missed invalidations.

```diff
diff --git a/include/mcensus.h b/include/mcensus.h
--- a/include/mcensus.h
+++ b/include/mcensus.h
@@ -71,6 +71,7 @@
 int mc_range_begin(mc_handle *h, int64_t first, int64_t count, int64_t first_read_id);
 int mc_range_end(mc_handle *h);
 int mc_ranges_in_flight(const mc_handle *h);
+int64_t mc_ranges_translated_ahead(const mc_handle *h);
 
 int64_t mc_debug_stage(mc_handle *h, int what, void *dst, int64_t cap_bytes, int32_t *record_bytes);
 void mc_debug_live(int64_t out[4]);
diff --git a/microbecensus_amd/_native.py b/microbecensus_amd/_native.py
--- a/microbecensus_amd/_native.py
+++ b/microbecensus_amd/_native.py
@@ -102,6 +102,8 @@
     lib.mc_range_begin.argtypes = [C.c_void_p, C.c_int64, C.c_int64, C.c_int64]
     lib.mc_range_end.argtypes = [C.c_void_p]
     lib.mc_ranges_in_flight.argtypes = [C.c_void_p]
+    lib.mc_ranges_translated_ahead.restype = C.c_int64
+    lib.mc_ranges_translated_ahead.argtypes = [C.c_void_p]
     lib.mc_result_rows.restype = C.c_int64
     lib.mc_result_rows.argtypes = [C.c_void_p, C.POINTER(C.POINTER(McRow))]
     lib.mc_result_best_hits.restype = C.c_int64
@@ -222,7 +224,7 @@
 
 
 EXPORTED_SYMBOLS = ["mc_last_error", "mc_device_count", "mc_open", "mc_close", "mc_set_index_cache", "mc_index_cache_check", "mc_open_rapdb", "mc_marker_count", "mc_marker_name", "mc_set_families", "mc_rapdb_verify", "mc_rapdb_write", "mc_index_view", "mc_set_run", "mc_search", "mc_search_varlen",
-                    "mc_upload", "mc_attach", "mc_run", "mc_run_range", "mc_set_counting", "mc_debug_stage", "mc_range_begin", "mc_range_end", "mc_ranges_in_flight", "mc_result_rows", "mc_result_best_hits", "mc_result_stats", "mc_write_m8", "mc_write_m8_named",
+                    "mc_upload", "mc_attach", "mc_run", "mc_run_range", "mc_set_counting", "mc_debug_stage", "mc_range_begin", "mc_range_end", "mc_ranges_in_flight", "mc_ranges_translated_ahead", "mc_result_rows", "mc_result_best_hits", "mc_result_stats", "mc_write_m8", "mc_write_m8_named",
                     "mc_reader_last_error", "mc_set_host_threads", "mc_reader_open", "mc_reader_open_range", "mc_reader_open_bz2_part", "mc_bz2_blocks", "mc_gz_chunks", "mc_reader_open_gz_part", "mc_reader_gz_provide", "mc_reader_gz_end_state", "mc_reader_gz_finish", "mc_reader_run", "mc_reader_reads", "mc_reader_get_stats", "mc_reader_times", "mc_reader_describe", "mc_dupset_open", "mc_dupset_close", "mc_dupset_walk", "mc_reader_take", "mc_reader_close", "mc_reader_trim", "mc_count_bases", "mc_quality_offset",
                     "mc_reader_start", "mc_reader_fetch", "mc_reader_join", "mc_reader_read_len", "mc_reader_nreads", "mc_search_files", "mc_search_files_multi", "mc_set_keep_rows", "mc_set_best_hits_only", "mc_grid_classify", "mc_bootstrap", "mc_bootstrap_ms",
                     "mc_fit_weights", "mc_weights_mue", "mc_fit_weights_ms",
@@ -871,6 +873,9 @@
     def ranges_in_flight(self):
         return self.lib.mc_ranges_in_flight(self.h)
 
+    def ranges_translated_ahead(self):
+        return int(self.lib.mc_ranges_translated_ahead(self.h))
+
     def run_range(self, first, count, first_read_id=0):
         self._check(self.lib.mc_run_range(self.h, first, count, first_read_id), "mc_run_range")
 
diff --git a/microbecensus_amd/csrc/mc_ahead.h b/microbecensus_amd/csrc/mc_ahead.h
--- /dev/null
+++ b/microbecensus_amd/csrc/mc_ahead.h
@@ -0,0 +1,30 @@
+#pragma once
+#include <stdint.h>
+#include <algorithm>
+
+struct McAheadKey { uint64_t reads_gen; int64_t first, count; int32_t read_len, FP; uint64_t tables_gen; };
+struct McAhead { McAheadKey key = {0, 0, 0, 0, 0, 0}; bool live = false; };
+
+inline int64_t mc_ahead_predict(int64_t first, int64_t count, int64_t nreads, int64_t *next_first)
+{
+    *next_first = 0;
+    if (first < 0 || count <= 0 || first > nreads - count) return 0;
+    const int64_t at = first + count;
+    const int64_t n = std::min(count, nreads - at);
+    if (n <= 0) return 0;
+    *next_first = at;
+    return n;
+}
+
+inline void mc_ahead_offer(McAhead &a, const McAheadKey &k) { a.key = k; a.live = true; }
+
+inline void mc_ahead_drop(McAhead &a) { a.live = false; }
+
+inline int64_t mc_ahead_take(McAhead &a, const McAheadKey &want)
+{
+    const bool was = a.live;
+    a.live = false;
+    const McAheadKey &k = a.key;
+    if (!was || want.count <= 0 || k.count <= 0 || k.reads_gen != want.reads_gen || k.first != want.first || k.read_len != want.read_len || k.FP != want.FP || k.tables_gen != want.tables_gen) return 0;
+    return std::min(k.count, want.count);
+}
diff --git a/microbecensus_amd/csrc/mc_hip.hip b/microbecensus_amd/csrc/mc_hip.hip
--- a/microbecensus_amd/csrc/mc_hip.hip
+++ b/microbecensus_amd/csrc/mc_hip.hip
@@ -15,6 +15,7 @@
 #include "k_abundance.h"
 #include "k_coverage.h"
 #include "mc_pieces.h"
+#include "mc_ahead.h"
 #include "mc_owned.h"
 
 #include <map>
@@ -34,7 +35,9 @@
     McDev<McGapCell> d_gws_full; McDev<uint32_t> d_retry, d_retry2; int gap_threads_full = 0;
     McDev<unsigned long long> d_gtab; uint32_t gtab_slots = 0; McDev<uint32_t> d_gleader; McDev<McFlankOut> d_fout;
     McPin<uint32_t> h_c; McPin<unsigned long long> h_stats; McPin<McBestHit> h_best; size_t h_best_cap = 0;
-    const uint8_t *reads = nullptr; int64_t n = 0, first_read_id = 0;
+    const uint8_t *reads = nullptr; int64_t n = 0, first_read_id = 0, first = 0;
+    int ahead_from = -1;
+    bool own_a0 = true;
     uint32_t ntasks = 0, ngaps = 0, gpad = 0, nh = 0, nh_all = 0, nheads = 0, nrows = 0, nbest = 0, nsegs = 0;
     bool busy = false;
 };
@@ -70,6 +73,8 @@
     McDev<uint8_t> d_reads;
     const uint8_t *reads_dev = nullptr;
     McCtx ctx;
+    McStream ahead_stream; McEvent ahead_ev[2][2]; int ahead_p = 0; bool ahead_wait = false;
+    McAhead ahead; uint64_t reads_gen = 0, tables_gen = 0; int64_t ahead_used = 0;
     McPin<mc_row> pin_slot[2]; size_t pin_slot_cap[2] = {0, 0}; int pin_cur = 0;
     McStream side, side2;
     McStream rows_stream; McEvent ev_rows; bool rows_pending = false, rows_ever = false;
@@ -82,6 +87,16 @@
     std::vector<uint8_t> best_cls; int64_t cls_reads[MC_CL_BINS] = {};
 };
 
+static void ahead_drop(mc_handle *h)
+{
+    if (h->ahead_wait) { (void)hipStreamSynchronize(h->ahead_stream); h->ahead_wait = false; }
+    mc_ahead_drop(h->ahead);
+}
+static constexpr bool MC_AHEAD_ON = true;
+static McAheadKey ahead_key(const mc_handle *h, int64_t first, int64_t count) { return {h->reads_gen, first, count, h->read_len, h->FP, h->tables_gen}; }
+static void reads_change(mc_handle *h) { ahead_drop(h); h->reads_gen++; }
+static void tables_change(mc_handle *h) { ahead_drop(h); h->tables_gen++; }
+
 static McIndex dev_index(const mc_handle *h)
 {
     McIndex X; X.res = h->d_res; X.off = h->d_off; X.bstart = h->d_bstart; X.post = h->d_post; X.post8 = h->d_post8; X.keys = h->d_keys; X.rec = h->d_rec; X.filt = h->d_filt; X.wild = h->d_wild; X.pair = h->d_pair; X.rt = h->d_rt; X.rt_mask = h->H.rt_mask; X.nseq = h->H.nseq;
@@ -101,6 +116,7 @@
 {
     if (!h) return;
     (void)hipSetDevice(h->device);
+    ahead_drop(h);
     if (h->rows_stream) (void)hipStreamSynchronize(h->rows_stream);
     delete h;
 }
@@ -156,6 +172,8 @@
         if (c.h_c.alloc(C_N) || c.h_stats.alloc(S_N)) return -1;
     }
     if (h->rows_stream.create() || h->ev_rows.create(false)) return -1;
+    if (h->ahead_stream.create()) return -1;
+    for (auto &pair : h->ahead_ev) for (auto &e : pair) if (e.create()) return -1;
     const McHostIndex &H = h->H;
     if (H.res.size() >= MC_TASK_ABS_LIMIT) { g_err = "marker database too large: more than 16 M residues (MC_TASK_W3)"; return -1; }
     if (h->d_res_base.alloc(H.res.size() + 128) || h->d_off.alloc(H.off.size()) || h->d_bstart.alloc(H.bstart.size()) || h->d_post.alloc(H.post.size() + 1) || h->d_post8.alloc((H.post.size() + 1) * MC_POST_WORDS) ||
@@ -323,6 +341,7 @@
     MC_OT("set_run: tables", t0);
     if (mc_seg_fx_verify(h->hT, nullptr) != 0) { g_err = "internal: the fixed-point SEG tests disagree with the reference arithmetic"; return -1; }
     MC_OT("set_run: seg_fx_verify", t0);
+    tables_change(h);
     memset(&h->hP, 0, sizeof h->hP);
     h->hP.nfam = h->nfam; h->hP.read_len = read_len;
     for (int f = 0; f < h->nfam; f++) { h->hP.min_cov[f] = min_cov[f]; h->hP.min_score[f] = min_score[f]; h->hP.max_aaid[f] = max_aaid[f]; h->hP.aln_stat[f] = aln_stat[f]; }
@@ -347,6 +366,7 @@
 {
     if (nreads <= c.cap_reads && h->read_len <= c.pool_len) return 0;
     if (h->best_from == &c) best_materialize(h);
+    ahead_drop(h);
     double t0 = mc_now();
     int64_t cap = nreads;
     if (cap > (1 << 21) - 1) { g_err = "batch larger than 2097151 reads"; return -1; }
@@ -379,7 +399,7 @@
 static int reads_reserve(mc_handle *h, int64_t nreads)
 {
     const int64_t need = nreads * (int64_t)h->read_len + 16;
-    if (need > h->cap_own) { if (h->d_reads.alloc((size_t)need)) return -1; h->cap_own = need; }
+    if (need > h->cap_own) { reads_change(h); if (h->d_reads.alloc((size_t)need)) return -1; h->cap_own = need; }
     return 0;
 }
 
@@ -387,6 +407,7 @@
 {
     if (!h || !h->run_set) { g_err = "mc_set_run() must be called first"; return -1; }
     HIPCK(hipSetDevice(h->device));
+    reads_change(h);
     if (reads_reserve(h, nreads)) return -1;
     if (nreads) HIPCK(hipMemcpyAsync(h->d_reads, reads, (size_t)nreads * h->read_len, hipMemcpyHostToDevice, h->ctx.stream));
     HIPCK(hipStreamSynchronize(h->ctx.stream));
@@ -397,6 +418,7 @@
 extern "C" int mc_attach(mc_handle *h, const void *device_reads, int64_t nreads)
 {
     if (!h || !h->run_set) { g_err = "mc_set_run() must be called first"; return -1; }
+    reads_change(h);
     h->reads_dev = (const uint8_t *)device_reads; h->nreads = nreads;
     return 0;
 }
@@ -407,8 +429,9 @@
 static int counters_to_host(McCtx &c) { HIPCK(hipMemcpyAsync(c.h_c, c.d_counters, sizeof(uint32_t) * C_N, hipMemcpyDeviceToHost, c.stream)); return 0; }
 
 #ifdef MC_EXP_TIMING
-static int exp_timing_dump(McCtx &c, char stage)
-{
+static int exp_timing_dump(mc_handle *h, McCtx &c, char stage)
+{
+    ahead_drop(h);
     if (stage == 'a') {
         HIPCK(hipStreamSynchronize(c.stream));
         unsigned long long acc[12], cnt[12];
@@ -464,22 +487,14 @@
     return 0;
 }
 #else
-static int exp_timing_dump(McCtx &, char) { return 0; }
+static int exp_timing_dump(mc_handle *, McCtx &, char) { return 0; }
 #endif
 
-static int stage_a(mc_handle *h, McCtx &c)
-{
-    const int64_t n = c.n;
+static int stage_a0(mc_handle *h, McCtx &c, hipStream_t st, const uint8_t *reads, int64_t at, int64_t n, hipEvent_t e0, hipEvent_t e1)
+{
     const int L = h->read_len, FP = h->FP;
-    hipStream_t st = c.stream;
-    McIndex X = dev_index(h);
-    c.ntasks = c.ngaps = c.gpad = c.nh = c.nheads = c.nrows = c.nbest = c.nsegs = 0;
-    HIPCK(hipMemsetAsync(c.d_counters, 0, sizeof(uint32_t) * C_N, st));
-    HIPCK(hipMemsetAsync(c.d_stats, 0, sizeof(unsigned long long) * S_N, st));
-    if (h->best_only) HIPCK(hipMemsetAsync(c.d_cand, 0, (size_t)n, st));
-    HIPCK(hipMemsetAsync(c.d_low, 0, (size_t)n, st));
-    HIPCK(hipEventRecord(c.ev[0], st));
-    const int64_t threads = n * 6;
+    uint8_t *frames = c.d_frames + at * 6 * FP;
+    HIPCK(hipEventRecord(e0, st));
     const size_t lds_rest = (size_t)MC_TS_NLNF(FP) * 8 + (size_t)MC_TS_THREADS * MC_TS_STRIDE(FP);
     const size_t lds_staged = (size_t)MC_TS_STAGE(L) + lds_rest, lds_direct = (size_t)MC_TS_STAGE(0) + lds_rest;
     static const int ts_force = getenv("MC_TS_STAGED") ? atoi(getenv("MC_TS_STAGED")) : -1;
@@ -490,13 +505,31 @@
     const unsigned ts_blocks = (unsigned)((n + MC_TS_READS - 1) / MC_TS_READS);
     if (staged) {
         if (lds > 48 * 1024) HIPCK(hipFuncSetAttribute((const void *)k_translate_seg<true>, hipFuncAttributeMaxDynamicSharedMemorySize, (int)lds));
-        k_translate_seg<true><<<dim3(ts_blocks), dim3(MC_TS_THREADS), lds, st>>>(h->d_T, c.reads, L, n, c.d_frames, FP, h->d_segtab);
+        k_translate_seg<true><<<dim3(ts_blocks), dim3(MC_TS_THREADS), lds, st>>>(h->d_T, reads, L, n, frames, FP, h->d_segtab);
     } else {
         if (lds > 48 * 1024) HIPCK(hipFuncSetAttribute((const void *)k_translate_seg<false>, hipFuncAttributeMaxDynamicSharedMemorySize, (int)lds));
-        k_translate_seg<false><<<dim3(ts_blocks), dim3(MC_TS_THREADS), lds, st>>>(h->d_T, c.reads, L, n, c.d_frames, FP, h->d_segtab);
-    }
-    HIPCK(hipEventRecord(c.ev[1], st));
-    if (exp_timing_dump(c, 'a')) return -1;
+        k_translate_seg<false><<<dim3(ts_blocks), dim3(MC_TS_THREADS), lds, st>>>(h->d_T, reads, L, n, frames, FP, h->d_segtab);
+    }
+    HIPCK(hipEventRecord(e1, st));
+    return 0;
+}
+
+static int stage_a(mc_handle *h, McCtx &c, int64_t covered)
+{
+    const int64_t n = c.n;
+    const int L = h->read_len, FP = h->FP;
+    hipStream_t st = c.stream;
+    McIndex X = dev_index(h);
+    c.ntasks = c.ngaps = c.gpad = c.nh = c.nheads = c.nrows = c.nbest = c.nsegs = 0;
+    HIPCK(hipMemsetAsync(c.d_counters, 0, sizeof(uint32_t) * C_N, st));
+    HIPCK(hipMemsetAsync(c.d_stats, 0, sizeof(unsigned long long) * S_N, st));
+    if (h->best_only) HIPCK(hipMemsetAsync(c.d_cand, 0, (size_t)n, st));
+    HIPCK(hipMemsetAsync(c.d_low, 0, (size_t)n, st));
+    c.own_a0 = covered < n;
+    if (!c.own_a0) HIPCK(hipEventRecord(c.ev[1], st));
+    else if (stage_a0(h, c, st, c.reads + covered * L, covered, n - covered, c.ev[0], c.ev[1])) return -1;
+    if (exp_timing_dump(h, c, 'a')) return -1;
+    const int64_t threads = n * 6;
     if (h->fast_enum) {
         const bool enq = !h->count_traffic;
         const size_t per_wave = enq ? MC_ENQ_WAVE_LDS(FP, L) : sizeof(McEnWave) + MC_EN_WAVE_LDS(FP, L);
@@ -648,7 +681,7 @@
         k_emit_rows<<<dim3((nheads + 255) / 256), dim3(256), 0, st>>>(c.d_heads, nheads, c.d_nrow, c.d_rowoff, c.d_tmp, c.d_rows, c.cap_rows, c.d_bestof, c.d_best, c.d_counters, h->best_only ? 0 : 1);
     }
     HIPCK(hipEventRecord(c.ev[6], st));
-    if (exp_timing_dump(c, 'd')) return -1;
+    if (exp_timing_dump(h, c, 'd')) return -1;
     HIPCK(hipMemcpyAsync(c.h_stats, c.d_stats, sizeof(unsigned long long) * S_N, hipMemcpyDeviceToHost, st));
     return counters_to_host(c);
 }
@@ -721,10 +754,25 @@
 static int range_begin(mc_handle *h, McCtx &c, int64_t first, int64_t count, int64_t first_read_id)
 {
     if (ensure_capacity(h, c, count)) return -1;
-    c.reads = h->reads_dev + first * h->read_len; c.n = count; c.first_read_id = first_read_id;
-    const int rc = stage_a(h, c);
+    c.reads = h->reads_dev + first * h->read_len; c.n = count; c.first_read_id = first_read_id; c.first = first;
+    const int64_t covered = mc_ahead_take(h->ahead, ahead_key(h, first, count));
+    if (h->ahead_wait) { HIPCK(hipStreamWaitEvent(c.stream, h->ahead_ev[h->ahead_p][1], 0)); h->ahead_wait = false; }
+    c.ahead_from = covered ? h->ahead_p : -1;
+    if (covered) { h->ahead_used++; h->ahead_p ^= 1; }
+    const int rc = stage_a(h, c, covered);
     if (rc) { (void)hipStreamSynchronize(c.stream); return rc; }
     c.busy = true;
+    return 0;
+}
+
+static int ahead_issue(mc_handle *h, McCtx &c, int64_t first, int64_t count)
+{
+    if (count <= 0 || count > c.cap_reads || h->read_len > c.pool_len || first < 0 || first + count > h->nreads || !h->reads_dev) return 0;
+    ahead_drop(h);
+    HIPCK(hipStreamWaitEvent(h->ahead_stream, c.ev[4], 0));
+    h->ahead_wait = true;
+    if (stage_a0(h, c, h->ahead_stream, h->reads_dev + first * h->read_len, 0, count, h->ahead_ev[h->ahead_p][0], h->ahead_ev[h->ahead_p][1])) { ahead_drop(h); return -1; }
+    mc_ahead_offer(h->ahead, ahead_key(h, first, count));
     return 0;
 }
 
@@ -739,7 +787,7 @@
     for (uint32_t i = 0; i < nb; i++) { const McBestHit &x = c->h_best[i]; mc_best_hit &o = h->best[i]; o.read = x.read; o.family = x.family; o.aln = x.aln; o.target_len = x.target_len; o.bits = x.bits; }
 }
 
-static int range_end(mc_handle *h, McCtx &c)
+static int range_end(mc_handle *h, McCtx &c, int64_t next_first = 0, int64_t next_count = 0)
 {
     c.busy = false;
     h->cls_results = false;
@@ -748,10 +796,11 @@
     h->stats.reads = c.n;
     int rc = stage_wait(c);
     if (rc == 0) rc = stage_b(h, c);
+    if (rc == 0 && MC_AHEAD_ON) rc = ahead_issue(h, c, next_first, next_count);
     if (rc == 0 && (rc = stage_wait(c)) == 0 && (rc = stage_c(h, c)) == 0) rc = stage_d(h, c);
     if (rc == 0) rc = stage_wait(c);
     if (rc == 0 && c.h_c[C_OVERFLOW]) { g_err = "row buffer overflow"; rc = -2; }
-    if (rc) { (void)hipStreamSynchronize(c.stream); return rc; }
+    if (rc) { (void)hipStreamSynchronize(c.stream); ahead_drop(h); return rc; }
     h->pin_cur ^= 1;
     c.nrows = (c.nh && !h->best_only) ? c.h_c[C_ROWS] : 0u; c.nsegs = c.h_c[C_SEGS]; c.nbest = c.h_c[C_BEST];
     const bool abund = h->abund && !h->best_only;
@@ -784,8 +833,9 @@
     h->stats.bucket_lookups += (int64_t)c.h_stats[S_LOOKUPS]; h->stats.key_probes += (int64_t)c.h_stats[S_KEYPROBES]; h->stats.seed_tasks += (int64_t)c.h_stats[S_TASKS];
     h->stats.seed_exact_asks += (int64_t)c.h_stats[S_EXACT]; h->stats.seed_wild_asks += (int64_t)c.h_stats[S_WILD]; h->stats.seed_pair_asks += (int64_t)c.h_stats[S_PAIRS]; h->stats.seed_probes += (int64_t)c.h_stats[S_PROBES];
     h->stats.gap_tasks += c.ngaps - c.gpad; h->stats.hsps += c.nh_all; h->stats.rows += c.nrows; h->stats.reads_with_rows += c.nsegs;
-    h->stats.ms_translate += ev_ms(c.ev[0], c.ev[1]); h->stats.ms_seed += ev_ms(c.ev[1], c.ev[2]); h->stats.ms_eval += ev_ms(c.ev[2], c.ev[3]);
-    h->stats.ms_gapped += ev_ms(c.ev[3], c.ev[4]); h->stats.ms_sort += ev_ms(c.ev[4], c.ev[5]); h->stats.ms_finish += ev_ms(c.ev[5], c.ev[6]); h->stats.ms_total += ev_ms(c.ev[0], c.ev[6]);
+    const float ms_tr = (c.own_a0 ? ev_ms(c.ev[0], c.ev[1]) : 0.0f) + (c.ahead_from >= 0 ? ev_ms(h->ahead_ev[c.ahead_from][0], h->ahead_ev[c.ahead_from][1]) : 0.0f);
+    h->stats.ms_translate += ms_tr; h->stats.ms_seed += ev_ms(c.ev[1], c.ev[2]); h->stats.ms_eval += ev_ms(c.ev[2], c.ev[3]);
+    h->stats.ms_gapped += ev_ms(c.ev[3], c.ev[4]); h->stats.ms_sort += ev_ms(c.ev[4], c.ev[5]); h->stats.ms_finish += ev_ms(c.ev[5], c.ev[6]); h->stats.ms_total += ms_tr + ev_ms(c.ev[1], c.ev[6]);
     h->stats.classified = (int64_t)c.nbest;
     return 0;
 }
@@ -820,13 +870,21 @@
     return 0;
 }
 
+static int range_end_next(mc_handle *h, int64_t first, int64_t count, bool predict)
+{
+    if (predict) count = mc_ahead_predict(h->ctx.first, h->ctx.n, h->nreads, &first);
+    return range_end(h, h->ctx, first, count);
+}
+
+extern "C" int64_t mc_ranges_translated_ahead(const mc_handle *h) { return h ? h->ahead_used : 0; }
+
 extern "C" int mc_range_end(mc_handle *h)
 {
     if (!h) { g_err = "null handle"; return -1; }
     if (h->pipe_nout == 0) { g_err = "mc_range_end: no range in flight"; return -1; }
     HIPCK(hipSetDevice(h->device));
     h->pipe_nout = 0;
-    return range_end(h, h->ctx);
+    return range_end_next(h, 0, 0, true);
 }
 
 extern "C" int mc_ranges_in_flight(const mc_handle *h) { return h ? h->pipe_nout : 0; }
@@ -836,6 +894,7 @@
     if (!h || !h->run_set || what < 0 || what > 5) { g_err = "mc_debug_stage: bad argument"; return -1; }
     if (h->pipe_nout) { g_err = "mc_debug_stage: ranges are in flight"; return -1; }
     HIPCK(hipSetDevice(h->device));
+    ahead_drop(h);
     const McCtx &c = h->ctx;
     if (what == 4) {
         if (!c.h_c) { g_err = "mc_debug_stage: no range has run"; return -1; }
@@ -864,6 +923,7 @@
 extern "C" int mc_set_counting(mc_handle *h, int on)
 {
     if (!h) { g_err = "null handle"; return -1; }
+    ahead_drop(h);
     h->count_traffic = on != 0;
     return 0;
 }
@@ -882,6 +942,7 @@
 {
     HIPCK(hipSetDevice(h->device));
     if (h->pipe_nout) { g_err = "ranges begun with mc_range_begin() are still in flight"; return -1; }
+    ahead_drop(h);
     const int64_t BMAX = MC_STREAM_BATCH, B = stream_batch(), L = h->read_len;
     double t0 = mc_now();
     int64_t bmax_run = B;
@@ -929,9 +990,12 @@
     bool pending = false;
     auto collect = [&]() { if (pending) { pending = false; R.take(h); } };
     auto release = [&](int k) { std::unique_lock<std::mutex> lk(mu); slot[k].state = 0; cv.notify_all(); };
-    auto end_batch = [&](int k) -> int {
-        int r = mc_range_end(h);
-        if (r == -2) { h->reads_dev = slot[k].dev; h->nreads = slot[k].n; r = mc_run_range(h, 0, slot[k].n, first_read_id + slot[k].first); }
+    auto reads_at = [&](int k) { reads_change(h); h->reads_dev = slot[k].dev; h->nreads = slot[k].n; };
+    auto end_batch = [&](int k, int next) -> int {
+        if (next >= 0) reads_at(next);
+        h->pipe_nout = 0;
+        int r = range_end_next(h, 0, next >= 0 ? slot[next].n : 0, false);
+        if (r == -2) { reads_at(k); r = mc_run_range(h, 0, slot[k].n, first_read_id + slot[k].first); if (next >= 0) reads_at(next); }
         if (r) return r;
         pending = true;
         release(k);
@@ -942,21 +1006,23 @@
         {
             bool ready;
             { std::unique_lock<std::mutex> lk(mu); ready = slot[k].state != 0; }
-            if (!ready && flying >= 0) { if ((rc = end_batch(flying)) != 0) break; flying = -1; collect(); }
+            if (!ready && flying >= 0) { if ((rc = end_batch(flying, -1)) != 0) break; flying = -1; collect(); }
         }
         { std::unique_lock<std::mutex> lk(mu); cv.wait(lk, [&] { return slot[k].state != 0; }); }
         if (slot[k].state == 2) { if (slot[k].rc < 0) { rc = (int)slot[k].rc; if (!up_err.empty()) g_err = up_err; } break; }
-        if (flying >= 0) { if ((rc = end_batch(flying)) != 0) break; flying = -1; }
-        h->reads_dev = slot[k].dev; h->nreads = slot[k].n;
+        if (flying >= 0) { if ((rc = end_batch(flying, k)) != 0) break; flying = -1; }
+        else reads_at(k);
         if ((rc = mc_range_begin(h, 0, slot[k].n, first_read_id + slot[k].first)) != 0) break;
         flying = k;
         collect();
     }
-    if (rc == 0 && flying >= 0) { rc = end_batch(flying); flying = -1; }
+    if (rc == 0 && flying >= 0) { rc = end_batch(flying, -1); flying = -1; }
     if (rc == 0) collect();
-    if (h->pipe_nout) (void)mc_range_end(h);
+    if (h->pipe_nout) { h->pipe_nout = 0; (void)range_end(h, h->ctx); }
+    ahead_drop(h);
     { std::unique_lock<std::mutex> lk(mu); abort_up = true; cv.notify_all(); }
     uploader.join();
+    reads_change(h);
     h->reads_dev = saved_reads; h->nreads = saved_n;
     if (rc) return rc;
     h->res_rows = R.rows.data(); h->n_res_rows = (int64_t)R.rows.size(); h->best.swap(R.best); h->best_from = nullptr; h->stats = R.tot;
@@ -1037,7 +1103,7 @@
 
 struct McLenBorrow {
     mc_handle *h; int read_len, FP; const uint8_t *reads_dev; int64_t nreads; bool tables = false, pars = false, open = true;
-    explicit McLenBorrow(mc_handle *h_) : h(h_), read_len(h_->read_len), FP(h_->FP), reads_dev(h_->reads_dev), nreads(h_->nreads) {}
+    explicit McLenBorrow(mc_handle *h_) : h(h_), read_len(h_->read_len), FP(h_->FP), reads_dev(h_->reads_dev), nreads(h_->nreads) { ahead_drop(h); }
     McLenBorrow(const McLenBorrow &) = delete;
     ~McLenBorrow() { (void)close(-1); }
     void set_len(int L) { h->read_len = L; h->FP = ((L / 3 + 2) + 3) & ~3; }
@@ -1052,6 +1118,7 @@
         auto it = h->vl_tables.find(L);
         if (it == h->vl_tables.end()) { it = h->vl_tables.emplace(L, McTables()).first; mc_fill_tables(it->second, h->H, L, h->vl_thr); }
         tables = true;
+        tables_change(h);
         HIPCK(hipMemcpy(h->d_T, &it->second, sizeof(McTables), hipMemcpyHostToDevice));
         if (P) { pars = true; HIPCK(hipMemcpy(h->d_P, P, sizeof(McClassPars), hipMemcpyHostToDevice)); }
         set_len(L);
@@ -1061,6 +1128,7 @@
     {
         if (!open) return rc;
         open = false;
+        tables_change(h); reads_change(h);
         h->read_len = read_len; h->FP = FP; h->reads_dev = reads_dev; h->nreads = nreads;
         hipError_t e = tables ? run_tables_up(h) : hipSuccess;
         if (e == hipSuccess && pars) e = hipMemcpy(h->d_P, &h->hP, sizeof(McClassPars), hipMemcpyHostToDevice);
@@ -1071,21 +1139,29 @@
 
 template <class BlockOf> static int run_pieces(mc_handle *h, McLenBorrow &len, const std::vector<McPiece> &pieces, BlockOf block_of, const McClassPars *pars, McResults &R)
 {
-    auto begin = [&](const McPiece &q) -> int {
-        if (len.use(q.L, pars ? pars + q.tag : nullptr)) return -1;
-        h->reads_dev = block_of(q); h->nreads = q.bin_n;
+    auto same_bin = [](const McPiece &a, const McPiece &b) { return a.tag == b.tag && a.L == b.L && a.bin_first == b.bin_first && a.bin_n == b.bin_n; };
+    auto begin = [&](const McPiece &q, const McPiece *before) -> int {
+        if (!before || !same_bin(*before, q)) {
+            if (len.use(q.L, pars ? pars + q.tag : nullptr)) return -1;
+            reads_change(h);
+            h->reads_dev = block_of(q); h->nreads = q.bin_n;
+        }
         return mc_range_begin(h, q.first, q.n, q.bin_first + q.first);
     };
-    int rc = pieces.empty() ? 0 : begin(pieces[0]);
+    int rc = pieces.empty() ? 0 : begin(pieces[0], nullptr);
     for (size_t j = 0; rc == 0 && j < pieces.size(); j++) {
         const McPiece &q = pieces[j];
-        rc = mc_range_end(h);
+        const McPiece *nx = j + 1 < pieces.size() ? &pieces[j + 1] : nullptr;
+        const bool ahead = nx && same_bin(q, *nx);
+        h->pipe_nout = 0;
+        rc = range_end_next(h, ahead ? nx->first : 0, ahead ? nx->n : 0, false);
         if (rc == -2) rc = mc_run_range(h, q.first, q.n, q.bin_first + q.first);
         if (rc) break;
-        if (j + 1 < pieces.size() && (rc = begin(pieces[j + 1])) != 0) break;
+        if (nx && (rc = begin(*nx, &q)) != 0) break;
         R.take(h, q.tag);
     }
-    if (h->pipe_nout) (void)mc_range_end(h);
+    if (h->pipe_nout) { h->pipe_nout = 0; (void)range_end(h, h->ctx); }
+    ahead_drop(h);
     return rc;
 }
 
@@ -2081,6 +2157,7 @@
 template <class S> static int simulate_resident(mc_handle *h, const S *s, uint64_t key, int64_t at, int64_t cnt, const McEvents &ev)
 {
     hipStream_t st = h->ctx.stream;
+    reads_change(h);
     if (hipEventRecord(ev[0], st) != hipSuccess || launch_simulate(s, h->read_len, key, at, cnt, h->d_reads, st) || hipEventRecord(ev[1], st) != hipSuccess) return -1;
     h->reads_dev = h->d_reads; h->nreads = cnt;
     return 0;
@@ -2094,6 +2171,7 @@
     if (g->lib.paired_end && (nreads & 1)) { g_err = "a paired-end library has an even number of reads (" + std::to_string(nreads) + " given)"; return -1; }
     if (g->device != h->device) { g_err = "mc_train_library: the genome lies on another device than the handle"; return -1; }
     if (h->pipe_nout) { g_err = "mc_train_library: ranges begun with mc_range_begin() are still in flight"; return -1; }
+    ahead_drop(h);
     if (h->abund) { g_err = "mc_train_library: refused while abundance counting is on (mc_set_abundance)"; return -1; }
     McGridPars G; std::vector<int> order;
     if (grid_pars(h, aln_covs, n_cov, max_pids, n_pid, min_scores, n_score, G, order)) return -1;
@@ -2148,12 +2226,14 @@
             if (!P.v.empty() && (rc = len.pools(P.Lmax, P.nmax)) != 0) break;
             for (const McPiece &q : P.v) {
                 if ((rc = len.use(q.L)) != 0) break;
+                reads_change(h);
                 h->reads_dev = d_sorted + boff[(size_t)q.L]; h->nreads = q.bin_n;
                 if ((rc = train_range(h, q.first, q.n, at + q.bin_first + q.first, G, d_bins, nbins, ev[2], ev[3], tot)) != 0) break;
             }
             (void)hipStreamSynchronize(st);
         }
         rc = len.close(rc);
+        reads_change(h);
         h->reads_dev = nullptr; h->nreads = 0;
     }
     h->res_rows = nullptr; h->n_res_rows = 0; h->best.clear(); h->best_from = nullptr;
@@ -2239,6 +2319,7 @@
     if (c->lib.paired_end && (nreads & 1)) { g_err = "a paired-end library has an even number of reads (" + std::to_string(nreads) + " given)"; return -1; }
     if (c->device != h->device) { g_err = "mc_community_library: the community lies on another device than the handle"; return -1; }
     if (h->pipe_nout) { g_err = "mc_community_library: ranges begun with mc_range_begin() are still in flight"; return -1; }
+    ahead_drop(h);
     if (h->abund) { g_err = "mc_community_library: refused while abundance counting is on (it runs best hits only; mc_set_abundance)"; return -1; }
     HIPCK(hipSetDevice(h->device));
     if (source_for_len(c, h->read_len)) return -1;
```

Result: faster. 66.39 million (median of 6 runs) (+3.2%).
